# LBM-EPFL/MaD

Hardware: AMD Instinct MI355X
Metric: anchor-pair x rotation correlations/sec on 256^3 map; top-k pose agreement (higher is better)
Workload: dtype i8 (correlation, exact int32 accumulate) / f64 (binning, pose scoring)

## Files before the change

### include/mad_amd.h

```cpp
#ifndef MAD_AMD_H
#define MAD_AMD_H

#include <stdint.h>

#ifdef __cplusplus
extern "C" {
#endif

#define MAD_OK        0
#define MAD_EINVAL   -22
#define MAD_ENOMEM   -12
#define MAD_ENOSPC   -28
#define MAD_ENODEV   -19
#define MAD_EDOM     -33
#define MAD_EHIP     -5

#define MAD_MAX_Z      128
#define MAD_MAX_FIELDS 64
#define MAD_POSE_CLUSTER_MAX_N 4096
#define MAD_RESULT_COLS 23

typedef struct mad_ctx mad_ctx;
typedef struct mad_set mad_set;


int mad_init(int device, mad_ctx **out);
void mad_destroy(mad_ctx *ctx);
const char *mad_last_error(const mad_ctx *ctx);
int mad_synchronize(mad_ctx *ctx);
void *mad_stream(mad_ctx *ctx);
int mad_set_overlap(mad_ctx *ctx, int on);
int mad_timing_enable(mad_ctx *ctx, int on);
int mad_timing_reset(mad_ctx *ctx);
int mad_timing_get(mad_ctx *ctx, const char *what, double *total_ms, int64_t *launches);
double mad_last_ms(mad_ctx *ctx, const char *what);

int mad_probe_peaks(mad_ctx *ctx, double *copy_gbs, double *i8_tops);

int mad_set_eqsp(mad_ctx *ctx, int which, int Z, const double *bounds,
                 const double *to_dom, const double *adj_sec);


int mad_upload_field(mad_ctx *ctx, int slot, const float *gx, const float *gy, const float *gz,
                     int nx, int ny, int nz);
int mad_upload_field_device(mad_ctx *ctx, int slot, const float *g3_device, int nx, int ny, int nz);
int mad_free_field(mad_ctx *ctx, int slot);


int mad_set_orient_window(mad_ctx *ctx, double gw_sig);
int mad_orient(mad_ctx *ctx, int slot, int octave, const int32_t *coords, int n, int r,
               int lim_main, int lim_sec,
               int32_t *row_anchor, int32_t *row_main, int32_t *row_sec, double *row_R,
               int32_t *row_count, int64_t *n_rows, int64_t cap, int32_t *n_reject);


int mad_describe(mad_ctx *ctx, int slot, int octave, const int32_t *coords, const double *R,
                 int64_t n_rows, int r, int16_t *dsc);
int mad_describe_sized(mad_ctx *ctx, int slot, int octave, const int32_t *coords, const double *R,
                       int64_t n_rows, int r, int dsc_size, int16_t *dsc);


int mad_correlate(mad_ctx *ctx, const int16_t *hi, int64_t n_hi, const int16_t *lo, int64_t n_lo,
                  int D, double cc, int32_t *pair_hi, int32_t *pair_lo, double *pair_score,
                  int64_t *n_pairs, int64_t cap);


int mad_pose_score(mad_ctx *ctx, const int32_t *pair_hi, const int32_t *pair_lo, const double *pair_score,
                   int64_t n_pairs,
                   const double *hi_p, const double *hi_R, const int32_t *hi_meta, int64_t n_hi,
                   const double *lo_p, const double *lo_R, const int32_t *lo_meta, int64_t n_lo,
                   const double *hi_cloud, int64_t l_hi, const double *lo_cloud, int64_t l_lo,
                   double dist, double *results, int32_t *counts);

int mad_topk(mad_ctx *ctx, const int32_t *counts, int64_t n, int64_t k, int64_t *order);


int mad_set_create(mad_ctx *ctx, mad_set **out);
void mad_set_destroy(mad_ctx *ctx, mad_set *set);
int mad_set_build(mad_ctx *ctx, mad_set *set, const int *slot_of_octave,
                  const int32_t *anc_coords, const int32_t *anc_octave, const double *anc_subv,
                  const int32_t *anc_index, int n_anchors, int r, int lim_main, int lim_sec);
int mad_set_build_many(mad_ctx *ctx, int n_sets, mad_set *const *sets, const int *slot_of_octave,
                       const int32_t *const *anc_coords, const int32_t *const *anc_octave,
                       const double *const *anc_subv, const int32_t *const *anc_index, const int *n_anchors,
                       int r, int lim_main, int lim_sec);
int mad_set_mark_wide(mad_ctx *ctx, mad_set *set, int wide);
int mad_set_is_wide(mad_ctx *ctx, const mad_set *set);
int mad_set_load(mad_ctx *ctx, mad_set *set, int64_t n_rows, const int32_t *row_anchor,
                 const int32_t *row_main, const double *row_R, const int16_t *dsc, int D,
                 const double *anc_subv, const int32_t *anc_index, const int32_t *anc_octave, int n_anchors);
int mad_set_size(mad_ctx *ctx, const mad_set *set, int64_t *n_rows, int32_t *n_anchors);
int mad_set_download(mad_ctx *ctx, const mad_set *set, int32_t *row_anchor, int32_t *row_main,
                     int32_t *row_sec, double *row_R, int16_t *dsc);

int mad_match_topk(mad_ctx *ctx, const mad_set *hi, const mad_set *lo, double cc, double dist,
                   int64_t k, double *results, int64_t *pair_index, int64_t *n_out, int64_t *stats);
int mad_match_topk_many(mad_ctx *ctx, int n, const mad_set *const *hi, const mad_set *lo, double cc, double dist,
                        int64_t k, double *results, int64_t *pair_index, int64_t *n_out, int64_t *stats);

int mad_match_topk_many_begin(mad_ctx *ctx, int n, const mad_set *const *hi, const mad_set *lo, double cc, double dist,
                              int64_t k, double *results, int64_t *pair_index, int64_t *n_out, int64_t *stats);
int mad_match_topk_many_finish(mad_ctx *ctx);
int mad_match_topk_many_begin2(mad_ctx *ctx, int n, const mad_set *const *hi, const mad_set *lo, double cc, double dist,
                               int64_t k, double *results, int64_t *pair_index, int64_t *n_out, int64_t *stats,
                               uint8_t *used_hi, uint8_t *used_lo);
int mad_match_topk_many2(mad_ctx *ctx, int n, const mad_set *const *hi, const mad_set *lo, double cc, double dist,
                         int64_t k, double *results, int64_t *pair_index, int64_t *n_out, int64_t *stats,
                         uint8_t *used_hi, uint8_t *used_lo);
int mad_set_batching(mad_ctx *ctx, int on);
int mad_set_option(mad_ctx *ctx, const char *name, double value);

int mad_last_pose_kernel(mad_ctx *ctx);
int64_t mad_last_pose_selected(mad_ctx *ctx);
int64_t mad_device_allocations(mad_ctx *ctx);
int mad_match_fetch(mad_ctx *ctx, int32_t *pair_hi, int32_t *pair_lo, double *pair_score,
                    int32_t *counts, int64_t cap);
int mad_match_results(mad_ctx *ctx, const mad_set *hi, const mad_set *lo, double *results, int64_t cap);
int mad_match_used(mad_ctx *ctx, uint8_t *hi_anchor_used, int32_t n_hi_anchors,
                   uint8_t *lo_anchor_used, int32_t n_lo_anchors);


int mad_upload_density(mad_ctx *ctx, const float *grid, int nx, int ny, int nz,
                       double ox, double oy, double oz, double voxsp);
int mad_refine(mad_ctx *ctx, double *coords, int n_cand, int64_t n_atoms, int n_steps,
               double max_step, double min_step, int32_t *converged, int32_t *last_step);


int mad_structure_to_density(mad_ctx *ctx, const double *atoms, const double *mass, int64_t n,
                             double resolution, double voxsp, double isovalue, int pad,
                             int32_t dims[3], double origin[3], float *grid);


int mad_ccc(mad_ctx *ctx, float *grid1, const int32_t dims1[3], const double origin1[3],
            float *grid2, const int32_t dims2[3], const double origin2[3],
            double voxsp, double isovalue, double *ccc);


int mad_match_shard_pairs(mad_ctx *ctx, const mad_set *hi, const mad_set *lo, int64_t lo_begin, int64_t lo_end, double cc,
                          uint8_t *used_hi, uint8_t *used_lo, int64_t *n_pairs);

int mad_match_shard_topk(mad_ctx *ctx, const mad_set *hi, const mad_set *lo, const uint8_t *used_hi_all,
                         const uint8_t *used_lo_all, double dist, int64_t k, double *results, int64_t *pair_rank,
                         int32_t *counts, int64_t *n_out, int64_t *l_hi);

int64_t mad_match_shard_record_doubles(int64_t k);
int mad_match_shard_begin(mad_ctx *ctx, const mad_set *hi, const mad_set *lo, int64_t lo_begin, int64_t lo_end, int64_t n_lo,
                          double cc, uint8_t *d_flags);
int mad_match_shard_score(mad_ctx *ctx, const mad_set *hi, const mad_set *lo, const uint8_t *d_flags_all, double dist, int64_t k,
                          double *d_out);
int mad_match_shard_collect(mad_ctx *ctx, const mad_set *hi, const double *d_all, int64_t n, int *ticket);
int mad_match_shard_wait(mad_ctx *ctx, int ticket, double *out, int64_t n);


int64_t mad_set_wire_bytes(int D, int64_t cap_rows);
int mad_set_export(mad_ctx *ctx, const mad_set *share, void *wire, int wire_on_device, int64_t cap_rows);
int mad_set_import(mad_ctx *ctx, mad_set *set, const void *wires, int wires_on_device, int n_shares, int64_t cap_rows,
                   const int32_t *anc_coords, const int32_t *anc_octave, const double *anc_subv, const int32_t *anc_index,
                   int n_anchors);
int mad_set_lane(mad_ctx *ctx, const mad_set *set);
void *mad_set_stream(mad_ctx *ctx, const mad_set *set);
int mad_set_bind_lane(mad_ctx *ctx, mad_set *set, int lane);

int mad_density_ccc(mad_ctx *ctx, const double *atoms, const double *mass, int n_cand, int64_t n,
                    double resolution, double density_isovalue, double ccc_isovalue, double *ccc);

int mad_dock_refine_score(mad_ctx *ctx, int n_struct, const double *base_atoms, const double *mass, const int64_t *first_atom,
                          int n_cand, const int32_t *cand_struct, const double *hi_p, const double *lo_p, const double *rot,
                          int n_steps, double max_step, double min_step, double resolution, double density_isovalue,
                          double ccc_isovalue, double *coords, int32_t *converged, int32_t *last_step, double *ccc);


int mad_grid_overlap(mad_ctx *ctx, float *grid1, const int32_t d1[3], const double o1[3], float *grid2,
                     const int32_t d2[3], const double o2[3], double voxsp, double isovalue, int64_t *common,
                     int64_t *n_pos1);

int mad_overlap_matrix(mad_ctx *ctx, const double *atoms, const double *mass, const int64_t *first_atom,
                       int n_struct, double resolution, double voxsp, double density_isovalue,
                       double overlap_isovalue, double *overlap);


typedef struct mad_space mad_space;

int mad_space_create(mad_ctx *ctx, mad_space **out);
void mad_space_destroy(mad_ctx *ctx, mad_space *s);

int mad_space_build(mad_ctx *ctx, mad_space *s, const void *grid, int is_f64, int nx, int ny, int nz, int pad,
                    int oct_mode, const double *g0, const double *g2, int radius, double sig2,
                    const double *pre, int pre_radius, const double *const *lu, const double *const *ev_w,
                    const int32_t *const *ev_i, int slot_up, int slot_base);

int mad_space_info(mad_ctx *ctx, const mad_space *s, int *n_octaves, int32_t *dims6, int32_t *kind2, int32_t *is_f64_2);

int mad_space_download(mad_ctx *ctx, const mad_space *s, int entry, int what, void *out);

int mad_space_peaks(mad_ctx *ctx, const mad_space *s, int entry, double threshold, int border, int64_t *lin_index,
                    double *value, int64_t cap, int64_t *n_out);

int mad_space_patches(mad_ctx *ctx, const mad_space *s, int entry, const int32_t *coords, int n, int r, void *out);

int mad_space_localize(mad_ctx *ctx, const mad_space *s, int entry, const int32_t *cand, int n, int32_t *status,
                       int32_t *coord, void *H, void *G, int64_t *n_undecided);

int mad_localize_volume(mad_ctx *ctx, const void *vol, int is_f64, int nx, int ny, int nz, const int32_t *cand, int n,
                        int32_t *status, int32_t *coord, void *H, void *G, int64_t *n_undecided);

int mad_pose_cluster_many(mad_ctx *ctx, int n_match, const double *const *rows, const int32_t *n_rows,
                          const double *const *cloud, const int32_t *n_cloud, double rmsd_thresh, int32_t *const *owner_out,
                          double *const *d2min_out, int32_t *n_done_out, int32_t *status_out);

#ifdef __cplusplus
}
#endif
#endif
```

### mad_amd/_lib.py

```python
import ctypes as C
import os

import numpy as np

_HERE = os.path.dirname(os.path.abspath(__file__))
LIB_PATH = os.environ.get("MAD_LIB_PATH") or os.path.join(_HERE, "libmad_amd.so")
RESULT_COLS = 23
POSE_CLUSTER_MAX_N = 4096
WIDE_FROM_R = 11
WIDE_C = 108
WIDE_MAX = WIDE_C + 127

ERRORS = {-22: "EINVAL", -12: "ENOMEM", -28: "ENOSPC", -19: "ENODEV", -33: "EDOM", -5: "EHIP"}

SYMBOLS = [
    "mad_init", "mad_destroy", "mad_last_error", "mad_synchronize", "mad_stream", "mad_set_overlap",
    "mad_timing_enable", "mad_timing_reset", "mad_timing_get", "mad_last_ms", "mad_probe_peaks",
    "mad_set_eqsp", "mad_upload_field", "mad_upload_field_device", "mad_free_field",
    "mad_set_orient_window", "mad_orient", "mad_describe", "mad_describe_sized", "mad_correlate", "mad_pose_score", "mad_topk",
    "mad_set_create", "mad_set_destroy", "mad_set_build", "mad_set_build_many", "mad_set_load", "mad_set_mark_wide", "mad_set_is_wide", "mad_set_size", "mad_set_download",
    "mad_match_topk", "mad_match_topk_many", "mad_match_topk_many_begin", "mad_match_topk_many_finish", "mad_match_topk_many_begin2", "mad_match_topk_many2", "mad_set_batching", "mad_set_option", "mad_last_pose_kernel", "mad_last_pose_selected", "mad_device_allocations", "mad_match_fetch", "mad_match_results", "mad_match_used",
    "mad_match_shard_pairs", "mad_match_shard_topk", "mad_match_shard_begin", "mad_match_shard_score", "mad_match_shard_record_doubles", "mad_match_shard_collect", "mad_match_shard_wait",
    "mad_set_wire_bytes", "mad_set_export", "mad_set_import", "mad_set_lane", "mad_set_stream", "mad_set_bind_lane",
    "mad_upload_density", "mad_refine", "mad_structure_to_density", "mad_ccc", "mad_density_ccc", "mad_dock_refine_score", "mad_grid_overlap", "mad_overlap_matrix",
    "mad_space_create", "mad_space_destroy", "mad_space_build", "mad_space_info", "mad_space_download",
    "mad_space_peaks", "mad_space_patches", "mad_space_localize", "mad_localize_volume",
    "mad_pose_cluster_many",
]


class MadBackendError(RuntimeError):
    pass


_dll = None


def _share_torch_hip_runtime():
    import importlib.util
    if os.environ.get("MAD_OWN_HIP_RUNTIME", "0") == "1":
        return
    try:
        spec = importlib.util.find_spec("torch")
    except (ImportError, ValueError):
        spec = None
    if spec is None or not spec.submodule_search_locations:
        return
    for d in spec.submodule_search_locations:
        path = os.path.join(d, "lib", "libamdhip64.so")
        if os.path.exists(path):
            try:
                C.CDLL(path, mode=C.RTLD_GLOBAL)
            except OSError:
                pass
            return


def load_library():
    global _dll
    if _dll is None:
        if not os.path.exists(LIB_PATH):
            raise MadBackendError(
                "MaD> %s not found: build it with `python -c 'import __graft_entry__ as g; g.build()'` "
                "or `make -C mad_amd/csrc` (there is no CPU fallback)" % LIB_PATH)
        _share_torch_hip_runtime()
        try:
            _dll = C.CDLL(LIB_PATH)
        except OSError as e:
            raise MadBackendError("MaD> cannot load %s: %s" % (LIB_PATH, e))
        _dll.mad_last_error.restype = C.c_char_p
        _dll.mad_last_error.argtypes = [C.c_void_p]
        _dll.mad_stream.restype = C.c_void_p
        _dll.mad_stream.argtypes = [C.c_void_p]
        _dll.mad_last_ms.restype = C.c_double
        _dll.mad_last_ms.argtypes = [C.c_void_p, C.c_char_p]
        _dll.mad_set_stream.restype = C.c_void_p
        _dll.mad_set_stream.argtypes = [C.c_void_p, C.c_void_p]
        _dll.mad_last_pose_selected.restype = C.c_int64
        _dll.mad_last_pose_selected.argtypes = [C.c_void_p]
        _dll.mad_device_allocations.restype = C.c_int64
        _dll.mad_device_allocations.argtypes = [C.c_void_p]
        _dll.mad_set_wire_bytes.restype = C.c_int64
        _dll.mad_set_wire_bytes.argtypes = [C.c_int, C.c_int64]
        _dll.mad_match_shard_record_doubles.restype = C.c_int64
        _dll.mad_match_shard_record_doubles.argtypes = [C.c_int64]
        _dll.mad_destroy.restype = None
        _dll.mad_set_destroy.restype = None
        _dll.mad_space_destroy.restype = None
    return _dll


def _p(a):
    return a.ctypes.data_as(C.c_void_p) if a is not None else None


def _c(a, dt):
    return np.ascontiguousarray(a, dtype=dt)


def _pad_rows(dsc, to=128):
    d = dsc.shape[1] if dsc.ndim == 2 else 0
    if d == 0 or d % to == 0:
        return dsc
    out = np.zeros((dsc.shape[0], (d + to - 1) // to * to), dsc.dtype)
    out[:, :d] = dsc
    return out


class BuildBatch(object):

    def __init__(self, lib, jobs, r, lim_main, lim_sec, gw_sig=0.0):
        self.lib, self.r, self.lim_main, self.lim_sec, self.gw_sig = lib, int(r), int(lim_main), int(lim_sec), float(gw_sig)
        n = len(jobs)
        self.sets = [job[5] if len(job) > 5 and job[5] is not None else DeviceSet(lib) for job in jobs]
        self._keep = []
        coords, octave, subv, index, counts, slots = [], [], [], [], [], []
        for job in jobs:
            c, o = _c(job[1], np.int32).reshape(-1, 3), _c(job[2], np.int32)
            v, i = _c(job[3], np.float64).reshape(-1, 3), _c(job[4], np.int32)
            if not (len(c) == len(o) == len(v) == len(i)):
                raise ValueError("set_build_many: anchor arrays of different lengths")
            self._keep += [c, o, v, i]
            coords.append(c.ctypes.data); octave.append(o.ctypes.data); subv.append(v.ctypes.data); index.append(i.ctypes.data)
            counts.append(len(o))
            slots += [int(job[0][0]), int(job[0][1])]
        self.counts = counts
        self._h = (C.c_void_p * max(n, 1))(*[s.h.value for s in self.sets])
        self._slots = (C.c_int * max(2 * n, 1))(*slots)
        self._coords = (C.c_void_p * max(n, 1))(*coords)
        self._octave = (C.c_void_p * max(n, 1))(*octave)
        self._subv = (C.c_void_p * max(n, 1))(*subv)
        self._index = (C.c_void_p * max(n, 1))(*index)
        self._n = (C.c_int * max(n, 1))(*counts)

    def run(self):
        self.lib.set_orient_window(self.gw_sig)
        for s, n in zip(self.sets, self.counts):
            s.n_anchors = n
        self.lib._chk(self.lib.dll.mad_set_build_many(self.lib.ctx, C.c_int(len(self.sets)), self._h, self._slots, self._coords, self._octave,
                                                      self._subv, self._index, self._n, C.c_int(self.r), C.c_int(self.lim_main),
                                                      C.c_int(self.lim_sec)))
        return self.sets


class DeviceSet(object):

    def __init__(self, lib, lane=None):
        self.lib = lib
        self.h = C.c_void_p()
        lib._chk(lib.dll.mad_set_create(lib.ctx, C.byref(self.h)))
        self.n_anchors = 0
        if lane is not None:
            self.bind_lane(lane)

    def lane(self):
        return int(self.lib.dll.mad_set_lane(self.lib.ctx, self.h))

    def is_wide(self):
        return int(self.lib.dll.mad_set_is_wide(self.lib.ctx, self.h)) == 1

    def bind_lane(self, lane):
        self.lib._chk(self.lib.dll.mad_set_bind_lane(self.lib.ctx, self.h, C.c_int(int(lane))))

    def stream(self):
        return self.lib.dll.mad_set_stream(self.lib.ctx, self.h)

    def size(self):
        n = C.c_int64(0)
        a = C.c_int32(0)
        self.lib._chk(self.lib.dll.mad_set_size(self.lib.ctx, self.h, C.byref(n), C.byref(a)))
        return n.value, a.value

    def download(self, want_dsc=True, D=1024):
        n, _ = self.size()
# ... 246 lines not shown
        R = np.zeros((cap, 9))
        cnt = np.zeros((cap, Z), np.int32) if want_counts else None
        nrows = C.c_int64(0)
        nrej = C.c_int32(0)
        self._chk(self.dll.mad_orient(self.ctx, C.c_int(slot), C.c_int(octave), _p(coords), C.c_int(n), C.c_int(r),
                                      C.c_int(lim_main), C.c_int(lim_sec), _p(ra), _p(rm), _p(rs), _p(R), _p(cnt),
                                      C.byref(nrows), C.c_int64(cap), C.byref(nrej)))
        k = nrows.value
        return dict(anchor=ra[:k].copy(), main=rm[:k].copy(), sec=rs[:k].copy(), R=R[:k].reshape(k, 3, 3).copy(),
                    counts=None if cnt is None else cnt[:k].copy(), n_reject=nrej.value)

    def describe(self, slot, octave, coords, R, r=8, Zd=16, dsc_size=64):
        coords = _c(coords, np.int32).reshape(-1, 3)
        R = _c(R, np.float64).reshape(-1, 9)
        n = len(coords)
        out = np.zeros((n, dsc_size * Zd), np.int16)
        self._chk(self.dll.mad_describe_sized(self.ctx, C.c_int(slot), C.c_int(octave), _p(coords), _p(R), C.c_int64(n), C.c_int(r),
                                              C.c_int(dsc_size), _p(out)))
        return out

    def correlate(self, hi, lo, cc):
        hi, lo = _pad_rows(_c(hi, np.int16)), _pad_rows(_c(lo, np.int16))
        n_hi, D = hi.shape
        n_lo = lo.shape[0]
        npairs = C.c_int64(0)
        cap = 1 << 16
        while True:
            ph, pl, ps = np.zeros(cap, np.int32), np.zeros(cap, np.int32), np.zeros(cap)
            rc = self.dll.mad_correlate(self.ctx, _p(hi), C.c_int64(n_hi), _p(lo), C.c_int64(n_lo), C.c_int(D), C.c_double(cc),
                                        _p(ph), _p(pl), _p(ps), C.byref(npairs), C.c_int64(cap))
            if rc == -28:
                cap = npairs.value
                continue
            self._chk(rc)
            break
        k = npairs.value
        return ph[:k].copy(), pl[:k].copy(), ps[:k].copy()

    def pose_score(self, pair_hi, pair_lo, pair_score, hi_p, hi_R, hi_meta, lo_p, lo_R, lo_meta, hi_cloud, lo_cloud,
                   dist=4.0, want_results=True):
        pair_hi, pair_lo = _c(pair_hi, np.int32), _c(pair_lo, np.int32)
        pair_score = _c(pair_score, np.float64)
        hi_p, lo_p = _c(hi_p, np.float64), _c(lo_p, np.float64)
        hi_R, lo_R = _c(hi_R, np.float64).reshape(-1, 9), _c(lo_R, np.float64).reshape(-1, 9)
        hi_meta, lo_meta = _c(hi_meta, np.int32), _c(lo_meta, np.int32)
        hi_cloud, lo_cloud = _c(hi_cloud, np.float64), _c(lo_cloud, np.float64)
        n = len(pair_hi)
        res = np.zeros((n, RESULT_COLS)) if want_results else None
        cnt = np.zeros(n, np.int32)
        self._chk(self.dll.mad_pose_score(self.ctx, _p(pair_hi), _p(pair_lo), _p(pair_score), C.c_int64(n),
                                          _p(hi_p), _p(hi_R), _p(hi_meta), C.c_int64(len(hi_p)),
                                          _p(lo_p), _p(lo_R), _p(lo_meta), C.c_int64(len(lo_p)),
                                          _p(hi_cloud), C.c_int64(len(hi_cloud)), _p(lo_cloud), C.c_int64(len(lo_cloud)),
                                          C.c_double(dist), _p(res), _p(cnt)))
        return res, cnt

    def topk(self, counts, k):
        counts = _c(counts, np.int32)
        k = min(int(k), len(counts))
        order = np.zeros(max(k, 1), np.int64)
        self._chk(self.dll.mad_topk(self.ctx, _p(counts), C.c_int64(len(counts)), C.c_int64(k), _p(order)))
        return order[:k]

    def set_build(self, slots, anc_coords, anc_octave, anc_subv, anc_index, r=8, lim_main=6, lim_sec=6, into=None, gw_sig=0.0):
        self.set_orient_window(gw_sig)
        s = into if into is not None else DeviceSet(self)
        slots = (C.c_int * 2)(int(slots[0]), int(slots[1]))
        anc_coords = _c(anc_coords, np.int32).reshape(-1, 3)
        anc_octave = _c(anc_octave, np.int32)
        anc_subv = _c(anc_subv, np.float64).reshape(-1, 3)
        anc_index = _c(anc_index, np.int32)
        s.n_anchors = len(anc_octave)
        self._chk(self.dll.mad_set_build(self.ctx, s.h, slots, _p(anc_coords), _p(anc_octave), _p(anc_subv), _p(anc_index),
                                         C.c_int(len(anc_octave)), C.c_int(r), C.c_int(lim_main), C.c_int(lim_sec)))
        return s

    def prepare_build_many(self, jobs, r=8, lim_main=6, lim_sec=6, gw_sig=0.0):
        return BuildBatch(self, jobs, r, lim_main, lim_sec, gw_sig)

    def set_build_many(self, jobs, r=8, lim_main=6, lim_sec=6, gw_sig=0.0):
        return self.prepare_build_many(jobs, r, lim_main, lim_sec, gw_sig).run()

    def set_load(self, row_anchor, row_main, row_R, dsc, anc_subv, anc_index, anc_octave, wide=False):
        s = DeviceSet(self)
        if wide:
            self._chk(self.dll.mad_set_mark_wide(self.ctx, s.h, C.c_int(1)))
        row_anchor, row_main = _c(row_anchor, np.int32), _c(row_main, np.int32)
        row_R = _c(row_R, np.float64).reshape(-1, 9)
        dsc = _c(dsc, np.int16)
        if dsc.ndim != 2:
            dsc = dsc.reshape(len(row_anchor), -1)
        dsc = _pad_rows(dsc)
        anc_subv = _c(anc_subv, np.float64).reshape(-1, 3)
        anc_index, anc_octave = _c(anc_index, np.int32), _c(anc_octave, np.int32)
        s.n_anchors = len(anc_index)
        self._chk(self.dll.mad_set_load(self.ctx, s.h, C.c_int64(len(row_anchor)), _p(row_anchor), _p(row_main), _p(row_R),
                                        _p(dsc), C.c_int(dsc.shape[1] if len(dsc) else 1024), _p(anc_subv), _p(anc_index),
                                        _p(anc_octave), C.c_int(len(anc_index))))
        return s

    def match_topk(self, hi, lo, cc, dist, k):
        k = int(k)
        res = np.zeros((max(k, 1), RESULT_COLS))
        idx = np.zeros(max(k, 1), np.int64)
        n_out = C.c_int64(0)
        stats = np.zeros(4, np.int64)
        self._chk(self.dll.mad_match_topk(self.ctx, hi.h, lo.h, C.c_double(cc), C.c_double(dist), C.c_int64(k), _p(res), _p(idx),
                                          C.byref(n_out), _p(stats)))
        g = n_out.value
        return res[:g], idx[:g], dict(n_pairs=int(stats[0]), l_hi=int(stats[1]), l_lo=int(stats[2]), n_corr=int(stats[3]))

    def match_topk_many(self, his, lo, cc, dist, k, want_used=False):
        h = self._many_args(his, lo, k, want_used)
        n = h["n"]
        if want_used:
            self._chk(self.dll.mad_match_topk_many2(self.ctx, C.c_int(n), h["arr"], lo.h, C.c_double(cc), C.c_double(dist), C.c_int64(h["k"]),
                                                    _p(h["res"]), _p(h["idx"]), _p(h["n_out"]), _p(h["stats"]), _p(h["used_hi"]),
                                                    _p(h["used_lo"])))
        else:
            self._chk(self.dll.mad_match_topk_many(self.ctx, C.c_int(n), h["arr"], lo.h, C.c_double(cc), C.c_double(dist), C.c_int64(h["k"]),
                                                   _p(h["res"]), _p(h["idx"]), _p(h["n_out"]), _p(h["stats"])))
        return self._many_unpack(h)

    @staticmethod
    def _many_args(his, lo, k, want_used):
        k = int(k)
        n = len(his)
        h = dict(n=n, k=k, res=np.zeros((max(n, 1), max(k, 1), RESULT_COLS)), idx=np.zeros((max(n, 1), max(k, 1)), np.int64),
                 n_out=np.zeros(max(n, 1), np.int64), stats=np.zeros((max(n, 1), 4), np.int64), sets=(list(his), lo),
                 arr=(C.c_void_p * max(n, 1))(*[x.h.value for x in his]), want_used=bool(want_used))
        if want_used:
            h["hi_off"] = np.concatenate([[0], np.cumsum([x.n_anchors for x in his], dtype=np.int64)]).astype(np.int64)
            h["used_hi"] = np.zeros(max(int(h["hi_off"][-1]), 1), np.uint8)
            h["used_lo"] = np.zeros((max(n, 1), max(lo.n_anchors, 1)), np.uint8)
        return h

    @staticmethod
    def _many_unpack(h):
        out = []
        for i in range(h["n"]):
            g = int(h["n_out"][i])
            st = h["stats"][i]
            row = (h["res"][i, :g], h["idx"][i, :g], dict(n_pairs=int(st[0]), l_hi=int(st[1]), l_lo=int(st[2]), n_corr=int(st[3])))
            if h["want_used"]:
                a, b = int(h["hi_off"][i]), int(h["hi_off"][i + 1])
                n_lo = h["sets"][1].n_anchors
                row += (h["used_hi"][a:b].astype(bool), h["used_lo"][i, :n_lo].astype(bool))
            out.append(row)
        return out

    def last_pose_kernel(self):
        return int(self.dll.mad_last_pose_kernel(self.ctx))

    def last_pose_selected(self):
        return int(self.dll.mad_last_pose_selected(self.ctx))

    def device_allocations(self):
        return int(self.dll.mad_device_allocations(self.ctx))

    def match_topk_many_begin(self, his, lo, cc, dist, k, want_used=False):
        h = self._many_args(his, lo, k, want_used)
        n = h["n"]
        if want_used:
            self._chk(self.dll.mad_match_topk_many_begin2(self.ctx, C.c_int(n), h["arr"], lo.h, C.c_double(cc), C.c_double(dist),
                                                          C.c_int64(h["k"]), _p(h["res"]), _p(h["idx"]), _p(h["n_out"]), _p(h["stats"]),
                                                          _p(h["used_hi"]), _p(h["used_lo"])))
        else:
            self._chk(self.dll.mad_match_topk_many_begin(self.ctx, C.c_int(n), h["arr"], lo.h, C.c_double(cc), C.c_double(dist),
                                                         C.c_int64(h["k"]), _p(h["res"]), _p(h["idx"]), _p(h["n_out"]), _p(h["stats"])))
        self._open_brackets = getattr(self, "_open_brackets", []) + [h]
        return h

    def match_topk_many_finish(self, h):
        pending = getattr(self, "_open_brackets", [])
        if not pending or pending[0] is not h:
            raise MadBackendError("MaD> match_topk_many_finish: brackets finish in the order they were begun")
        self._open_brackets = pending[1:]
        self._chk(self.dll.mad_match_topk_many_finish(self.ctx))
        return self._many_unpack(h)

    def match_shard_pairs(self, hi, lo, lo_begin, lo_end, cc):
        used_hi, used_lo = np.zeros(max(hi.n_anchors, 1), np.uint8), np.zeros(max(lo.n_anchors, 1), np.uint8)
        n = C.c_int64(0)
        self._chk(self.dll.mad_match_shard_pairs(self.ctx, hi.h, lo.h, C.c_int64(lo_begin), C.c_int64(lo_end), C.c_double(cc),
                                                 _p(used_hi), _p(used_lo), C.byref(n)))
        return used_hi[:hi.n_anchors], used_lo[:lo.n_anchors], n.value

    def match_shard_topk(self, hi, lo, used_hi_all, used_lo_all, dist, k):
        uh, ul = _c(used_hi_all, np.uint8), _c(used_lo_all, np.uint8)
        assert len(uh) == hi.n_anchors and len(ul) == lo.n_anchors
        res = np.zeros((k, RESULT_COLS))
        rank, cnt = np.zeros(k, np.int64), np.zeros(k, np.int32)
        n, l_hi = C.c_int64(0), C.c_int64(0)
        self._chk(self.dll.mad_match_shard_topk(self.ctx, hi.h, lo.h, _p(uh), _p(ul), C.c_double(dist), C.c_int64(k), _p(res), _p(rank),
                                                _p(cnt), C.byref(n), C.byref(l_hi)))
        m = n.value
        return res[:m].copy(), cnt[:m].copy(), rank[:m].copy(), l_hi.value

    def match_shard_record_doubles(self, k):
        return int(self.dll.mad_match_shard_record_doubles(C.c_int64(int(k))))

    def match_shard_begin(self, hi, lo, lo_begin, lo_end, n_lo, cc, flags_ptr):
        self._chk(self.dll.mad_match_shard_begin(self.ctx, hi.h, lo.h, C.c_int64(int(lo_begin)), C.c_int64(int(lo_end)), C.c_int64(int(n_lo)),
                                                 C.c_double(cc), C.c_void_p(int(flags_ptr))))

    def match_shard_score(self, hi, lo, flags_all_ptr, dist, k, out_ptr):
        self._chk(self.dll.mad_match_shard_score(self.ctx, hi.h, lo.h, C.c_void_p(int(flags_all_ptr)), C.c_double(dist), C.c_int64(int(k)),
                                                 C.c_void_p(int(out_ptr))))

    def match_shard_collect(self, hi, all_ptr, n):
        t = C.c_int(0)
        self._chk(self.dll.mad_match_shard_collect(self.ctx, hi.h, C.c_void_p(int(all_ptr)), C.c_int64(int(n)), C.byref(t)))
        return t.value

    def match_shard_wait(self, ticket, n):
        out = np.zeros(int(n))
        self._chk(self.dll.mad_match_shard_wait(self.ctx, C.c_int(int(ticket)), _p(out), C.c_int64(int(n))))
        return out

    def set_wire_bytes(self, cap_rows, D=1024):
        n = int(self.dll.mad_set_wire_bytes(C.c_int(int(D)), C.c_int64(int(cap_rows))))
        if n < 0:
            raise ValueError("set_wire_bytes(%r, %r)" % (cap_rows, D))
        return n

    def set_export(self, share, cap_rows, wire=None, device_ptr=None):
        if device_ptr is not None:
            self._chk(self.dll.mad_set_export(self.ctx, share.h, C.c_void_p(int(device_ptr)), C.c_int(1), C.c_int64(int(cap_rows))))
            return None
        nbytes = self.set_wire_bytes(cap_rows)
        if wire is None:
            wire = np.zeros(nbytes, np.uint8)
        if wire.dtype != np.uint8 or wire.size != nbytes or not wire.flags.c_contiguous:
            raise ValueError("set_export: wire must be a contiguous uint8 array of %d bytes" % nbytes)
        self._chk(self.dll.mad_set_export(self.ctx, share.h, _p(wire), C.c_int(0), C.c_int64(int(cap_rows))))
        return wire

    def set_import(self, n_shares, cap_rows, anc_coords, anc_octave, anc_subv, anc_index, wires=None, device_ptr=None, into=None):
        s = into if into is not None else DeviceSet(self)
        anc_octave = _c(anc_octave, np.int32)
        anc_subv = _c(anc_subv, np.float64).reshape(-1, 3)
        anc_index = _c(anc_index, np.int32)
        anc_coords = None if anc_coords is None else _c(anc_coords, np.int32).reshape(-1, 3)
        n = len(anc_octave)
        if len(anc_subv) != n or len(anc_index) != n or (anc_coords is not None and len(anc_coords) != n):
            raise ValueError("set_import: anchor arrays of different lengths")
        if device_ptr is not None:
            src, on_dev = C.c_void_p(int(device_ptr)), 1
        else:
            wires = np.ascontiguousarray(wires, dtype=np.uint8)
            if wires.size != n_shares * self.set_wire_bytes(cap_rows):
                raise ValueError("set_import: %d bytes for %d shares of %d" % (wires.size, n_shares, self.set_wire_bytes(cap_rows)))
            src, on_dev = _p(wires), 0
        s.n_anchors = n
        self._chk(self.dll.mad_set_import(self.ctx, s.h, src, C.c_int(on_dev), C.c_int(int(n_shares)), C.c_int64(int(cap_rows)),
                                          _p(anc_coords), _p(anc_octave), _p(anc_subv), _p(anc_index), C.c_int(n)))
        return s

    def match_fetch(self, n_pairs):
        ph, pl = np.zeros(n_pairs, np.int32), np.zeros(n_pairs, np.int32)
        ps, cn = np.zeros(n_pairs), np.zeros(n_pairs, np.int32)
        self._chk(self.dll.mad_match_fetch(self.ctx, _p(ph), _p(pl), _p(ps), _p(cn), C.c_int64(n_pairs)))
        return ph, pl, ps, cn

    def match_results(self, hi, lo, n_pairs):
        res = np.zeros((max(n_pairs, 1), RESULT_COLS))
        self._chk(self.dll.mad_match_results(self.ctx, hi.h, lo.h, _p(res), C.c_int64(n_pairs)))
        return res[:n_pairs]

    def match_used(self, n_hi_anchors, n_lo_anchors):
        uh, ul = np.zeros(max(n_hi_anchors, 1), np.uint8), np.zeros(max(n_lo_anchors, 1), np.uint8)
        self._chk(self.dll.mad_match_used(self.ctx, _p(uh), C.c_int32(n_hi_anchors), _p(ul), C.c_int32(n_lo_anchors)))
        return uh[:n_hi_anchors].astype(bool), ul[:n_lo_anchors].astype(bool)

    def pose_cluster_many(self, rows_list, clouds, n_samples_list, rmsd_thresh=10.0):
        nm = len(rows_list)
        if not (len(clouds) == len(n_samples_list) == nm):
            raise ValueError("pose_cluster_many: %d row lists, %d clouds, %d sample counts" % (nm, len(clouds), len(n_samples_list)))
        rows, cl, ns = [], [], []
        for r, c, k in zip(rows_list, clouds, n_samples_list):
            r = _c(r, np.float64).reshape(-1, RESULT_COLS)
            if int(k) < 0:
                raise ValueError("pose_cluster_many: n_samples = %d" % int(k))
            rows.append(r)
            cl.append(_c(c, np.float64).reshape(-1, 3))
            ns.append(min(len(r), int(k)))
        owner = [np.zeros(n, np.int32) for n in ns]
        d2min = [np.zeros(n, np.float64) for n in ns]
        n_rows, n_cloud = np.array(ns, np.int32), np.array([len(c) for c in cl], np.int32)
        n_done, status = np.zeros(max(nm, 1), np.int32), np.zeros(max(nm, 1), np.int32)
        PP = C.c_void_p * max(nm, 1)
        ptrs = [PP(*[a.ctypes.data if a.size else None for a in arrs]) for arrs in (rows, cl, owner, d2min)]
        self._chk(self.dll.mad_pose_cluster_many(self.ctx, C.c_int(nm), ptrs[0], _p(n_rows), ptrs[1], _p(n_cloud), C.c_double(float(rmsd_thresh)),
                                                 ptrs[2], ptrs[3], _p(n_done), _p(status)))
        return [(owner[m], d2min[m], int(n_done[m]), int(status[m])) for m in range(nm)]

    def upload_density(self, grid, origin, voxsp):
        grid = _c(grid, np.float32)
        nx, ny, nz = grid.shape
        self._chk(self.dll.mad_upload_density(self.ctx, _p(grid), C.c_int(nx), C.c_int(ny), C.c_int(nz),
                                              C.c_double(origin[0]), C.c_double(origin[1]), C.c_double(origin[2]), C.c_double(voxsp)))

    def refine(self, coords, n_steps=500, max_step=0.5, min_step=0.01):
        c = _c(coords, np.float64).copy()
        single = c.ndim == 2
        if single:
# ... 118 lines not shown
```

### mad_amd/csrc/mad_common.h

```cpp
#pragma once

#include <hip/hip_runtime.h>

#include <cmath>
#include <cstdarg>
#include <cstdint>
#include <cstdio>
#include <cstdlib>
#include <cstring>

#include "../../include/mad_amd.h"

#define MAD_WAVE 64
#define MAD_ZLUT 1024
#define MAD_MAX_BELT 32


struct __attribute__((aligned(16))) EqspFastLds {
    float g32[MAD_MAX_Z][4];
    float z_in_lo[MAD_MAX_BELT], z_in_hi[MAD_MAX_BELT], belt_lo0[MAD_MAX_BELT], belt_inv_w[MAD_MAX_BELT];
    int belt_first[MAD_MAX_BELT], belt_count[MAD_MAX_BELT];
    unsigned char zlut[MAD_ZLUT];
    float4 belt_f[MAD_MAX_BELT];
    int2 belt_i[MAD_MAX_BELT];
    double dir[MAD_MAX_Z][4];
    double zthr[MAD_MAX_BELT][4];
    int nbelt;
    int tier2_ok;
    double th_lo[MAD_MAX_Z], th_hi[MAD_MAX_Z], ph_lo[MAD_MAX_BELT], ph_hi[MAD_MAX_BELT];
};

#define MAD_TAB_BELTS 4
#define MAD_TAB_PBINS 2048
#define MAD_TAB_ZBINS 2048
#define MAD_TAB_GUARD 4e-3
struct __attribute__((aligned(16))) EqspTabLds {
    unsigned char zbelt[MAD_TAB_ZBINS];
    unsigned char ptab[MAD_TAB_BELTS][MAD_TAB_PBINS];
};

#define MAD_T2_MARGIN64 1e-9
#define MAD_T2_MARGIN32 2e-6

struct EqspDev {
    int Z;
    int nbelt;
    double th_lo[MAD_MAX_Z];
    double th_hi[MAD_MAX_Z];
    double ph_lo[MAD_MAX_Z];
    double ph_hi[MAD_MAX_Z];
    int belt_first[MAD_MAX_Z];
    int belt_count[MAD_MAX_Z];
    double to_dom[MAD_MAX_Z][9];
    double adj_sec[MAD_MAX_Z][9];
    unsigned char zlut[MAD_ZLUT];
    float z_in_lo[MAD_MAX_BELT];
    float z_in_hi[MAD_MAX_BELT];
    float belt_lo0[MAD_MAX_BELT];
    float belt_inv_w[MAD_MAX_BELT];
    int belt_first32[MAD_MAX_BELT];
    int belt_count32[MAD_MAX_BELT];
    float g32[MAD_MAX_Z][4];
    EqspFastLds image;
    EqspTabLds tab;
    int tab_ok;
};

#ifndef MAD_EQSP_GUARD
#define MAD_EQSP_GUARD 4e-5
#endif

struct FieldDev {
    const float4 *tex;
    int nx, ny, nz;
    const unsigned *tex4;
};

#ifdef __HIPCC__
__host__ __device__
#endif
static inline bool mad_ball_interior(int c0, int c1, int c2, int nx, int ny, int nz) {
    const int reach = 14;
    return c0 - reach >= 1 && c0 + reach <= nx - 2 && c1 - reach >= 1 && c1 + reach <= ny - 2 && c2 - reach >= 1 && c2 + reach <= nz - 2;
}


struct DevBuf {
    void *p = nullptr;
    size_t cap = 0;
};

enum { MAD_T_ORIENT = 0, MAD_T_DESCRIBE, MAD_T_CORRELATE, MAD_T_PAIRS, MAD_T_POSE, MAD_T_TOPK, MAD_T_REFINE,
       MAD_T_DENSITY, MAD_T_CCC, MAD_T_COUNT };

#define MAD_T_RING 32
#define MAD_LANES 8
#define MAD_BRACKETS 3
#define MAD_SHARD_RING 8
#define MAD_RES (2 * MAD_LANES)

struct TimerGroup {
    hipEvent_t start[MAD_T_RING];
    hipEvent_t stop[MAD_T_RING];
    int pending = 0;
    double total_ms = 0.0;
    int64_t launches = 0;
};

struct DensityDev {
    float *grid = nullptr;
    float4 *grad = nullptr;
    int nx = 0, ny = 0, nz = 0;
    double o[3] = {0, 0, 0};
    double vs = 0;
};

struct MatchState {
    int64_t n_pairs = 0;
    int32_t l_hi = 0, l_lo = 0;
    int32_t n_hi_anchors = 0, n_lo_anchors = 0;
    int64_t cap_c = 0;
    int64_t cap_pairs = 0;
    int lane = 0;
    bool pruned = false, fits = true;
    const void *hi = nullptr, *lo = nullptr;
    uint64_t hi_gen = 0, lo_gen = 0;
    double dist = 0;
    int64_t cap_pairs_used = 0;
    int64_t n_sel = 0;
    const void *shard_hi = nullptr, *shard_lo = nullptr;
    int64_t shard_begin = 0, shard_end = 0, shard_pairs = 0, shard_cap_pairs = 0;
};

struct ShardAsync {
    const void *hi = nullptr, *lo = nullptr;
    uint64_t hi_gen = 0, lo_gen = 0;
    int64_t begin = 0, nb = 0, n_lo = 0, cap_pairs = 0;
};

struct mad_ctx {
    int device = -1;
    hipStream_t stream = nullptr;
    hipStream_t lane_stream[MAD_LANES] = {};
    int next_set_lane = 0;
    bool overlap = true;
    int ori_queue_cap = 1 << 20, dsc_queue_cap = 1 << 20;
    int pose_mx = 0;
    int pose_split = -1;
    int64_t n_device_allocs = 0;
    int64_t pose_split_min = 4096;
    bool batch_gemm = false;
    bool spatial_order = true;
    char err[512] = {0};
    FieldDev fields[MAD_MAX_FIELDS];
    void *field_mem[MAD_MAX_FIELDS];
    EqspDev *eq[2] = {nullptr, nullptr};
    EqspDev eq_host[2];
    bool eq_set[2] = {false, false};
    double gw_sig = 0.0, gw_built = 0.0;
    unsigned long long *gw_tab = nullptr;
    int gw_r = -1;
    int8_t *mask_off = nullptr;
    int mask_r = -1;
    int mask_n = 0;
    unsigned *ball_colinfo = nullptr;
    bool dsc_ball = false;
    DevBuf scratch[64 * MAD_LANES];
    int lane = 0;
    hipEvent_t lane_done[MAD_BRACKETS][MAD_RES];
    hipEvent_t lane_pre[MAD_LANES];
    hipEvent_t gemm_done[MAD_BRACKETS];
    void *host_res[MAD_BRACKETS][MAD_RES] = {};
    size_t host_res_cap[MAD_BRACKETS][MAD_RES] = {};
    void *host_used[MAD_BRACKETS][MAD_RES] = {};
    size_t host_used_cap[MAD_BRACKETS][MAD_RES] = {};
    int res_slot = 0, res_idx = 0;
    int64_t *pinned = nullptr;
    int next_pinned = 64;
    DensityDev dens;
    MatchState match;
    ShardAsync shard_async[MAD_LANES];
    void *shard_host[MAD_LANES][MAD_SHARD_RING] = {};
    size_t shard_host_cap[MAD_LANES][MAD_SHARD_RING] = {};
    hipEvent_t shard_ev[MAD_LANES][MAD_SHARD_RING] = {};
    bool shard_busy[MAD_LANES][MAD_SHARD_RING] = {};
    int shard_next[MAD_LANES] = {};
    int last_pose_kernel = -1;
    int64_t lane_sel_hint[MAD_LANES] = {};
    void *many[MAD_BRACKETS] = {};
    int many_oldest = 0, many_open = 0;
    bool timing = false;
    TimerGroup timers[MAD_T_COUNT];
    int n_cu = 256;
};

#define MAD_WIDE_FROM_R 11
#define MAD_WIDE_C 108
#define MAD_WIDE_MAX (MAD_WIDE_C + 127)
#define MAD_WIDE_ZERO4 ((int32_t)0x94949494)
#define MAD_WIDE_BIAS(sum, D) (MAD_WIDE_C * (int)(sum) - ((int)(D) / 2) * (MAD_WIDE_C * MAD_WIDE_C))
static_assert((uint8_t)(int8_t)-MAD_WIDE_C == 0x94, "MAD_WIDE_ZERO4");

struct mad_set {
    int32_t n_anchors = 0;
    uint64_t gen = 0;
    int64_t cap_rows = 0;
    int D = 0;
    DevBuf anc_blob;
    DevBuf anc_coords, anc_octave, anc_subv, anc_index, anc_canon;
    DevBuf anc_order;
    void *host_stage = nullptr;
    size_t host_stage_cap = 0;
    int staged_n = -1;
    bool staged_coords = false;
    hipEvent_t uploaded = nullptr;
    int lane = 0;
    hipEvent_t built = nullptr;
    DevBuf row_anchor, row_main, row_sec, row_R, row_Rinv, row_meta, dsc, dsc8, norm;
    DevBuf rsum;
    bool wide = false;
    bool wide_mark = false;
    DevBuf row_perm;
    DevBuf row_rec;
    DevBuf anc_rows;
    int n_rowwise = 0;
    int ball_dims[3] = {0, 0, 0};
    int last_fan = 0;
    DevBuf dev_n;
    int64_t n_rows_host = -1;
    bool range_bad = false;
    int64_t rows_hint = 0;
    FieldDev last_f[2];
    int last_r = 0;
    bool last_perm = false, last_rec = false;
    int pinned_slot = 0;
    hipEvent_t ready = nullptr;
    DevBuf cell_start, cell_pts, cell_ids;
    double cell_min[3] = {0, 0, 0};
    double bb_min[3] = {0, 0, 0}, bb_max[3] = {0, 0, 0};
    double cell_size = 0;
    int cell_dim[3] = {0, 0, 0};
    bool cells_ready = false;
};

#define MAD_BATCH_MAX 16
template <class Args> struct Batch {
    int n_jobs;
    int first[MAD_BATCH_MAX + 1];
    Args job[MAD_BATCH_MAX];
};
template <class Args> __device__ __forceinline__ int batch_job(const Batch<Args> &B, int block) {
    int j = 0;
    while (j + 1 < B.n_jobs && block >= B.first[j + 1]) j++;
    return j;
}

enum {
    S_COORDS = 0, S_OCT, S_SLOT_CNT, S_SLOT_MAIN, S_SLOT_SEC, S_SLOT_HIST, S_ROW_OFF, S_SCAN_TMP,
    S_ROW_ANCHOR, S_ROW_MAIN, S_ROW_SEC, S_ROW_R, S_ROW_COUNT, S_DSC, S_ROW_COORDS,
    S_HI16, S_LO16, S_HI8, S_LO8, S_HNORM, S_LNORM, S_CMAT, S_ROWCNT, S_ROWOFF,
    S_PAIR_HI, S_PAIR_LO, S_PAIR_SCORE, S_COUNTS, S_USED_HI, S_USED_LO, S_HI_CLOUD, S_MISC,
    S_HIST, S_SEL, S_RESULTS, S_TMP_A, S_TMP_B, S_TMP_C, S_TMP_D, S_TMP_E, S_TMP_F, S_TMP_G,
    S_TIE_FLAG, S_TIE_OFF, S_SEL_OUT, S_TMP_H, S_TMP_I, S_TMP_J,
    S_CELL_START, S_CELL_PTS, S_CELL_IDS, S_PG_START, S_PG_PTS, S_PG_PTSF, S_ZERO, S_CMASK, S_PG_BITS, S_PG_PAIRS, S_PERM_OFF, S_CFLAG,
    S_FILT_IN, S_FILT_D2, S_FILT_OUT,
    S_N_SLOTS
};
static_assert(S_N_SLOTS <= 64, "grow mad_ctx::scratch");

int mad_fail(mad_ctx *ctx, int code, const char *fmt, ...);
int mad_reserve(mad_ctx *ctx, DevBuf &b, size_t bytes);
void mad_release(DevBuf &b);
int mad_field_alloc(mad_ctx *ctx, int slot, int nx, int ny, int nz, size_t *n_texels);
static inline DevBuf &mad_sb(mad_ctx *ctx, int slot) { return ctx->scratch[ctx->lane * 64 + slot]; }
static inline void mad_use_lane(mad_ctx *ctx, int lane) { ctx->lane = lane; ctx->stream = ctx->lane_stream[ctx->overlap ? lane : 0]; }
template <class T> static inline T *scratch(mad_ctx *ctx, int slot) { return (T *)mad_sb(ctx, slot).p; }

void mad_timer_begin(mad_ctx *ctx, int group);
void mad_timer_end(mad_ctx *ctx, int group);

int mad_scan_i32(mad_ctx *ctx, const int32_t *in, int32_t *out, int64_t n);

void mad_scan_small(mad_ctx *ctx, const int32_t *in, int32_t *out, const int32_t *d_n, int32_t *total_out, int n_host = 0);

struct alignas(16) DscRowRec {
    int32_t row;
    int32_t c[3];
    int32_t octave;
    int32_t pad0[3];
    double inv[9];
    int32_t pad1[6];
    float hf[9];
    float rf[9];
    float ru[3];
    int32_t pad2[3];
};
#define MAD_ROWREC_WORDS ((int)(sizeof(DscRowRec) / 4))
#define MAD_ANCROW_WORDS 8
static_assert(sizeof(DscRowRec) == 224 && offsetof(DscRowRec, hf) == 128, "k_describe reads the first 32 dwords of a DscRowRec");

struct OrientOut {
    int32_t *row_anchor, *row_main, *row_sec;
    double *row_R;
    int32_t *row_count;
    double *row_Rinv = nullptr;
    int32_t *row_meta = nullptr;
    const int32_t *anc_index = nullptr, *anc_octave = nullptr;
    const int32_t *anc_order = nullptr;
    int32_t *row_perm = nullptr;
    DscRowRec *row_rec = nullptr;
    int32_t *anc_rows = nullptr;
    bool counters_zeroed = false;
    int32_t *d_n_rows;
    int32_t *d_n_reject;
};
int mad_orient_device(mad_ctx *ctx, FieldDev f0, FieldDev f1, const int32_t *d_coords, const int32_t *d_octave,
                      int uniform_octave, int n, int r, int lim_main, int lim_sec, OrientOut out);
struct OrientJob {
    FieldDev f[2];
    const int32_t *d_coords, *d_octave;
    int uniform_octave;
    int n;
    OrientOut out;
};
struct DescribeJob {
    FieldDev f[2];
    const int32_t *d_anc_coords, *d_anc_octave;
    int uniform_octave;
    const int32_t *d_row_anchor;
    const double *d_row_R, *d_row_Rinv;
    const int32_t *d_row_perm = nullptr;
    const DscRowRec *d_row_rec = nullptr;
    const int32_t *d_anc_rows = nullptr;
    int n_anchors = 0, n_rowwise = 0, fan = 0;
    const int32_t *d_n_rows;
    int64_t grid_rows;
    int32_t *d_overflow;
    int16_t *d_dsc;
    int8_t *d_dsc8;
// ... 267 lines not shown
```

### mad_amd/csrc/mad_ctx.hip

```cpp
#include "mad_common.h"

static char g_init_err[512] = "";
#define MAD_TWO_PI_H 6.283185307179586476925286766559

int mad_fail(mad_ctx *ctx, int code, const char *fmt, ...) {
    char *dst = ctx ? ctx->err : g_init_err;
    va_list ap;
    va_start(ap, fmt);
    vsnprintf(dst, 512, fmt, ap);
    va_end(ap);
    return code;
}

extern "C" const char *mad_last_error(const mad_ctx *ctx) { return ctx ? ctx->err : g_init_err; }

int mad_reserve(mad_ctx *ctx, DevBuf &b, size_t bytes) {
    if (bytes == 0) bytes = 16;
    if (b.cap >= bytes) return MAD_OK;
    if (b.p) {
        MAD_HIP(hipStreamSynchronize(ctx->stream));
        (void)hipFree(b.p);
        b.p = nullptr;
        b.cap = 0;
    }
    size_t want = bytes + bytes / 4 + 256;
    want = (want + 255) & ~size_t(255);
    hipError_t e = hipMalloc(&b.p, want);
    if (e != hipSuccess) {
        b.p = nullptr;
        return mad_fail(ctx, MAD_ENOMEM, "hipMalloc(%zu) failed: %s", want, hipGetErrorString(e));
    }
    b.cap = want;
    ctx->n_device_allocs++;
    return MAD_OK;
}

extern "C" int64_t mad_device_allocations(mad_ctx *ctx) { return ctx ? ctx->n_device_allocs : -1; }

void mad_release(DevBuf &b) {
    if (b.p) (void)hipFree(b.p);
    b.p = nullptr;
    b.cap = 0;
}

extern "C" int mad_init(int device, mad_ctx **out) {
    if (!out) return mad_fail(nullptr, MAD_EINVAL, "mad_init: out is NULL");
    *out = nullptr;
    int ndev = 0;
    hipError_t e = hipGetDeviceCount(&ndev);
    if (e != hipSuccess || ndev == 0)
        return mad_fail(nullptr, MAD_ENODEV, "mad_init: no HIP device (%s)", hipGetErrorString(e));
    if (device < 0 || device >= ndev) return mad_fail(nullptr, MAD_EINVAL, "mad_init: device %d of %d", device, ndev);
    e = hipSetDevice(device);
    if (e != hipSuccess) return mad_fail(nullptr, MAD_ENODEV, "hipSetDevice(%d): %s", device, hipGetErrorString(e));
    hipDeviceProp_t prop;
    e = hipGetDeviceProperties(&prop, device);
    if (e != hipSuccess) return mad_fail(nullptr, MAD_ENODEV, "hipGetDeviceProperties: %s", hipGetErrorString(e));
    if (strncmp(prop.gcnArchName, "gfx950", 6) != 0)
        return mad_fail(nullptr, MAD_ENODEV, "mad_init: device %d is %s; this library is built for gfx950 only", device,
                        prop.gcnArchName);
    mad_ctx *ctx = new mad_ctx();
    ctx->spatial_order = getenv("MAD_NO_SPATIAL_ORDER") == nullptr;
    ctx->batch_gemm = getenv("MAD_GEMM_BATCH") != nullptr;
    if (getenv("MAD_POSE_SPLIT_MIN")) ctx->pose_split_min = atoll(getenv("MAD_POSE_SPLIT_MIN"));
    if (getenv("MAD_POSE_SPLIT")) ctx->pose_split = atoi(getenv("MAD_POSE_SPLIT"));
    if (getenv("MAD_POSE_MX")) ctx->pose_mx = atoi(getenv("MAD_POSE_MX")) != 0;
    if (getenv("MAD_BALL")) ctx->dsc_ball = atoi(getenv("MAD_BALL")) != 0;
    ctx->device = device;
    ctx->n_cu = prop.multiProcessorCount;
    for (int i = 0; i < MAD_MAX_FIELDS; i++) {
        ctx->fields[i] = FieldDev{nullptr, 0, 0, 0};
        ctx->field_mem[i] = nullptr;
    }
    bool streams_ok = true;
    for (int l = 0; l < MAD_LANES; l++) streams_ok &= hipStreamCreateWithFlags(&ctx->lane_stream[l], hipStreamNonBlocking) == hipSuccess;
    ctx->stream = ctx->lane_stream[0];
    if (!streams_ok ||
        hipMalloc((void **)&ctx->eq[0], sizeof(EqspDev)) != hipSuccess ||
        hipMalloc((void **)&ctx->eq[1], sizeof(EqspDev)) != hipSuccess ||
        hipHostMalloc((void **)&ctx->pinned, 8192) != hipSuccess) {
        mad_fail(nullptr, MAD_EHIP, "mad_init: stream / table allocation failed");
        delete ctx;
        return MAD_EHIP;
    }
    for (int g = 0; g < MAD_T_COUNT; g++)
        for (int i = 0; i < MAD_T_RING; i++) {
            (void)hipEventCreate(&ctx->timers[g].start[i]);
            (void)hipEventCreate(&ctx->timers[g].stop[i]);
        }
    for (int r = 0; r < MAD_BRACKETS; r++)
        for (int l = 0; l < MAD_RES; l++) (void)hipEventCreateWithFlags(&ctx->lane_done[r][l], hipEventDisableTiming);
    for (int l = 0; l < MAD_LANES; l++) (void)hipEventCreateWithFlags(&ctx->lane_pre[l], hipEventDisableTiming);
    for (int r = 0; r < MAD_BRACKETS; r++) (void)hipEventCreateWithFlags(&ctx->gemm_done[r], hipEventDisableTiming);
    *out = ctx;
    return MAD_OK;
}

extern "C" void mad_destroy(mad_ctx *ctx) {
    if (ctx) { mad_synchronize(ctx); mad_many_abandon(ctx); }
    if (!ctx) return;
    (void)hipSetDevice(ctx->device);
    for (int l = 0; l < MAD_LANES; l++) (void)hipStreamSynchronize(ctx->lane_stream[l]);
    for (int i = 0; i < MAD_MAX_FIELDS; i++)
        if (ctx->field_mem[i]) (void)hipFree(ctx->field_mem[i]);
    for (auto &b : ctx->scratch) mad_release(b);
    if (ctx->eq[0]) (void)hipFree(ctx->eq[0]);
    if (ctx->eq[1]) (void)hipFree(ctx->eq[1]);
    if (ctx->mask_off) (void)hipFree(ctx->mask_off);
    if (ctx->gw_tab) (void)hipFree(ctx->gw_tab);
    if (ctx->pinned) (void)hipHostFree(ctx->pinned);
    if (ctx->dens.grid) (void)hipFree(ctx->dens.grid);
    if (ctx->dens.grad) (void)hipFree(ctx->dens.grad);
    for (int g = 0; g < MAD_T_COUNT; g++)
        for (int i = 0; i < MAD_T_RING; i++) {
            (void)hipEventDestroy(ctx->timers[g].start[i]);
            (void)hipEventDestroy(ctx->timers[g].stop[i]);
        }
    for (int r = 0; r < MAD_BRACKETS; r++) (void)hipEventDestroy(ctx->gemm_done[r]);
    for (int l = 0; l < MAD_LANES; l++) (void)hipEventDestroy(ctx->lane_pre[l]);
    for (int l = 0; l < MAD_LANES; l++)
        for (int r = 0; r < MAD_SHARD_RING; r++) {
            if (ctx->shard_ev[l][r]) (void)hipEventDestroy(ctx->shard_ev[l][r]);
            if (ctx->shard_host[l][r]) (void)hipHostFree(ctx->shard_host[l][r]);
        }
    for (int l = 0; l < MAD_RES; l++)
        for (int r = 0; r < MAD_BRACKETS; r++) {
            (void)hipEventDestroy(ctx->lane_done[r][l]);
            if (ctx->host_res[r][l]) (void)hipHostFree(ctx->host_res[r][l]);
            if (ctx->host_used[r][l]) (void)hipHostFree(ctx->host_used[r][l]);
        }
    for (int l = 0; l < MAD_LANES; l++)
        if (ctx->lane_stream[l]) (void)hipStreamDestroy(ctx->lane_stream[l]);
    delete ctx;
}

extern "C" int mad_synchronize(mad_ctx *ctx) {
    if (!ctx) return MAD_EINVAL;
    for (int l = 0; l < MAD_LANES; l++) MAD_HIP(hipStreamSynchronize(ctx->lane_stream[l]));
    return MAD_OK;
}

extern "C" int mad_set_overlap(mad_ctx *ctx, int on) {
    if (!ctx) return MAD_EINVAL;
    MAD_TRY(mad_synchronize(ctx));
    ctx->overlap = on != 0;
    mad_use_lane(ctx, 0);
    return MAD_OK;
}

extern "C" void *mad_stream(mad_ctx *ctx) { return ctx ? (void *)ctx->lane_stream[0] : nullptr; }


static void timer_drain(mad_ctx *ctx, TimerGroup &t) {
    for (int i = 0; i < t.pending; i++) {
        float ms = 0;
        if (hipEventSynchronize(t.stop[i]) == hipSuccess && hipEventElapsedTime(&ms, t.start[i], t.stop[i]) == hipSuccess)
            t.total_ms += ms;
        t.launches++;
    }
    t.pending = 0;
}

void mad_timer_begin(mad_ctx *ctx, int group) {
    if (!ctx->timing) return;
    TimerGroup &t = ctx->timers[group];
    if (t.pending == MAD_T_RING) timer_drain(ctx, t);
    (void)hipEventRecord(t.start[t.pending], ctx->stream);
}

void mad_timer_end(mad_ctx *ctx, int group) {
    if (!ctx->timing) return;
    TimerGroup &t = ctx->timers[group];
    (void)hipEventRecord(t.stop[t.pending], ctx->stream);
    t.pending++;
}

static const char *k_timer_names[MAD_T_COUNT] = {"orient", "describe", "correlate", "pairs", "pose",
                                                 "topk",   "refine",   "density",   "ccc"};

extern "C" int mad_timing_enable(mad_ctx *ctx, int on) {
    if (!ctx) return MAD_EINVAL;
    ctx->timing = on != 0;
    return MAD_OK;
}

extern "C" int mad_timing_reset(mad_ctx *ctx) {
    if (!ctx) return MAD_EINVAL;
    for (int g = 0; g < MAD_T_COUNT; g++) {
        timer_drain(ctx, ctx->timers[g]);
        ctx->timers[g].total_ms = 0;
        ctx->timers[g].launches = 0;
    }
    return MAD_OK;
}

extern "C" int mad_timing_get(mad_ctx *ctx, const char *what, double *total_ms, int64_t *launches) {
    if (!ctx || !what) return MAD_EINVAL;
    for (int g = 0; g < MAD_T_COUNT; g++)
        if (strcmp(what, k_timer_names[g]) == 0) {
            timer_drain(ctx, ctx->timers[g]);
            if (total_ms) *total_ms = ctx->timers[g].total_ms;
            if (launches) *launches = ctx->timers[g].launches;
            return MAD_OK;
        }
    return mad_fail(ctx, MAD_EINVAL, "mad_timing_get: unknown group '%s'", what);
}

extern "C" double mad_last_ms(mad_ctx *ctx, const char *what) {
    double t = -1;
    int64_t n = 0;
    if (mad_timing_get(ctx, what, &t, &n) != MAD_OK || n == 0) return -1.0;
    return t / (double)n;
}


extern "C" int mad_set_eqsp(mad_ctx *ctx, int which, int Z, const double *bounds, const double *to_dom,
                            const double *adj_sec) {
    if (!ctx) return MAD_EINVAL;
// ... 423 lines not shown
```

### mad_amd/csrc/mad_match.hip

```cpp
#include <vector>

#include "mad_common.h"

enum { ST_NPAIRS = 0, ST_LHI, ST_LLO, ST_NKEYS, ST_FLAG_C, ST_FLAG_PAIRS, ST_BAD, ST_NSEL, ST_NHI = 8, ST_NLO = 12, ST_FLAG_SEL = 16, ST_COUNT = 20 };


__global__ __launch_bounds__(256) void k_pack_rows(const int16_t *__restrict__ src, const int32_t *__restrict__ n_ptr, int D,
                                                   int8_t *__restrict__ dst, double *__restrict__ norm,
                                                   int32_t *__restrict__ bad) {
    const int64_t n = *n_ptr;
    const int64_t n_pad = (n + 127) / 128 * 128;
    const int lane = lane_id();
    const int64_t wave = (int64_t)blockIdx.x * 4 + (threadIdx.x >> 6), nw = (int64_t)gridDim.x * 4;
    for (int64_t row = wave; row < n_pad; row += nw) {
        if (row >= n) {
            for (int k = lane; k < D; k += MAD_WAVE) dst[row * D + k] = 0;
            if (lane == 0) norm[row] = 0.0;
            continue;
        }
        long long ss = 0;
        int oob = 0;
        for (int k = lane; k < D; k += MAD_WAVE) {
            const int v = src[row * D + k];
            if (v > 127 || v < -128) oob = 1;
// ... 337 lines not shown
                const int b = __ffs(m) - 1;
                m &= m - 1;
                list[o++] = (unsigned)((f + q) * 32 + b);
            }
        }
        __builtin_amdgcn_fence(__ATOMIC_ACQ_REL, "wavefront");
    }
    return total;
}

__global__ __launch_bounds__(256) void k_pair_count(const int32_t *__restrict__ C, uint32_t *__restrict__ mask, const uint8_t *__restrict__ cflag,
                                                    const int32_t *__restrict__ n_hi_ptr, const int32_t *__restrict__ n_lo_ptr,
                                                    const double *__restrict__ hn, const double *__restrict__ ln, double cc,
                                                    int32_t *__restrict__ row_cnt, const int32_t *__restrict__ status) {
    __shared__ unsigned s_list[4][PAIR_LIST];
    if (status[ST_FLAG_C]) return;
    const int64_t n_hi = *n_hi_ptr, n_lo = *n_lo_ptr;
    const int64_t ldc = (n_lo + GEMM_BN - 1) / GEMM_BN * GEMM_BN, ldm = ldc / 32, ldf = mad_cflag_pitch(ldc);
    const int lane = (int)lane_id();
    unsigned *const list = s_list[threadIdx.x >> 6];
    for (int64_t i = (int64_t)blockIdx.x * 4 + (threadIdx.x >> 6); i < n_hi; i += (int64_t)gridDim.x * 4) {
        const double nh = hn[i];
        uint32_t *const mrow = mask + i * ldm;
        int c = 0;
        for (int64_t f0 = 0; f0 < ldf; f0 += PAIR_WORDS * MAD_WAVE) {
            unsigned mw[PAIR_WORDS];
            const int total = pair_list_row(mrow, cflag + i * ldf, f0, ldf, list, mw);
            if (total > PAIR_LIST) {
#pragma unroll
                for (int q = 0; q < PAIR_WORDS; q++) {
                    unsigned m = mw[q], exact = 0;
                    if (!m) continue;
                    const int64_t w = f0 + PAIR_WORDS * lane + q;
                    while (m) {
                        const int b = __ffs(m) - 1;
                        m &= m - 1;
                        const int64_t j = w * 32 + b;
                        if (j < n_lo && corr_score(C[i * ldc + j], nh, ln[j]) > cc) exact |= 1u << b;
                    }
                    mrow[w] = exact;
                    c += __popc(exact);
                }
                continue;
            }
            for (int k = lane; k < total; k += MAD_WAVE) {
                const int64_t j = list[k];
                const bool ok = j < n_lo && corr_score(C[i * ldc + j], nh, ln[j]) > cc;
                if (!ok) atomicAnd(&mrow[j >> 5], ~(1u << (j & 31)));
                c += ok ? 1 : 0;
            }
        }
        c = wave_sum_i32(c);
        if (lane == 0) row_cnt[i] = c;
    }
}

__global__ __launch_bounds__(256) void k_pair_emit2(const int32_t *__restrict__ C, const uint32_t *__restrict__ mask, const uint8_t *__restrict__ cflag,
                                                    const int32_t *__restrict__ n_hi_ptr, const int32_t *__restrict__ n_lo_ptr,
                                                    const double *__restrict__ hn, const double *__restrict__ ln,
                                                    const int32_t *__restrict__ row_cnt, int64_t cap_pairs,
                                                    int32_t *__restrict__ pair_hi, int32_t *__restrict__ pair_lo,
                                                    double *__restrict__ pair_score, const int32_t *__restrict__ hi_row_anchor,
                                                    const int32_t *__restrict__ lo_row_anchor, const int32_t *__restrict__ hi_canon,
                                                    const int32_t *__restrict__ lo_canon, uint8_t *__restrict__ used_hi,
                                                    uint8_t *__restrict__ used_lo, int32_t *__restrict__ status) {
    __shared__ unsigned s_list[4][PAIR_LIST];
    __shared__ long long s_sum[4];
    __shared__ int s_cnt[4];
    if (status[ST_FLAG_C]) return;
    const int64_t n_hi = *n_hi_ptr, n_lo = *n_lo_ptr;
    const int64_t ldc = (n_lo + GEMM_BN - 1) / GEMM_BN * GEMM_BN, ldm = ldc / 32, ldf = mad_cflag_pitch(ldc);
    const int lane = (int)lane_id(), wv = threadIdx.x >> 6;
    unsigned *const list = s_list[wv];
    auto block_sum = [&](int64_t a, int64_t b) -> long long {
        long long v = 0;
        for (int64_t q = a + threadIdx.x; q < b; q += 256) v += row_cnt[q];
#pragma unroll
        for (int o = 32; o > 0; o >>= 1) v += __shfl_xor(v, o, MAD_WAVE);
        __syncthreads();
        if (lane == 0) s_sum[wv] = v;
        __syncthreads();
        return s_sum[0] + s_sum[1] + s_sum[2] + s_sum[3];
    };
    if (blockIdx.x == 0) {
        const long long total = block_sum(0, n_hi);
        if (threadIdx.x == 0) {
            status[ST_NPAIRS] = (int32_t)min(total, (long long)INT32_MAX);
            if (total > cap_pairs) status[ST_FLAG_PAIRS] = 1;
        }
    }
    int64_t done = 0;
    long long before = 0;
    for (int64_t i0 = (int64_t)blockIdx.x * 4; i0 < n_hi; i0 += (int64_t)gridDim.x * 4) {
        before += block_sum(done, i0);
        const int64_t i = i0 + wv;
        const int count = i < n_hi ? row_cnt[i] : 0;
        if (lane == 0) s_cnt[wv] = count;
        __syncthreads();
        long long mine = before;
        for (int q = 0; q < wv; q++) mine += s_cnt[q];
        before += s_cnt[0] + s_cnt[1] + s_cnt[2] + s_cnt[3];
        done = min(i0 + 4, n_hi);
        if (count == 0 || mine + count > cap_pairs) continue;
        const double nh = hn[i];
        int64_t base = mine;
        auto put = [&](int64_t o, int64_t j) {
            pair_hi[o] = (int32_t)i;
            pair_lo[o] = (int32_t)j;
            pair_score[o] = corr_score(C[i * ldc + j], nh, ln[j]);
            if (used_lo) { const int a = lo_row_anchor ? lo_row_anchor[j] : (int)j; used_lo[lo_canon ? lo_canon[a] : a] = 1; }
        };
        for (int64_t f0 = 0; f0 < ldf; f0 += PAIR_WORDS * MAD_WAVE) {
            unsigned mw[PAIR_WORDS];
            const int total = pair_list_row(mask + i * ldm, cflag + i * ldf, f0, ldf, list, mw);
            if (total > PAIR_LIST) {
                int pc = 0;
#pragma unroll
                for (int q = 0; q < PAIR_WORDS; q++) pc += __popc(mw[q]);
                int64_t o = base + wave_incl_scan_i32(pc) - pc;
#pragma unroll
                for (int q = 0; q < PAIR_WORDS; q++) {
                    unsigned m = mw[q];
                    while (m) {
                        const int b = __ffs(m) - 1;
                        m &= m - 1;
                        put(o++, (f0 + PAIR_WORDS * lane + q) * 32 + b);
                    }
                }
            } else {
                for (int k = lane; k < total; k += MAD_WAVE) put(base + k, (int64_t)list[k]);
            }
            base += total;
        }
        if (lane == 0 && used_hi) { const int a = hi_row_anchor ? hi_row_anchor[i] : (int)i; used_hi[hi_canon ? hi_canon[a] : a] = 1; }
    }
}


struct CloudJob {
    const double *subv;
    const uint8_t *used;
    int n;
    double *cloud;
    int32_t *count;
    const int32_t *hi_words, *lo_words;
    int32_t *status;
};

__device__ __forceinline__ void compact_cloud_block(const CloudJob &J, int *wt , int *s_base) {
    if (threadIdx.x == 0) *s_base = 0;
    if (J.hi_words && threadIdx.x < 4) J.status[ST_NHI + threadIdx.x] = J.hi_words[threadIdx.x];
    if (J.lo_words && threadIdx.x >= 4 && threadIdx.x < 8) J.status[ST_NLO + threadIdx.x - 4] = J.lo_words[threadIdx.x - 4];
    __syncthreads();
    for (int b = 0; b < J.n; b += 1024) {
        const int i = b + threadIdx.x;
        const bool p = i < J.n && (!J.used || J.used[i]);
        int tot;
        const int pos = block_excl_scan(p ? 1 : 0, wt, &tot);
        if (p) {
            const int o = *s_base + pos;
            J.cloud[3 * o] = J.subv[3 * i]; J.cloud[3 * o + 1] = J.subv[3 * i + 1]; J.cloud[3 * o + 2] = J.subv[3 * i + 2];
        }
        __syncthreads();
        if (threadIdx.x == 0) *s_base += tot;
        __syncthreads();
    }
    if (threadIdx.x == 0) *J.count = *s_base;
}

__global__ __launch_bounds__(1024) void k_compact_cloud(CloudJob J) {
    __shared__ int wt[17];
    __shared__ int s_base;
    compact_cloud_block(J, wt, &s_base);
}

__global__ void k_count_flags(const uint8_t *__restrict__ used, int n, int32_t *__restrict__ count) {
    const int i = blockIdx.x * blockDim.x + threadIdx.x;
    const int v = (i < n && used[i]) ? 1 : 0;
    const int s = wave_sum_i32(v);
    if (lane_id() == 0 && s) atomicAdd(count, s);
}

struct PoseGrid {
    double mn[3];
    double inv_cell[3];
    float inv_cell_f[3];
    int dim[3];
    int ncell;
};

__device__ __forceinline__ int pg_cell(double v, double mn, double inv, int dim) {
    const int c = (int)floor((v - mn) * inv);
    return min(max(c, 0), dim - 1);
}

__device__ __forceinline__ void pose_grid_block(const double *__restrict__ pts, const uint8_t *__restrict__ used, int n, const PoseGrid &G,
                                                int32_t *__restrict__ cell_start, unsigned short *__restrict__ cell_start16,
                                                double *__restrict__ sorted, float4 *__restrict__ sorted_f, int32_t *__restrict__ n_used,
                                                int *cnt, int *wt, int *carry_p) {
    int &carry = *carry_p;
    for (int c = threadIdx.x; c < G.ncell; c += 1024) cnt[c] = 0;
    if (threadIdx.x == 0) carry = 0;
    __syncthreads();
    for (int i = threadIdx.x; i < n; i += 1024)
        if (!used || used[i]) {
            const int c = (pg_cell(pts[3 * i], G.mn[0], G.inv_cell[0], G.dim[0]) * G.dim[1] +
                           pg_cell(pts[3 * i + 1], G.mn[1], G.inv_cell[1], G.dim[1])) * G.dim[2] +
                          pg_cell(pts[3 * i + 2], G.mn[2], G.inv_cell[2], G.dim[2]);
            atomicAdd(&cnt[c], 1);
        }
    __syncthreads();
    {
        const int per = (G.ncell + 1023) / 1024;
        const int c0 = min((int)threadIdx.x * per, G.ncell), c1 = min(c0 + per, G.ncell);
        int sum = 0;
        for (int c = c0; c < c1; c++) sum += cnt[c];
        int tot;
        int run = block_excl_scan(sum, wt, &tot);
        for (int c = c0; c < c1; c++) {
            const int v = cnt[c];
            cnt[c] = run; cell_start[c] = run; cell_start16[c] = (unsigned short)run;
            run += v;
        }
        if (threadIdx.x == 0) carry = tot;
        __syncthreads();
    }
    if (threadIdx.x == 0) {
        cell_start[G.ncell] = carry; *n_used = carry;
        cell_start16[G.ncell] = (unsigned short)carry; cell_start16[G.ncell + 1] = 0;
    }
    __syncthreads();
    for (int i = threadIdx.x; i < n; i += 1024)
        if (!used || used[i]) {
            const int c = (pg_cell(pts[3 * i], G.mn[0], G.inv_cell[0], G.dim[0]) * G.dim[1] +
                           pg_cell(pts[3 * i + 1], G.mn[1], G.inv_cell[1], G.dim[1])) * G.dim[2] +
                          pg_cell(pts[3 * i + 2], G.mn[2], G.inv_cell[2], G.dim[2]);
            const int o = atomicAdd(&cnt[c], 1);
            sorted[3 * o] = pts[3 * i]; sorted[3 * o + 1] = pts[3 * i + 1]; sorted[3 * o + 2] = pts[3 * i + 2];
            if (sorted_f)
                sorted_f[o] = make_float4((float)(pts[3 * i] - G.mn[0]), (float)(pts[3 * i + 1] - G.mn[1]), (float)(pts[3 * i + 2] - G.mn[2]), 0.f);
        }
}

__global__ __launch_bounds__(1024) void k_pose_grid_build(const double *__restrict__ pts, const uint8_t *__restrict__ used, int n,
                                                          PoseGrid G, int32_t *__restrict__ cell_start,
                                                          unsigned short *__restrict__ cell_start16, double *__restrict__ sorted,
                                                          float4 *__restrict__ sorted_f, int32_t *__restrict__ n_used, CloudJob J) {
    extern __shared__ __align__(16) unsigned char smem[];
    __shared__ int wt[17];
    __shared__ int carry;
    if (J.subv) {
        compact_cloud_block(J, wt, &carry);
        __syncthreads();
    }
    pose_grid_block(pts, used, n, G, cell_start, cell_start16, sorted, sorted_f, n_used, (int *)smem, wt, &carry);
}

__host__ __device__ __forceinline__ size_t pad16(size_t b) { return (b + 15) & ~(size_t)15; }

struct PoseBits {
    double mn[3];
    double h;
    int dim[3];
    int wz;
};

struct PoseBitsJobs {
    PoseBits B[4];
    double rad[4];
    int plane[4];
    int planes[4];
    unsigned *bits[4];
};

__device__ __forceinline__ void pose_bits_point(const PoseBits &B, double rad, int plane, int planes, unsigned *__restrict__ bits, double qx,
                                                double qy, double qz, int t0, int nthr) {
    const double inv_h = 1.0 / B.h, rad2 = rad * rad;
    const double px = qx - B.mn[0], py = qy - B.mn[1], pz = qz - B.mn[2];
    const int x0 = max((int)floor((px - rad) * inv_h - 0.5), 0), x1 = min((int)ceil((px + rad) * inv_h - 0.5), B.dim[0] - 1);
    const int y0 = max((int)floor((py - rad) * inv_h - 0.5), 0), y1 = min((int)ceil((py + rad) * inv_h - 0.5), B.dim[1] - 1);
    const int ny = y1 - y0 + 1, nrow = (x1 - x0 + 1) * ny;
    for (int t = t0; t < nrow; t += nthr) {
        const int kx = x0 + t / ny, ky = y0 + t % ny;
        const double dx = (kx + 0.5) * B.h - px, dy = (ky + 0.5) * B.h - py;
        const double rem = rad2 - dx * dx - dy * dy;
        if (rem < 0.0) continue;
        const double sq = sqrt(rem);
        const int z0 = max(plane == 0 ? (int)floor((pz - sq) * inv_h - 0.5) : (int)ceil((pz - sq) * inv_h - 0.5 + 1e-9), 0);
        const int z1 = min(plane == 0 ? (int)ceil((pz + sq) * inv_h - 0.5) : (int)floor((pz + sq) * inv_h - 0.5 - 1e-9), B.dim[2] - 1);
        if (z1 < z0) continue;
        unsigned *row = bits + planes * ((size_t)kx * B.dim[1] + ky) * B.wz + plane;
        for (int w = z0 >> 5; w <= (z1 >> 5); w++) {
            const int lo = max(z0 - 32 * w, 0), hi = min(z1 - 32 * w, 31);
            const unsigned m = (hi == 31 ? 0xffffffffu : ((1u << (hi + 1)) - 1u)) & ~((1u << lo) - 1u);
            atomicOr(&row[planes * w], m);
        }
    }
}

__global__ __launch_bounds__(256) void k_pose_bits(const double *__restrict__ sorted, const int32_t *__restrict__ cell_start, int ncell,
                                                   PoseBitsJobs J) {
    const PoseBits B = J.B[blockIdx.y];
    const int l_lo = cell_start[ncell];
    for (int p = blockIdx.x; p < l_lo; p += gridDim.x)
        pose_bits_point(B, J.rad[blockIdx.y], J.plane[blockIdx.y], J.planes[blockIdx.y], J.bits[blockIdx.y], sorted[3 * p], sorted[3 * p + 1],
                        sorted[3 * p + 2], (int)threadIdx.x, 256);
}

struct PoseVox {
    float m[9], t[3];
};

__device__ __forceinline__ void pose_vox_setup(const double *R, double ph0, double ph1, double ph2, double pl0, double pl1, double pl2,
                                               const PoseBits &B, PoseVox *V) {
    const double ih = 1.0 / B.h;
    for (int i = 0; i < 9; i++) V->m[i] = (float)(R[i] * ih);
    V->t[0] = (float)(((pl0 - (ph0 * R[0] + ph1 * R[1] + ph2 * R[2])) - B.mn[0]) * ih);
    V->t[1] = (float)(((pl1 - (ph0 * R[3] + ph1 * R[4] + ph2 * R[5])) - B.mn[1]) * ih);
    V->t[2] = (float)(((pl2 - (ph0 * R[6] + ph1 * R[7] + ph2 * R[8])) - B.mn[2]) * ih);
}

__device__ __forceinline__ void pose_vox_fetch(const PoseVox &V, float cx, float cy, float cz, const PoseBits &B,
                                               const unsigned *bits, uint2 *word, int *bit) {
    const float vx = fmaf(cz, V.m[2], fmaf(cy, V.m[1], fmaf(cx, V.m[0], V.t[0])));
    const float vy = fmaf(cz, V.m[5], fmaf(cy, V.m[4], fmaf(cx, V.m[3], V.t[1])));
    const float vz = fmaf(cz, V.m[8], fmaf(cy, V.m[7], fmaf(cx, V.m[6], V.t[2])));
    const int ix = cvt_floor(vx), iy = cvt_floor(vy), iz = cvt_floor(vz);
    *bit = iz & 31;
    *word = make_uint2(0u, 0u);
    const bool in = ((unsigned)ix < (unsigned)B.dim[0]) & ((unsigned)iy < (unsigned)B.dim[1]) & ((unsigned)iz < (unsigned)B.dim[2]);
    if (in) *word = ((const uint2 *)bits)[mad_u24(mad_u24((unsigned)ix, (unsigned)B.dim[1], (unsigned)iy), (unsigned)B.wz, (unsigned)(iz >> 5))];
}

#define POSE_STACK 128
#define POSE_BATCH 4
template <class Cloud32, class Exact>
__device__ __forceinline__ int pose_count_filtered(int l_hi, const PoseVox &V, const PoseBits &B, const unsigned *bits,
                                                   unsigned short *stack, Cloud32 cloud32, Exact exact) {
    const int lane = lane_id();
    int nq = 0, cnt = 0;
    for (int a0 = 0; a0 < l_hi; a0 += MAD_WAVE * POSE_BATCH) {
        uint2 word[POSE_BATCH];
        int bit[POSE_BATCH];
#pragma unroll
        for (int u = 0; u < POSE_BATCH; u++) {
            const int a = a0 + u * MAD_WAVE + lane;
            word[u] = make_uint2(0u, 0u); bit[u] = 0;
            if (a < l_hi) {
                float cx, cy, cz;
                cloud32(a, cx, cy, cz);
                pose_vox_fetch(V, cx, cy, cz, B, bits, &word[u], &bit[u]);
            }
        }
#pragma unroll
        for (int u = 0; u < POSE_BATCH; u++) {
            if (a0 + u * MAD_WAVE >= l_hi) break;
            const bool certain = (word[u].y >> bit[u]) & 1u;
            cnt += certain ? 1 : 0;
            const bool sv = ((word[u].x >> bit[u]) & 1u) && !certain;
            const unsigned long long bal = __ballot(sv);
            if (sv) stack[nq + __popcll(bal & lanemask_lt())] = (unsigned short)(a0 + u * MAD_WAVE + lane);
            nq += __popcll(bal);
            if (nq >= MAD_WAVE) {
                __builtin_amdgcn_wave_barrier();
                const int a2 = stack[nq - MAD_WAVE + lane];
                __builtin_amdgcn_wave_barrier();
                cnt += exact(a2) ? 1 : 0;
                nq -= MAD_WAVE;
            }
        }
    }
    if (nq > 0) {
        __builtin_amdgcn_wave_barrier();
        const int a2 = lane < nq ? stack[lane] : 0;
        __builtin_amdgcn_wave_barrier();
        if (lane < nq) cnt += exact(a2) ? 1 : 0;
    }
    return cnt;
}

struct PosePair {
    double R[9];
    double ph[3], pl[3];
    PoseVox vf, vc;
};

__device__ __forceinline__ void pose_prep_range(const int32_t *__restrict__ pair_hi, const int32_t *__restrict__ pair_lo, int64_t n_pairs,
                                                int64_t first, int64_t stride, const double *__restrict__ hi_p, const double *__restrict__ hi_R,
                                                const double *__restrict__ lo_p, const double *__restrict__ lo_Rinv,
                                                const int32_t *__restrict__ hi_row_anchor, const int32_t *__restrict__ lo_row_anchor,
                                                const PoseBits &Bf, const PoseBits &Bc, PosePair *__restrict__ rec) {
    for (int64_t p = first; p < n_pairs; p += stride) {
        const int ih = pair_hi[p], il = pair_lo[p];
        PosePair P;
        mat3_mul(lo_Rinv + 9 * il, hi_R + 9 * ih, P.R);
        const int ah = hi_row_anchor ? hi_row_anchor[ih] : ih, al = lo_row_anchor ? lo_row_anchor[il] : il;
        for (int d = 0; d < 3; d++) { P.ph[d] = hi_p[3 * ah + d]; P.pl[d] = lo_p[3 * al + d]; }
        pose_vox_setup(P.R, P.ph[0], P.ph[1], P.ph[2], P.pl[0], P.pl[1], P.pl[2], Bf, &P.vf);
        pose_vox_setup(P.R, P.ph[0], P.ph[1], P.ph[2], P.pl[0], P.pl[1], P.pl[2], Bc, &P.vc);
        rec[p] = P;
    }
}

__global__ __launch_bounds__(256) void k_pose_prep(const int32_t *__restrict__ pair_hi, const int32_t *__restrict__ pair_lo,
                                                   const int32_t *__restrict__ status, int64_t cap_pairs,
                                                   const double *__restrict__ hi_p, const double *__restrict__ hi_R,
                                                   const double *__restrict__ lo_p, const double *__restrict__ lo_Rinv,
                                                   const int32_t *__restrict__ hi_row_anchor, const int32_t *__restrict__ lo_row_anchor,
                                                   PoseBits Bf, PoseBits Bc, PosePair *__restrict__ rec) {
    if (status[ST_FLAG_C] || status[ST_FLAG_PAIRS]) return;
    const int64_t n_pairs = min((int64_t)status[ST_NPAIRS], cap_pairs);
    pose_prep_range(pair_hi, pair_lo, n_pairs, (int64_t)blockIdx.x * 256 + threadIdx.x, (int64_t)gridDim.x * 256, hi_p, hi_R, lo_p, lo_Rinv,
                    hi_row_anchor, lo_row_anchor, Bf, Bc, rec);
}

struct PoseSetup {
    const double *pts; const uint8_t *used; int n;
    PoseGrid G;
    int32_t *cell_start; unsigned short *cell_start16; double *sorted; float4 *sorted_f; int32_t *n_used;
    CloudJob J;
    PoseBitsJobs bits; int n_bit_jobs; int n_bits_wgs;
    const int32_t *pair_hi, *pair_lo; const int32_t *status; int64_t cap_pairs;
    const double *hi_p, *hi_R, *lo_p, *lo_Rinv; const int32_t *hi_row_anchor, *lo_row_anchor;
    PoseBits Bf, Bc; PosePair *rec;
    int roles;
};

__global__ __launch_bounds__(1024, 8) void k_pose_setup(PoseSetup S) {
    extern __shared__ __align__(16) unsigned char smem[];
    __shared__ int wt[17];
    __shared__ int carry;
    const int b = (int)blockIdx.x;
    if (b == 0) {
        if (S.roles & 1) pose_grid_block(S.pts, S.used, S.n, S.G, S.cell_start, S.cell_start16, S.sorted, S.sorted_f, S.n_used, (int *)smem, wt, &carry);
        return;
    }
    if (b == 1) {
        if (S.J.subv && (S.roles & 2)) compact_cloud_block(S.J, wt, &carry);
        return;
    }
    if (b < 2 + S.n_bits_wgs) {
        if (!(S.roles & 4)) return;
        const int groups = S.n_bits_wgs * 4 / S.n_bit_jobs;
        const int g = (b - 2) * 4 + ((int)threadIdx.x >> 8);
        const int job = g / groups, first = g % groups;
        if (job >= S.n_bit_jobs) return;
        const PoseBits B = S.bits.B[job];
        for (int p = first; p < S.n; p += groups) {
            if (S.used && !S.used[p]) continue;
            pose_bits_point(B, S.bits.rad[job], S.bits.plane[job], S.bits.planes[job], S.bits.bits[job], S.pts[3 * p], S.pts[3 * p + 1],
                            S.pts[3 * p + 2], (int)threadIdx.x & 255, 256);
        }
        return;
    }
    if (S.status[ST_FLAG_C] || S.status[ST_FLAG_PAIRS] || !(S.roles & 8)) return;
    const int64_t n_pairs = min((int64_t)S.status[ST_NPAIRS], S.cap_pairs);
    const int64_t wg = b - 2 - S.n_bits_wgs, n_wg = (int64_t)gridDim.x - 2 - S.n_bits_wgs;
    pose_prep_range(S.pair_hi, S.pair_lo, n_pairs, wg * 1024 + threadIdx.x, n_wg * 1024, S.hi_p, S.hi_R, S.lo_p, S.lo_Rinv, S.hi_row_anchor,
                    S.lo_row_anchor, S.Bf, S.Bc, S.rec);
}

#define POSE_LDS_THREADS 1024
__device__ __forceinline__ int topk_threshold(const int32_t *__restrict__ hist, int nbins, int64_t k, int *wt, int *sh, int *need);
#define POSE_PARTS 4
#define POSE_RING 256
#define POSE_WAVE_LDS (POSE_RING * 2 + 256)
#define POSE_OWN_CAP 2048

struct PoseOwnSel {
    const unsigned short *upper;
    const int32_t *hist;
    int nbins;
    int64_t k;
    int32_t *sel_out;
    int64_t sel_cap;
    int32_t *status_w;
};

__global__ __launch_bounds__(POSE_LDS_THREADS) void k_pose_lds(const int32_t *__restrict__ status, int64_t cap_pairs,
                                                               const PosePair *__restrict__ rec,
                                                               const double *__restrict__ hi_cloud, const double *__restrict__ lo_sorted,
                                                               const int32_t *__restrict__ cell_start,
                                                               const unsigned short *__restrict__ cell_start16, PoseGrid G, int l_hi_cap,
                                                               int l_lo_cap, float reach, double dd_lim, PoseBits B,
                                                               const unsigned *__restrict__ bits, int32_t *__restrict__ counts,
                                                               const int32_t *__restrict__ sel, PoseOwnSel own) {
    extern __shared__ __align__(16) unsigned char smem[];
    __shared__ int t_wt[POSE_LDS_THREADS / MAD_WAVE + 1];
    __shared__ int t_sh[3];
    __shared__ int s_nloc, s_gbase;
    if (status[ST_FLAG_C] || status[ST_FLAG_PAIRS]) return;
    double *cl = (double *)smem;
    double *lp = (double *)(smem + pad16((size_t)l_hi_cap * 24));
    float4 *clf = (float4 *)((unsigned char *)lp + pad16((size_t)l_lo_cap * 24));
    unsigned short *cs = (unsigned short *)(clf + l_hi_cap);
    unsigned char *wave_lds = (unsigned char *)cs + pad16((size_t)(G.ncell + 1) * 2) + (threadIdx.x >> 6) * POSE_WAVE_LDS;
    unsigned short *ring = (unsigned short *)wave_lds;
    double *recs = (double *)(wave_lds + POSE_RING * 2);
    const bool own_sel = own.upper != nullptr;
    const bool listed = own_sel || sel != nullptr;
    const int parts = listed ? POSE_PARTS : 1;
    const int l_hi = status[ST_LHI];
    const int l_lo = cell_start[G.ncell];
    stage_lds(lp, lo_sorted, (size_t)l_lo * 24);
    stage_lds(cs, cell_start16, (size_t)((G.ncell + 2) & ~1) * 2);
    stage_lds(cl, hi_cloud, (size_t)l_hi * 24);
    const int lane = lane_id();
    int *own_list = (int *)((unsigned char *)cs + pad16((size_t)(G.ncell + 1) * 2) + (POSE_LDS_THREADS / MAD_WAVE) * POSE_WAVE_LDS);
    if (own_sel) {
        const int64_t n_all = min((int64_t)status[ST_NPAIRS], cap_pairs);
        int need;
        const int T = max(topk_threshold(own.hist, own.nbins, min(own.k, n_all), t_wt, t_sh, &need), 0);
        if (threadIdx.x == 0) s_nloc = 0;
        __syncthreads();
        const int64_t per_wg = (n_all + gridDim.x - 1) / gridDim.x;
        for (int64_t j0 = 0; j0 < per_wg; j0 += POSE_LDS_THREADS) {
            const int64_t i = (int64_t)blockIdx.x + (int64_t)gridDim.x * (j0 + threadIdx.x);
            const bool take = i < n_all && (int)own.upper[i] >= T;
            const unsigned long long bal = __ballot(take);
            if (bal == 0ull) continue;
            int base = 0;
            if (lane == 0) base = atomicAdd(&s_nloc, __popcll(bal));
            base = __shfl(base, 0, MAD_WAVE);
            const int o = base + __popcll(bal & lanemask_lt());
            if (take) {
                if (o < POSE_OWN_CAP) own_list[o] = (int)i;
                counts[i] = 0;
            }
        }
        __syncthreads();
        if (threadIdx.x == 0) {
            const int n_loc = s_nloc;
            if (n_loc > POSE_OWN_CAP) { own.status_w[ST_FLAG_SEL] = 1; s_gbase = -1; }
            else s_gbase = n_loc ? atomicAdd(own.status_w + ST_NSEL, n_loc) : 0;
        }
    }
    __syncthreads();
    if (own_sel) {
        if (s_gbase < 0) return;
        for (int i = threadIdx.x; i < s_nloc; i += POSE_LDS_THREADS)
            if (s_gbase + i < own.sel_cap) own.sel_out[s_gbase + i] = own_list[i];
            else own.status_w[ST_FLAG_SEL] = 1;
    }
    const int *lst = own_sel ? own_list : sel;
    const int64_t n_pairs = own_sel ? (int64_t)s_nloc * parts
                                    : (sel ? (int64_t)status[ST_NSEL] * parts : min((int64_t)status[ST_NPAIRS], cap_pairs));
    for (int i = threadIdx.x; i < l_hi; i += POSE_LDS_THREADS)
        clf[i] = make_float4((float)cl[3 * i], (float)cl[3 * i + 1], (float)cl[3 * i + 2], 0.f);
    __syncthreads();
    const int64_t wave = own_sel ? (int64_t)(threadIdx.x >> 6)
                                 : (int64_t)__builtin_amdgcn_readfirstlane((int)(blockIdx.x * (POSE_LDS_THREADS / MAD_WAVE) + (threadIdx.x >> 6)));
    const int64_t nwaves = own_sel ? (int64_t)(POSE_LDS_THREADS / MAD_WAVE) : (int64_t)gridDim.x * (POSE_LDS_THREADS / MAD_WAVE);
    PosePair cur;
    if (wave < n_pairs) cur = rec[listed ? lst[wave / parts] : wave];
    const float mnx = (float)G.mn[0], mny = (float)G.mn[1], mnz = (float)G.mn[2];
    const int part_len = (l_hi + parts - 1) / parts;
    auto emit = [&](int64_t p, int c) {
        if (listed) atomicAdd(&counts[p], c);
        else counts[p] = c;
    };

    auto exact = [&](int e) -> bool {
        const double *P = recs + 16 * (e >> 15);
        const int a = e & 0x7fff;
        const double d0 = cl[3 * a] - P[9], d1 = cl[3 * a + 1] - P[10], d2 = cl[3 * a + 2] - P[11];
        const double x = (d0 * P[0] + d1 * P[1] + d2 * P[2]) + P[12];
        const double y = (d0 * P[3] + d1 * P[4] + d2 * P[5]) + P[13];
        const double z = (d0 * P[6] + d1 * P[7] + d2 * P[8]) + P[14];
        const float xf = (float)x - mnx, yf = (float)y - mny, zf = (float)z - mnz;
        const int x0 = cvt_floor((xf - reach) * G.inv_cell_f[0]), x1 = cvt_floor((xf + reach) * G.inv_cell_f[0]);
        const int y0 = cvt_floor((yf - reach) * G.inv_cell_f[1]), y1 = cvt_floor((yf + reach) * G.inv_cell_f[1]);
        const int z0 = cvt_floor((zf - reach) * G.inv_cell_f[2]), z1 = cvt_floor((zf + reach) * G.inv_cell_f[2]);
        bool hit = false;
        if (x1 >= 0 && x0 < G.dim[0] && y1 >= 0 && y0 < G.dim[1] && z1 >= 0 && z0 < G.dim[2]) {
            const int zz0 = max(z0, 0), zz1 = min(z1, G.dim[2] - 1) + 1;
            const int xa = max(x0, 0), xb = min(x1, G.dim[0] - 1), ya = max(y0, 0), yb = min(y1, G.dim[1] - 1);
            const int c00 = __mul24(__mul24(xa, G.dim[1]) + ya, G.dim[2]), c01 = __mul24(__mul24(xa, G.dim[1]) + yb, G.dim[2]);
            const int c10 = __mul24(__mul24(xb, G.dim[1]) + ya, G.dim[2]), c11 = __mul24(__mul24(xb, G.dim[1]) + yb, G.dim[2]);
            int s[4], e4[4];
            s[0] = cs[c00 + zz0]; e4[0] = cs[c00 + zz1];
            s[1] = cs[c01 + zz0]; e4[1] = (yb != ya) ? cs[c01 + zz1] : s[1];
            s[2] = cs[c10 + zz0]; e4[2] = (xb != xa) ? cs[c10 + zz1] : s[2];
            s[3] = cs[c11 + zz0]; e4[3] = (xb != xa && yb != ya) ? cs[c11 + zz1] : s[3];
            const int n0 = e4[0] - s[0], n1 = n0 + (e4[1] - s[1]), n2 = n1 + (e4[2] - s[2]), n3 = n2 + (e4[3] - s[3]);
            const int b1 = s[1] - n0, b2 = s[2] - n1, b3 = s[3] - n2;
            for (int t = 0; t < n3 && !hit; t++) {
                const int q = t + (t < n0 ? s[0] : (t < n1 ? b1 : (t < n2 ? b2 : b3)));
                const double e0 = lp[3 * q] - x, e1 = lp[3 * q + 1] - y, e2 = lp[3 * q + 2] - z;
                hit = (e0 * e0 + e1 * e1 + e2 * e2) < dd_lim;
            }
        }
        return hit;
    };

    int head = 0, count = 0;
    int slot = 0;
    int cnt_cur = 0, cnt_old = 0;
    int old_left = 0;
    int64_t p_old = -1;
    auto round = [&](int n_take) {
        __builtin_amdgcn_wave_barrier();
        const int e = lane < n_take ? ring[(head + lane) & (POSE_RING - 1)] : 0;
        __builtin_amdgcn_wave_barrier();
        bool hit = false;
        if (lane < n_take) hit = exact(e);
        const unsigned long long bal = __ballot(hit), mine = __ballot(lane < n_take && (e >> 15) == slot);
        cnt_cur += __popcll(bal & mine);
        cnt_old += __popcll(bal & ~mine);
        head = (head + n_take) & (POSE_RING - 1);
        count -= n_take;
        if (old_left > 0) {
            old_left = max(old_left - n_take, 0);
            if (old_left == 0 && lane == 0) emit(p_old, cnt_old);
        }
    };
    for (int64_t it = wave; it < n_pairs; it += nwaves) {
        const int64_t p = listed ? lst[it / parts] : it;
        const int a_begin = listed ? (int)(it % parts) * part_len : 0, a_end = listed ? min(a_begin + part_len, l_hi) : l_hi;
        PosePair nxt;
        if (it + nwaves < n_pairs) nxt = rec[listed ? lst[(it + nwaves) / parts] : it + nwaves];
        const PoseVox V = cur.vf;
        if (lane == 0) {
            double *P = recs + 16 * slot;
            for (int i = 0; i < 9; i++) P[i] = cur.R[i];
            for (int i = 0; i < 3; i++) { P[9 + i] = cur.ph[i]; P[12 + i] = cur.pl[i]; }
        }
        for (int a0 = a_begin; a0 < a_end; a0 += MAD_WAVE * POSE_BATCH) {
            uint2 word[POSE_BATCH];
            int bit[POSE_BATCH];
            if (a0 + MAD_WAVE * POSE_BATCH <= a_end) {
                unsigned idx[POSE_BATCH];
                bool in[POSE_BATCH];
#pragma unroll
                for (int u = 0; u < POSE_BATCH; u++) {
                    const float4 c = clf[a0 + u * MAD_WAVE + lane];
                    const float vx = fmaf(c.z, V.m[2], fmaf(c.y, V.m[1], fmaf(c.x, V.m[0], V.t[0])));
                    const float vy = fmaf(c.z, V.m[5], fmaf(c.y, V.m[4], fmaf(c.x, V.m[3], V.t[1])));
                    const float vz = fmaf(c.z, V.m[8], fmaf(c.y, V.m[7], fmaf(c.x, V.m[6], V.t[2])));
                    const int ix = cvt_floor(vx), iy = cvt_floor(vy), iz = cvt_floor(vz);
                    bit[u] = iz & 31;
                    in[u] = ((unsigned)ix < (unsigned)B.dim[0]) & ((unsigned)iy < (unsigned)B.dim[1]) & ((unsigned)iz < (unsigned)B.dim[2]);
                    idx[u] = mad_u24(mad_u24((unsigned)ix, (unsigned)B.dim[1], (unsigned)iy), (unsigned)B.wz, (unsigned)(iz >> 5));
                }
#pragma unroll
                for (int u = 0; u < POSE_BATCH; u++) {
                    word[u] = make_uint2(0u, 0u);
                    if (in[u]) word[u] = ((const uint2 *)bits)[idx[u]];
                }
            } else {
#pragma unroll
                for (int u = 0; u < POSE_BATCH; u++) {
                    const int a = a0 + u * MAD_WAVE + lane;
                    word[u] = make_uint2(0u, 0u); bit[u] = 0;
                    if (a < a_end) {
                        const float4 c = clf[a];
                        pose_vox_fetch(V, c.x, c.y, c.z, B, bits, &word[u], &bit[u]);
                    }
                }
            }
#pragma unroll
            for (int u = 0; u < POSE_BATCH; u++) {
                if (a0 + u * MAD_WAVE >= a_end) break;
                const bool certain = (word[u].y >> bit[u]) & 1u;
                cnt_cur += __popcll(__ballot(certain));
                const bool sv = ((word[u].x >> bit[u]) & 1u) && !certain;
                const unsigned long long bal = __ballot(sv);
                if (sv)
                    ring[(head + count + __popcll(bal & lanemask_lt())) & (POSE_RING - 1)] =
                        (unsigned short)((slot << 15) | (a0 + u * MAD_WAVE + lane));
                count += __popcll(bal);
                if (count >= MAD_WAVE) round(MAD_WAVE);
            }
        }
        if (old_left > 0) round(count);
        p_old = p; cnt_old = cnt_cur; cnt_cur = 0; old_left = count;
        if (old_left == 0 && lane == 0) emit(p, cnt_old);
        slot ^= 1;
        cur = nxt;
    }
    if (count > 0) round(count);
}


template <bool HI_LDS>
__global__ __launch_bounds__(POSE_LDS_THREADS) void k_pose_lds32(const int32_t *__restrict__ status, int64_t cap_pairs,
                                                                 const PosePair *__restrict__ rec,
                                                                 const double *__restrict__ hi_cloud, const double *__restrict__ lo_sorted,
                                                                 const float4 *__restrict__ lo_sorted_f,
                                                                 const int32_t *__restrict__ cell_start,
                                                                 const unsigned short *__restrict__ cell_start16, PoseGrid G, int l_lo_cap, int l_hi_cap,
                                                                 float reach, double dd_lim, float lim_in, float lim_out, PoseBits B,
                                                                 const unsigned *__restrict__ bits, int32_t *__restrict__ counts,
                                                                 const int32_t *__restrict__ sel) {
    extern __shared__ __align__(16) unsigned char smem[];
    if (status[ST_FLAG_C] || status[ST_FLAG_PAIRS]) return;
    float4 *lpf = (float4 *)smem;
    unsigned short *cs = (unsigned short *)(lpf + l_lo_cap + 1);
    unsigned short *stack = (unsigned short *)((unsigned char *)cs + pad16((size_t)(G.ncell + 1) * 2)) + (threadIdx.x >> 6) * POSE_STACK;
    const int64_t n_pairs = sel ? (int64_t)status[ST_NSEL] : min((int64_t)status[ST_NPAIRS], cap_pairs);
    const int l_hi = status[ST_LHI];
    const int l_lo = cell_start[G.ncell];
    double *cl = (double *)((unsigned char *)cs + pad16((size_t)(G.ncell + 1) * 2) + (POSE_LDS_THREADS / MAD_WAVE) * POSE_STACK * 2);
    float4 *clf = (float4 *)((unsigned char *)cl + pad16((size_t)l_hi_cap * 24));
    stage_lds(lpf, lo_sorted_f, (size_t)l_lo * 16);
    stage_lds(cs, cell_start16, (size_t)((G.ncell + 2) & ~1) * 2);
// ... 852 lines not shown
}

static int build_cells(mad_ctx *ctx, const double bb_min[3], const double bb_max[3], const double *d_pts, int n, double cell,
                       DevBuf &b_start, DevBuf &b_pts, DevBuf &b_ids, double mn_out[3], int dim_out[3]) {
    size_t ncell = 1;
    for (int d = 0; d < 3; d++) {
        dim_out[d] = (int)floor((bb_max[d] - bb_min[d]) / cell) + 1;
        if (dim_out[d] < 1) dim_out[d] = 1;
        mn_out[d] = bb_min[d];
        ncell *= (size_t)dim_out[d];
    }
    if (ncell > ((size_t)1 << 28)) return mad_fail(ctx, MAD_EINVAL, "cell list of %zu cells is too large", ncell);
    MAD_TRY(mad_reserve(ctx, b_start, (ncell + 1) * 4));
    MAD_TRY(mad_reserve(ctx, b_pts, (size_t)(n > 0 ? n : 1) * 24));
    MAD_TRY(mad_reserve(ctx, b_ids, (size_t)(n > 0 ? n : 1) * 4));
    MAD_TRY(mad_reserve(ctx, mad_sb(ctx, S_TMP_C), (ncell + 1) * 4));
    MAD_TRY(mad_reserve(ctx, mad_sb(ctx, S_TMP_D), (size_t)(n > 0 ? n : 1) * 4));
    int32_t *cnt = scratch<int32_t>(ctx, S_TMP_C);
    int32_t *pt_cell = scratch<int32_t>(ctx, S_TMP_D);
    MAD_HIP(hipMemsetAsync(cnt, 0, (ncell + 1) * 4, ctx->stream));
    if (n > 0) {
        const unsigned nb = (unsigned)mad_ceil_div(n, 256);
        hipLaunchKernelGGL(k_cell_count, dim3(nb), dim3(256), 0, ctx->stream, d_pts, n, bb_min[0], bb_min[1], bb_min[2], 1.0 / cell,
                           dim_out[0], dim_out[1], dim_out[2], cnt, pt_cell);
        MAD_TRY(mad_scan_i32(ctx, cnt, (int32_t *)b_start.p, (int64_t)ncell));
        MAD_HIP(hipMemsetAsync(cnt, 0, (ncell + 1) * 4, ctx->stream));
        hipLaunchKernelGGL(k_cell_fill, dim3(nb), dim3(256), 0, ctx->stream, d_pts, n, pt_cell, (const int32_t *)b_start.p,
                           cnt, (double *)b_pts.p, (int32_t *)b_ids.p);
    } else {
        MAD_HIP(hipMemsetAsync(b_start.p, 0, (ncell + 1) * 4, ctx->stream));
    }
    MAD_HIP(hipGetLastError());
    return MAD_OK;
}

int mad_build_cells(mad_ctx *ctx, mad_set *set, double cell) {
    MAD_TRY(build_cells(ctx, set->bb_min, set->bb_max, (const double *)set->anc_subv.p, set->n_anchors, cell, set->cell_start,
                        set->cell_pts, set->cell_ids, set->cell_min, set->cell_dim));
    set->cell_size = cell;
    set->cells_ready = true;
    return MAD_OK;
}

static double sqrt_limit(double dist) {
    double t = dist * dist;
    while (sqrt(nextafter(t, 0.0)) >= dist) t = nextafter(t, 0.0);
    while (sqrt(t) < dist) t = nextafter(t, INFINITY);
    return t;
}


struct Side {
    const int8_t *dsc8;
    const double *norm;
    const double *R;
    const double *Rinv;
    const int32_t *meta;
    const int32_t *row_anchor;
    const int32_t *anc_canon;
    const double *p;
    const int32_t *n_rows;
    int64_t cap_rows;
    const int32_t *bias = nullptr;
};

template __global__ void k_corr_gemm2<true>(GemmBatchT<true> G);

template <bool WIDE>
static int gemm2_launch(mad_ctx *ctx, const GemmBatchT<WIDE> &G) {
    constexpr int lds = WIDE ? G2_LDS_WIDE : G2_LDS;
    static bool attr = false;
    if (!attr) {
        MAD_HIP(hipFuncSetAttribute((const void *)k_corr_gemm2<WIDE>, hipFuncAttributeMaxDynamicSharedMemorySize, lds));
        attr = true;
    }
    static const int per_cu = getenv("MAD_GEMM_WG_PER_CU") ? std::max(1, std::min(2, atoi(getenv("MAD_GEMM_WG_PER_CU")))) : 2;
    hipLaunchKernelGGL(k_corr_gemm2<WIDE>, dim3(ctx->n_cu * per_cu), dim3(GEMM_THREADS), lds, ctx->stream, G);
    return MAD_OK;
}

static size_t cflag_bytes(int64_t cap_c) { return (size_t)cap_c / 16 + 64; }

static int correlate_reserve(mad_ctx *ctx, const Side &hi, const Side &lo, int D, double cc, int32_t *d_status, int64_t cap_c,
                             int64_t cap_pairs, GemmJob *job) {
    if (D % GEMM_BK) return mad_fail(ctx, MAD_EINVAL, "correlate: D = %d is not a multiple of %d", D, GEMM_BK);
    if (hi.cap_rows > 65000) return mad_fail(ctx, MAD_EINVAL, "correlate: %lld hi rows exceed the single-launch scan", (long long)hi.cap_rows);
    MAD_TRY(mad_reserve(ctx, mad_sb(ctx, S_CMAT), (size_t)cap_c * 4));
    MAD_TRY(mad_reserve(ctx, mad_sb(ctx, S_ROWCNT), (size_t)(hi.cap_rows + 2) * 4));
    MAD_TRY(mad_reserve(ctx, mad_sb(ctx, S_ROWOFF), (size_t)(hi.cap_rows + 2) * 4));
    MAD_TRY(mad_reserve(ctx, mad_sb(ctx, S_PAIR_HI), (size_t)cap_pairs * 4));
    MAD_TRY(mad_reserve(ctx, mad_sb(ctx, S_PAIR_LO), (size_t)cap_pairs * 4));
    MAD_TRY(mad_reserve(ctx, mad_sb(ctx, S_PAIR_SCORE), (size_t)cap_pairs * 8));
    MAD_TRY(mad_reserve(ctx, mad_sb(ctx, S_CMASK), (size_t)cap_c / 8 + 64));
    MAD_TRY(mad_reserve(ctx, mad_sb(ctx, S_CFLAG), cflag_bytes(cap_c)));
    if ((hi.bias != nullptr) != (lo.bias != nullptr))
        return mad_fail(ctx, MAD_EINVAL, "correlate: a wide set (descriptor radius >= %d) against a narrow one", MAD_WIDE_FROM_R);
    *job = GemmJob{{hi.dsc8, lo.dsc8, scratch<int32_t>(ctx, S_CMAT), hi.n_rows, lo.n_rows, cap_c, d_status, hi.norm, lo.norm,
                    scratch<uint32_t>(ctx, S_CMASK), scratch<uint8_t>(ctx, S_CFLAG)}, hi.bias, lo.bias};
    return MAD_OK;
}

static int correlate_gemm(mad_ctx *ctx, int n_jobs, const GemmJob *jobs, int D, double cc) {
    mad_timer_begin(ctx, MAD_T_CORRELATE);
    static const bool no_split = getenv("MAD_GEMM_NO_SPLIT") != nullptr;
    const bool wide = n_jobs > 0 && jobs[0].hb != nullptr;
    for (int j = 1; j < n_jobs; j++)
        if ((jobs[j].hb != nullptr) != wide) return mad_fail(ctx, MAD_EINVAL, "correlate: wide and narrow sets in one batch of matches");
    for (int j0 = 0; j0 < n_jobs; j0 += MAD_BATCH_MAX) {
        if (!wide) {
            GemmBatch G;
            G.n_jobs = std::min(n_jobs - j0, MAD_BATCH_MAX); G.K = D; G.cc = cc;
            G.split_tail = no_split ? 0 : 1;
            for (int j = 0; j < G.n_jobs; j++) G.job[j] = jobs[j0 + j];
            MAD_TRY(gemm2_launch(ctx, G));
            continue;
        }
        GemmBatchT<true> G;
        G.n_jobs = std::min(n_jobs - j0, MAD_BATCH_MAX); G.K = D; G.cc = cc;
        G.split_tail = no_split ? 0 : 1;
        for (int j = 0; j < G.n_jobs; j++) G.job[j] = jobs[j0 + j];
        MAD_TRY(gemm2_launch(ctx, G));
    }
    mad_timer_end(ctx, MAD_T_CORRELATE);
    MAD_HIP(hipGetLastError());
    return MAD_OK;
}

static int correlate_pairs(mad_ctx *ctx, const Side &hi, const Side &lo, double cc, int32_t *d_status, int64_t cap_pairs, uint8_t *d_used_hi,
                           uint8_t *d_used_lo) {
    int32_t *C = scratch<int32_t>(ctx, S_CMAT);
    uint32_t *mask = scratch<uint32_t>(ctx, S_CMASK);
    mad_timer_begin(ctx, MAD_T_PAIRS);
    const uint8_t *cflag = scratch<uint8_t>(ctx, S_CFLAG);
    hipLaunchKernelGGL(k_pair_count, dim3(ctx->n_cu * 4), dim3(256), 0, ctx->stream, C, mask, cflag, hi.n_rows, lo.n_rows, hi.norm, lo.norm, cc,
                       scratch<int32_t>(ctx, S_ROWCNT), d_status);
    hipLaunchKernelGGL(k_pair_emit2, dim3(ctx->n_cu * 4), dim3(256), 0, ctx->stream, C, mask, cflag, hi.n_rows, lo.n_rows, hi.norm, lo.norm,
                       scratch<int32_t>(ctx, S_ROWCNT), cap_pairs, scratch<int32_t>(ctx, S_PAIR_HI), scratch<int32_t>(ctx, S_PAIR_LO),
                       scratch<double>(ctx, S_PAIR_SCORE), hi.row_anchor, lo.row_anchor, hi.anc_canon, lo.anc_canon, d_used_hi, d_used_lo,
                       d_status);
    mad_timer_end(ctx, MAD_T_PAIRS);
    MAD_HIP(hipGetLastError());
    return MAD_OK;
}

static int correlate_device(mad_ctx *ctx, const Side &hi, const Side &lo, int D, double cc, int32_t *d_status, int64_t cap_c,
                            int64_t cap_pairs, uint8_t *d_used_hi, uint8_t *d_used_lo) {
    GemmJob job;
    MAD_TRY(correlate_reserve(ctx, hi, lo, D, cc, d_status, cap_c, cap_pairs, &job));
    mad_zero_words(ctx, job.cflag, cflag_bytes(cap_c));
    MAD_TRY(correlate_gemm(ctx, 1, &job, D, cc));
    return correlate_pairs(ctx, hi, lo, cc, d_status, cap_pairs, d_used_hi, d_used_lo);
}

static int pose_wgs_per_cu() {
    static const int v = getenv("MAD_POSE_WGS") ? atoi(getenv("MAD_POSE_WGS")) : 1;
    return v == 2 ? 2 : 1;
}

struct PosePlan {
    PoseGrid G;
    PoseBits B;
    PoseCoarse PC;
    double bits_rad, bits_rad_in, rad_c_out, dd_lim, reach;
    size_t n_words, fine_bytes, coarse_bytes, lds, lds32, lds32_hi;
    float lim_in, lim_out;
    bool fits64, fits32, hi_in_lds, lds_path, prune;
    int l_hi_max, n_cloud;
};

static void pose_plan(const mad_ctx *ctx, int l_hi_max, int n_cloud, const double bb_min[3], const double bb_max[3], bool have_fallback,
                      double dist, int64_t prune_k, bool have_hist2, PosePlan *Q) {
    PosePlan &P = *Q;
    P.l_hi_max = l_hi_max; P.n_cloud = n_cloud;
    P.dd_lim = sqrt_limit(dist);
    P.reach = dist + 0.01;
    const double reach = P.reach;
    PoseGrid &G = P.G;
    G.ncell = 1;
    for (int d = 0; d < 3; d++) {
        const double ext = bb_max[d] - bb_min[d];
        double cell = 2.0 * reach + 0.05;
        if (ext / cell > 24.0) cell = ext / 24.0;
        G.mn[d] = bb_min[d];
        G.inv_cell[d] = 1.0 / cell;
        G.inv_cell_f[d] = (float)(1.0 / cell);
        G.dim[d] = (int)floor(ext / cell) + 1;
        if (G.dim[d] < 1) G.dim[d] = 1;
        G.ncell *= G.dim[d];
    }
    const size_t stacks = (size_t)(POSE_LDS_THREADS / MAD_WAVE) * POSE_WAVE_LDS;
    const size_t stacks32 = (size_t)(POSE_LDS_THREADS / MAD_WAVE) * POSE_STACK * 2;
    P.lds32 = (size_t)(n_cloud + 1) * 16 + pad16((size_t)(G.ncell + 1) * 2) + stacks32 + 16;
    P.lds32_hi = P.lds32 + pad16((size_t)l_hi_max * 24) + (size_t)l_hi_max * 16;
    P.hi_in_lds = P.lds32_hi <= 150 * 1024;
    const size_t lds_base = pad16((size_t)l_hi_max * 24) + pad16((size_t)n_cloud * 24) + (size_t)l_hi_max * 16 + pad16((size_t)(G.ncell + 1) * 2) +
                            stacks + (size_t)POSE_OWN_CAP * 4 + 16;
    const bool base64 = lds_base <= 150 * 1024;
    const size_t bits_budget = (size_t)16 << 20;
    static const double h0 = getenv("MAD_POSE_VOXEL") ? atof(getenv("MAD_POSE_VOXEL")) : 0.8;
    PoseBits &B = P.B;
    const double slack = 0.02;
    for (B.h = (h0 >= 0.25 && h0 <= 8.0) ? h0 : 0.8;; B.h *= 1.08) {
        const double guard = dist + B.h * 0.8660254037844387 + slack + B.h;
        for (int d = 0; d < 3; d++) {
            B.mn[d] = bb_min[d] - guard;
            B.dim[d] = (int)ceil((bb_max[d] - bb_min[d] + 2.0 * guard) / B.h) + 1;
        }
        B.wz = (B.dim[2] + 31) / 32;
        P.n_words = 2 * (size_t)B.dim[0] * B.dim[1] * B.wz;
        if (P.n_words * 4 <= bits_budget) break;
    }
    P.lds = lds_base;
    P.bits_rad = dist + B.h * 0.8660254037844387 + slack;
    P.bits_rad_in = dist - B.h * 0.8660254037844387 - slack;
    {
        PoseBits &Bc = P.PC.B;
        const int nb_sets = (l_hi_max + MAD_WAVE - 1) / MAD_WAVE;
        const size_t q_sets = nb_sets <= 8 ? (size_t)2 * ((nb_sets + 1) & ~1) + 1 : (size_t)((nb_sets + 1) & ~1) + 5;
        const size_t budget = (size_t)150 * 1024 - pad16((size_t)(l_hi_max + 4) * 16) - (size_t)(PB_THREADS / MAD_WAVE) * (q_sets * MAD_WAVE * 2 + 192) - pad16((size_t)(l_hi_max + 1) * 4) - 64;
        size_t n_words_c = 0;
        for (Bc.h = std::max(1.2, B.h);; Bc.h *= 1.05) {
            const double guard = dist + Bc.h * 0.8660254037844387 + slack + Bc.h;
            for (int d = 0; d < 3; d++) {
                Bc.mn[d] = bb_min[d] - guard;
                Bc.dim[d] = (int)ceil((bb_max[d] - bb_min[d] + 2.0 * guard) / Bc.h) + 1;
            }
            Bc.wz = (Bc.dim[2] + 31) / 32;
            n_words_c = (size_t)Bc.dim[0] * Bc.dim[1] * Bc.wz;
            if (n_words_c * 4 <= budget || Bc.h > 16.0) break;
        }
        P.PC.n_words = (int)n_words_c;
        P.rad_c_out = dist + Bc.h * 0.8660254037844387 + slack;
    }
    double M = reach;
    for (int d = 0; d < 3; d++) M = std::max(M, bb_max[d] - bb_min[d] + 2.0 * reach);
    const double ulpM = ldexp(1.0, (int)ceil(log2(M)) - 23);
    const double band = 4.0 * (2.0 * sqrt(3.0) * (dist + 1.0) * ulpM + 1e-5 * dist * dist);
    P.lim_in = nextafterf((float)(dist * dist - band), 0.f);
    P.lim_out = nextafterf((float)(dist * dist + band), 1e30f);
    P.fits64 = base64 && l_hi_max < 32768;
    P.fits32 = P.lds32 <= 150 * 1024 && P.lim_in > 0.f && l_hi_max < 65536;
    P.lds_path = !have_fallback && (P.fits64 || P.fits32) && n_cloud < 65535 && G.ncell <= 30000;
    static const bool no_prune = getenv("MAD_NO_PRUNE") != nullptr;
    P.prune = P.lds_path && prune_k > 0 && have_hist2 && P.bits_rad_in > 0.5 && P.PC.B.h <= 16.0 && l_hi_max <= PB_MAX_SETS * MAD_WAVE && !no_prune;
    P.fine_bytes = P.lds_path ? pad16(P.n_words * 4) : 0;
    P.coarse_bytes = P.prune ? pad16((size_t)P.PC.n_words * 4) : 0;
    (void)ctx;
}

static int pose_device(mad_ctx *ctx, const Side &hi, const Side &lo, int32_t *d_status, int64_t cap_pairs,
                       const double *d_hi_cloud, int l_hi_max, const double *d_cloud, int n_cloud, const uint8_t *d_cloud_used,
                       const double bb_min[3], const double bb_max[3], const CellGrid *fallback, double dist, int64_t prune_k = 0,
                       int32_t *hist2 = nullptr, bool *pruned = nullptr, const CloudJob *job = nullptr, const PosePlan *pre = nullptr,
                       bool fused = false, bool *own_sel = nullptr) {
    if (pruned) *pruned = false;
    if (own_sel) *own_sel = false;
    const CloudJob no_job = {nullptr, nullptr, 0, nullptr, nullptr, nullptr, nullptr, nullptr};
    MAD_TRY(mad_reserve(ctx, mad_sb(ctx, S_COUNTS), (size_t)cap_pairs * 4));
    PosePlan local;
    if (!pre) pose_plan(ctx, l_hi_max, n_cloud, bb_min, bb_max, fallback != nullptr, dist, prune_k, hist2 != nullptr, &local);
    const PosePlan &P = pre ? *pre : local;
    const PoseGrid &G = P.G;
    const PoseBits &B = P.B;
    const PoseCoarse &PC = P.PC;
    const double dd_lim = P.dd_lim, reach = P.reach;
    const bool fits64 = P.fits64;
    if (P.lds_path) {
        MAD_TRY(mad_reserve(ctx, mad_sb(ctx, S_PG_START), (size_t)(G.ncell + 2) * 4 + pad16((size_t)(G.ncell + 2) * 2) + 16));
        unsigned short *d_start16 = (unsigned short *)(scratch<char>(ctx, S_PG_START) + pad16((size_t)(G.ncell + 2) * 4));
        MAD_TRY(mad_reserve(ctx, mad_sb(ctx, S_PG_PTS), (size_t)(n_cloud + 2) * 24));
        if (!fits64) MAD_TRY(mad_reserve(ctx, mad_sb(ctx, S_PG_PTSF), (size_t)(n_cloud + 2) * 16));
        static bool attr_set = false;
        if (!attr_set) {
            MAD_HIP(hipFuncSetAttribute((const void *)k_pose_lds32<true>, hipFuncAttributeMaxDynamicSharedMemorySize, 160 * 1024));
            MAD_HIP(hipFuncSetAttribute((const void *)k_pose_lds32<false>, hipFuncAttributeMaxDynamicSharedMemorySize, 160 * 1024));
            MAD_HIP(hipFuncSetAttribute((const void *)k_pose_lds, hipFuncAttributeMaxDynamicSharedMemorySize, 159 * 1024));
            MAD_HIP(hipFuncSetAttribute((const void *)k_pose_grid_build, hipFuncAttributeMaxDynamicSharedMemorySize, 150 * 1024));
            MAD_HIP(hipFuncSetAttribute((const void *)k_pose_setup, hipFuncAttributeMaxDynamicSharedMemorySize, 150 * 1024));
            attr_set = true;
        }
        const bool prune = P.prune;
        static const bool dbg_prune = getenv("MAD_DEBUG_PRUNE") != nullptr;
        if (dbg_prune)
            fprintf(stderr, "pose_device: prune=%d prune_k=%lld hist2=%p rad_in=%g coarse h=%g l_hi_max=%d fits64=%d fits32=%d fine h=%g n_cloud=%d\n", (int)prune,
                    (long long)prune_k, (void *)hist2, P.bits_rad_in, PC.B.h, l_hi_max, (int)fits64, (int)P.fits32, B.h, n_cloud);
        const size_t fine_bytes = P.fine_bytes, coarse_bytes = P.coarse_bytes;
        if (!pre) {
            MAD_TRY(mad_reserve(ctx, mad_sb(ctx, S_PG_BITS), fine_bytes + coarse_bytes + 16));
            mad_zero_words(ctx, scratch<unsigned>(ctx, S_PG_BITS), fine_bytes + coarse_bytes);
        }
        unsigned *d_bits = scratch<unsigned>(ctx, S_PG_BITS);
        unsigned *d_bits_c = (unsigned *)(scratch<char>(ctx, S_PG_BITS) + fine_bytes);
        PoseBitsJobs J;
        int n_jobs = 0;
        auto bjob = [&](const PoseBits &b, double rad, int plane, int planes, unsigned *bits) {
            J.B[n_jobs] = b; J.rad[n_jobs] = rad; J.plane[n_jobs] = plane; J.planes[n_jobs] = planes; J.bits[n_jobs] = bits; n_jobs++;
        };
        bjob(B, P.bits_rad, 0, 2, d_bits);
        if (P.bits_rad_in > 0.5) bjob(B, P.bits_rad_in, 1, 2, d_bits);
        if (prune) bjob(PC.B, P.rad_c_out, 0, 1, d_bits_c);
        for (int j = n_jobs; j < 4; j++) { J.B[j] = B; J.rad[j] = 0; J.plane[j] = 0; J.planes[j] = 2; J.bits[j] = nullptr; }
        MAD_TRY(mad_reserve(ctx, mad_sb(ctx, S_PG_PAIRS), (size_t)cap_pairs * sizeof(PosePair)));
        PosePair *d_rec = scratch<PosePair>(ctx, S_PG_PAIRS);
        if (fused) {
            PoseSetup S;
            S.pts = d_cloud; S.used = d_cloud_used; S.n = n_cloud; S.G = G;
            S.cell_start = scratch<int32_t>(ctx, S_PG_START); S.cell_start16 = d_start16; S.sorted = scratch<double>(ctx, S_PG_PTS);
            S.sorted_f = fits64 ? (float4 *)nullptr : scratch<float4>(ctx, S_PG_PTSF); S.n_used = d_status + ST_LLO;
            S.J = job ? *job : no_job;
            S.bits = J; S.n_bit_jobs = n_jobs; S.n_bits_wgs = n_jobs * 64;
            S.pair_hi = scratch<int32_t>(ctx, S_PAIR_HI); S.pair_lo = scratch<int32_t>(ctx, S_PAIR_LO); S.status = d_status; S.cap_pairs = cap_pairs;
            S.hi_p = hi.p; S.hi_R = hi.R; S.lo_p = lo.p; S.lo_Rinv = lo.Rinv; S.hi_row_anchor = hi.row_anchor; S.lo_row_anchor = lo.row_anchor;
            S.Bf = B; S.Bc = PC.B; S.rec = d_rec;
            const int prep_wgs = std::max(ctx->n_cu * 2 - 2 - S.n_bits_wgs, ctx->n_cu / 2);
            S.roles = 15;
            hipLaunchKernelGGL(k_pose_setup, dim3((unsigned)(2 + S.n_bits_wgs + prep_wgs)), dim3(1024), (size_t)G.ncell * 4, ctx->stream, S);
            static const bool probe_setup = getenv("MAD_PROBE_SETUP") != nullptr;
            if (probe_setup)
                for (int r = 1; r < 16; r <<= 1) {
                    S.roles = r;
                    hipLaunchKernelGGL(k_pose_setup, dim3((unsigned)(2 + S.n_bits_wgs + prep_wgs)), dim3(1024), (size_t)G.ncell * 4, ctx->stream, S);
                }
        } else {
            hipLaunchKernelGGL(k_pose_grid_build, dim3(1), dim3(1024), (size_t)G.ncell * 4, ctx->stream, d_cloud, d_cloud_used, n_cloud, G,
                               scratch<int32_t>(ctx, S_PG_START), d_start16, scratch<double>(ctx, S_PG_PTS),
                               fits64 ? (float4 *)nullptr : scratch<float4>(ctx, S_PG_PTSF), d_status + ST_LLO, job ? *job : no_job);
            hipLaunchKernelGGL(k_pose_bits, dim3((unsigned)std::min(std::max(n_cloud, 1), ctx->n_cu * 4), n_jobs), dim3(256), 0, ctx->stream,
                               (const double *)scratch<double>(ctx, S_PG_PTS), (const int32_t *)scratch<int32_t>(ctx, S_PG_START), G.ncell, J);
            hipLaunchKernelGGL(k_pose_prep, dim3(ctx->n_cu * 8), dim3(256), 0, ctx->stream, scratch<int32_t>(ctx, S_PAIR_HI),
                               scratch<int32_t>(ctx, S_PAIR_LO), d_status, cap_pairs, hi.p, hi.R, lo.p, lo.Rinv, hi.row_anchor, lo.row_anchor, B, PC.B, d_rec);
        }
        ctx->last_pose_kernel = fits64 ? 0 : 1;
        mad_timer_begin(ctx, MAD_T_POSE);
        const int32_t *d_sel = nullptr;
        PoseOwnSel own = {nullptr, nullptr, 0, 0, nullptr, 0, nullptr};
        if (prune) {
            MAD_TRY(mad_reserve(ctx, mad_sb(ctx, S_TMP_C), (size_t)cap_pairs * 2 + 64));
            MAD_TRY(mad_reserve(ctx, mad_sb(ctx, S_TMP_D), (size_t)cap_pairs * 4 + 64));
            const int nbins = l_hi_max + 1;
            static bool attr_b = false;
            if (!attr_b) {
                MAD_HIP(hipFuncSetAttribute((const void *)k_pose_bounds<2, false>, hipFuncAttributeMaxDynamicSharedMemorySize, 155 * 1024));
                MAD_HIP(hipFuncSetAttribute((const void *)k_pose_bounds<2, true>, hipFuncAttributeMaxDynamicSharedMemorySize, 155 * 1024));
                MAD_HIP(hipFuncSetAttribute((const void *)k_pose_bounds<4, false>, hipFuncAttributeMaxDynamicSharedMemorySize, 155 * 1024));
                MAD_HIP(hipFuncSetAttribute((const void *)k_pose_bounds<4, true>, hipFuncAttributeMaxDynamicSharedMemorySize, 155 * 1024));
                MAD_HIP(hipFuncSetAttribute((const void *)k_pose_bounds<6, false>, hipFuncAttributeMaxDynamicSharedMemorySize, 155 * 1024));
                MAD_HIP(hipFuncSetAttribute((const void *)k_pose_bounds<6, true>, hipFuncAttributeMaxDynamicSharedMemorySize, 155 * 1024));
                MAD_HIP(hipFuncSetAttribute((const void *)k_pose_bounds<8, false>, hipFuncAttributeMaxDynamicSharedMemorySize, 155 * 1024));
                MAD_HIP(hipFuncSetAttribute((const void *)k_pose_bounds<8, true>, hipFuncAttributeMaxDynamicSharedMemorySize, 155 * 1024));
                MAD_HIP(hipFuncSetAttribute((const void *)k_pose_bounds<10, false>, hipFuncAttributeMaxDynamicSharedMemorySize, 155 * 1024));
                MAD_HIP(hipFuncSetAttribute((const void *)k_pose_bounds<10, true>, hipFuncAttributeMaxDynamicSharedMemorySize, 155 * 1024));
                MAD_HIP(hipFuncSetAttribute((const void *)k_pose_bounds<12, false>, hipFuncAttributeMaxDynamicSharedMemorySize, 155 * 1024));
                MAD_HIP(hipFuncSetAttribute((const void *)k_pose_bounds<12, true>, hipFuncAttributeMaxDynamicSharedMemorySize, 155 * 1024));
                MAD_HIP(hipFuncSetAttribute((const void *)k_pose_bounds<16, false>, hipFuncAttributeMaxDynamicSharedMemorySize, 155 * 1024));
                MAD_HIP(hipFuncSetAttribute((const void *)k_pose_bounds<16, true>, hipFuncAttributeMaxDynamicSharedMemorySize, 155 * 1024));
                MAD_HIP(hipFuncSetAttribute((const void *)k_pose_bounds_mx<2>, hipFuncAttributeMaxDynamicSharedMemorySize, 155 * 1024));
                MAD_HIP(hipFuncSetAttribute((const void *)k_pose_bounds_mx<4>, hipFuncAttributeMaxDynamicSharedMemorySize, 155 * 1024));
                MAD_HIP(hipFuncSetAttribute((const void *)k_pose_bounds_mx<6>, hipFuncAttributeMaxDynamicSharedMemorySize, 155 * 1024));
                MAD_HIP(hipFuncSetAttribute((const void *)k_pose_bounds_mx<8>, hipFuncAttributeMaxDynamicSharedMemorySize, 155 * 1024));
                attr_b = true;
            }
            const bool split = ctx->pose_split >= 0 ? ctx->pose_split != 0 : l_hi_max > 8 * MAD_WAVE;
            static const int split_factor = getenv("MAD_POSE_SPLIT_FACTOR") ? atoi(getenv("MAD_POSE_SPLIT_FACTOR")) : 64;
            const int64_t target_a = std::max<int64_t>(ctx->pose_split_min, (int64_t)split_factor * prune_k);
            const int nb = (l_hi_max + MAD_WAVE - 1) / MAD_WAVE;
            const int nbv = nb <= 2 ? 2 : (nb <= 4 ? 4 : (nb <= 6 ? 6 : (nb <= 8 ? 8 : (nb <= 10 ? 10 : (nb <= 12 ? 12 : 16)))));
            const size_t lds_b = pad16((size_t)PC.n_words * 4) + pad16((size_t)(l_hi_max + 4) * 16) + (size_t)(PB_THREADS / MAD_WAVE) * (nbv + 1) * MAD_WAVE * 2 +
                                 pad16((size_t)nbins * 4) + 16;
#define MAD_PB_LAUNCH(NBV, SPL)                                                                                                              \
    hipLaunchKernelGGL((k_pose_bounds<NBV, SPL>), dim3(ctx->n_cu), dim3(PB_THREADS), lds_b, ctx->stream, d_status, cap_pairs, d_rec, d_hi_cloud, B, \
                       d_bits, PC, d_bits_c, scratch<int32_t>(ctx, S_COUNTS), scratch<unsigned short>(ctx, S_TMP_C), hist2, nbins,              \
                       (const double *)scratch<double>(ctx, S_PAIR_SCORE), pb_phase, target_a, pb_stop)
            static_assert(3 <= 17, "hist2 has l_hi_max + 17 words (zr_hist2): bins 0 .. l_hi_max, then T_stop and the ticket");
            if (split && nbins + 3 > l_hi_max + 17) return mad_fail(ctx, MAD_EINVAL, "pose bounds: %d bins for %d hi anchors", nbins, l_hi_max);
            const bool mx = ctx->pose_mx != 0 && !split && nbv <= 8;
            if (mx) {
                const size_t lds_mx = pad16((size_t)PC.n_words * 4) + pad16((size_t)(l_hi_max + 4) * 16) +
                                      (size_t)(PB_THREADS / MAD_WAVE) * ((size_t)(2 * nbv + 1) * MAD_WAVE * 2 + 192) + pad16((size_t)nbins * 4) + 16;
                if (lds_mx > (size_t)155 * 1024) return mad_fail(ctx, MAD_EINVAL, "pose bounds: %zu bytes of LDS", lds_mx);
#define MAD_PBX_LAUNCH(NBV)                                                                                                                        \
    hipLaunchKernelGGL((k_pose_bounds_mx<NBV>), dim3(ctx->n_cu), dim3(PB_THREADS), lds_mx, ctx->stream, d_status, cap_pairs, d_rec, d_hi_cloud, B, \
                       d_bits, PC, d_bits_c, scratch<int32_t>(ctx, S_COUNTS), scratch<unsigned short>(ctx, S_TMP_C), hist2, nbins)
                if (nbv == 2) MAD_PBX_LAUNCH(2);
                else if (nbv == 4) MAD_PBX_LAUNCH(4);
                else if (nbv == 6) MAD_PBX_LAUNCH(6);
                else MAD_PBX_LAUNCH(8);
#undef MAD_PBX_LAUNCH
            }
            for (int pass = 0; pass < (mx ? 0 : (split ? 2 : 1)); pass++) {
                const int pb_phase = split ? pass + 1 : 0;
                const int64_t pb_stop = split ? prune_k : 0;
                if (split) {
                    if (nbv == 2) MAD_PB_LAUNCH(2, true);
                    else if (nbv == 4) MAD_PB_LAUNCH(4, true);
                    else if (nbv == 6) MAD_PB_LAUNCH(6, true);
                    else if (nbv == 8) MAD_PB_LAUNCH(8, true);
                    else if (nbv == 10) MAD_PB_LAUNCH(10, true);
                    else if (nbv == 12) MAD_PB_LAUNCH(12, true);
                    else MAD_PB_LAUNCH(16, true);
                } else {
                    if (nbv == 2) MAD_PB_LAUNCH(2, false);
                    else if (nbv == 4) MAD_PB_LAUNCH(4, false);
                    else if (nbv == 6) MAD_PB_LAUNCH(6, false);
                    else if (nbv == 8) MAD_PB_LAUNCH(8, false);
                    else if (nbv == 10) MAD_PB_LAUNCH(10, false);
                    else if (nbv == 12) MAD_PB_LAUNCH(12, false);
                    else MAD_PB_LAUNCH(16, false);
                }
            }
#undef MAD_PB_LAUNCH
            if (fused && fits64 && ctx->lane_sel_hint[ctx->lane] > 0) {
                own.upper = scratch<unsigned short>(ctx, S_TMP_C); own.hist = hist2; own.nbins = nbins; own.k = prune_k;
                own.sel_out = scratch<int32_t>(ctx, S_TMP_D); own.sel_cap = cap_pairs; own.status_w = d_status;
                if (own_sel) *own_sel = true;
            } else {
                hipLaunchKernelGGL(k_prune_select, dim3(ctx->n_cu / 2), dim3(256), 0, ctx->stream, d_status, cap_pairs, hist2, nbins, prune_k,
                                   scratch<unsigned short>(ctx, S_TMP_C), scratch<int32_t>(ctx, S_TMP_D), d_status + ST_NSEL, hist2 + nbins,
                                   fits64 ? scratch<int32_t>(ctx, S_COUNTS) : (int32_t *)nullptr);
                d_sel = scratch<int32_t>(ctx, S_TMP_D);
            }
            if (pruned) *pruned = true;
        }
        unsigned wgs_sel = (unsigned)ctx->n_cu;
        if ((d_sel || own.upper) && ctx->lane_sel_hint[ctx->lane] > 0)
            wgs_sel = (unsigned)std::min<int64_t>(ctx->n_cu, std::max<int64_t>(16, (ctx->lane_sel_hint[ctx->lane] * (fits64 ? POSE_PARTS : 1) * 5 / 4) / (POSE_LDS_THREADS / MAD_WAVE) + 4));
        const bool listed = d_sel || own.upper;
        if (fits64)
            hipLaunchKernelGGL(k_pose_lds, dim3(listed ? wgs_sel : ctx->n_cu * (P.lds > 80 * 1024 ? 1 : pose_wgs_per_cu())), dim3(POSE_LDS_THREADS), P.lds, ctx->stream, d_status, cap_pairs, d_rec,
                               d_hi_cloud, scratch<double>(ctx, S_PG_PTS), scratch<int32_t>(ctx, S_PG_START), d_start16, G,
                               l_hi_max, n_cloud, (float)reach, dd_lim, B, d_bits, scratch<int32_t>(ctx, S_COUNTS), d_sel, own);
        else if (P.hi_in_lds)
            hipLaunchKernelGGL(k_pose_lds32<true>, dim3(d_sel ? wgs_sel : ctx->n_cu), dim3(POSE_LDS_THREADS), P.lds32_hi, ctx->stream, d_status, cap_pairs, d_rec,
                               d_hi_cloud, scratch<double>(ctx, S_PG_PTS), scratch<float4>(ctx, S_PG_PTSF),
                               scratch<int32_t>(ctx, S_PG_START), d_start16, G, n_cloud, l_hi_max, (float)reach, dd_lim, P.lim_in, P.lim_out, B, d_bits,
                               scratch<int32_t>(ctx, S_COUNTS), d_sel);
        else
            hipLaunchKernelGGL(k_pose_lds32<false>, dim3(d_sel ? wgs_sel : ctx->n_cu), dim3(POSE_LDS_THREADS), P.lds32, ctx->stream, d_status, cap_pairs, d_rec,
                               d_hi_cloud, scratch<double>(ctx, S_PG_PTS), scratch<float4>(ctx, S_PG_PTSF),
                               scratch<int32_t>(ctx, S_PG_START), d_start16, G, n_cloud, l_hi_max, (float)reach, dd_lim, P.lim_in, P.lim_out, B, d_bits,
                               scratch<int32_t>(ctx, S_COUNTS), d_sel);
        mad_timer_end(ctx, MAD_T_POSE);
        MAD_HIP(hipGetLastError());
        return MAD_OK;
    }
    if (!fallback) return mad_fail(ctx, MAD_EINVAL, "pose: clouds of %d + %d points need the global cell list", l_hi_max, n_cloud);
    if (job) hipLaunchKernelGGL(k_compact_cloud, dim3(1), dim3(1024), 0, ctx->stream, *job);
    const size_t lds2 = (size_t)l_hi_max * 24;
    if (lds2 > 150 * 1024) return mad_fail(ctx, MAD_EINVAL, "pose: hi cloud of %d anchors does not fit LDS", l_hi_max);
    MAD_HIP(hipFuncSetAttribute((const void *)k_pose, hipFuncAttributeMaxDynamicSharedMemorySize, 160 * 1024));
    MAD_HIP(hipMemsetAsync(d_status + ST_LLO, 0, 4, ctx->stream));
    if (d_cloud_used)
        hipLaunchKernelGGL(k_count_flags, dim3((unsigned)mad_ceil_div(n_cloud, 256)), dim3(256), 0, ctx->stream, d_cloud_used, n_cloud,
                           d_status + ST_LLO);
    else
        MAD_HIP(hipMemcpyAsync(d_status + ST_LLO, &n_cloud, 4, hipMemcpyHostToDevice, ctx->stream));
    ctx->last_pose_kernel = 2;
    mad_timer_begin(ctx, MAD_T_POSE);
    hipLaunchKernelGGL(k_pose, dim3(ctx->n_cu * 8), dim3(POSE_THREADS), lds2, ctx->stream, scratch<int32_t>(ctx, S_PAIR_HI),
                       scratch<int32_t>(ctx, S_PAIR_LO), d_status, cap_pairs, hi.p, hi.R, lo.p, lo.Rinv, hi.row_anchor, lo.row_anchor,
                       d_hi_cloud, *fallback, dd_lim, scratch<int32_t>(ctx, S_COUNTS));
    mad_timer_end(ctx, MAD_T_POSE);
    MAD_HIP(hipGetLastError());
    return MAD_OK;
}

static bool clouds_fit_lds(int64_t l_hi, int64_t l_lo) {
    const size_t cells = 15632 * 2 + 16 + 64;
    const size_t fixed = cells + (POSE_LDS_THREADS / MAD_WAVE) * POSE_WAVE_LDS + (size_t)POSE_OWN_CAP * 4, fixed32 = cells + (POSE_LDS_THREADS / MAD_WAVE) * POSE_STACK * 2;
    return ((size_t)(l_hi + l_lo) * 24 + (size_t)l_hi * 16 + fixed <= 150 * 1024 || (size_t)(l_lo + 1) * 16 + fixed32 <= 150 * 1024) && l_lo < 65535 &&
           l_hi < 65536;
}

static int32_t *status_words(mad_ctx *ctx) {
    return scratch<int32_t>(ctx, S_MISC) + 64;
}


static int stage_rows(mad_ctx *ctx, const int16_t *h_rows, int64_t n, int D, int slot16, int slot8, int slotn, int32_t *d_n,
                      int32_t *d_bad) {
    const int64_t n_pad = mad_ceil_div(n > 0 ? n : 1, GEMM_BM) * GEMM_BM;
    MAD_TRY(mad_reserve(ctx, mad_sb(ctx, slot16), (size_t)n * D * 2));
    MAD_TRY(mad_reserve(ctx, mad_sb(ctx, slot8), (size_t)n_pad * D));
    MAD_TRY(mad_reserve(ctx, mad_sb(ctx, slotn), (size_t)n_pad * 8));
    const int32_t n32 = (int32_t)n;
    MAD_HIP(hipMemcpyAsync(d_n, &n32, 4, hipMemcpyHostToDevice, ctx->stream));
    MAD_HIP(hipMemcpyAsync(mad_sb(ctx, slot16).p, h_rows, (size_t)n * D * 2, hipMemcpyHostToDevice, ctx->stream));
    hipLaunchKernelGGL(k_pack_rows, dim3((unsigned)std::min<int64_t>(mad_ceil_div(n_pad, 4), 4096)), dim3(256), 0, ctx->stream,
                       scratch<int16_t>(ctx, slot16), d_n, D, scratch<int8_t>(ctx, slot8), scratch<double>(ctx, slotn), d_bad);
    MAD_HIP(hipGetLastError());
    return MAD_OK;
}

extern "C" int mad_correlate(mad_ctx *ctx, const int16_t *hi, int64_t n_hi, const int16_t *lo, int64_t n_lo, int D,
                             double cc, int32_t *pair_hi, int32_t *pair_lo, double *pair_score, int64_t *n_pairs,
                             int64_t cap) {
    if (ctx) mad_use_lane(ctx, 0);
    if (!ctx || !n_pairs) return MAD_EINVAL;
    *n_pairs = 0;
    if (n_hi <= 0 || n_lo <= 0) return MAD_OK;
    if (!hi || !lo) return mad_fail(ctx, MAD_EINVAL, "mad_correlate: NULL descriptors");
    if (n_hi * n_lo >= ((int64_t)1 << 31)) return mad_fail(ctx, MAD_EINVAL, "mad_correlate: %lld x %lld too large", (long long)n_hi, (long long)n_lo);
    MAD_TRY(mad_reserve(ctx, mad_sb(ctx, S_MISC), 4096));
    int32_t *st = status_words(ctx);
    MAD_HIP(hipMemsetAsync(st, 0, ST_COUNT * 4, ctx->stream));
    MAD_TRY(stage_rows(ctx, hi, n_hi, D, S_HI16, S_HI8, S_HNORM, st + ST_NHI, st + ST_BAD));
    MAD_TRY(stage_rows(ctx, lo, n_lo, D, S_LO16, S_LO8, S_LNORM, st + ST_NLO, st + ST_BAD));
    const int64_t hp = mad_ceil_div(n_hi, GEMM_BM) * GEMM_BM, lp = mad_ceil_div(n_lo, GEMM_BN) * GEMM_BN;
    const Side H = {scratch<int8_t>(ctx, S_HI8), scratch<double>(ctx, S_HNORM), nullptr, nullptr, nullptr, nullptr, nullptr, nullptr, st + ST_NHI, n_hi};
    const Side L = {scratch<int8_t>(ctx, S_LO8), scratch<double>(ctx, S_LNORM), nullptr, nullptr, nullptr, nullptr, nullptr, nullptr, st + ST_NLO, n_lo};
    const int32_t *hs = (const int32_t *)&ctx->pinned[0];
    int64_t cap_pairs = std::max<int64_t>(cap, 1);
    for (int attempt = 0; attempt < 2; attempt++) {
        MAD_TRY(correlate_device(ctx, H, L, D, cc, st, hp * lp, cap_pairs, nullptr, nullptr));
        MAD_HIP(hipMemcpyAsync(&ctx->pinned[0], st, ST_COUNT * 4, hipMemcpyDeviceToHost, ctx->stream));
        MAD_HIP(hipStreamSynchronize(ctx->stream));
        if (hs[ST_BAD]) return mad_fail(ctx, MAD_EDOM, "descriptor count outside the int8 range");
        *n_pairs = hs[ST_NPAIRS];
        if (!hs[ST_FLAG_PAIRS]) break;
        if (*n_pairs > cap) return mad_fail(ctx, MAD_ENOSPC, "mad_correlate: %lld pairs, capacity %lld", (long long)*n_pairs, (long long)cap);
        cap_pairs = *n_pairs;
        MAD_HIP(hipMemsetAsync(st + ST_FLAG_PAIRS, 0, 4, ctx->stream));
    }
    const int64_t np = *n_pairs;
    if (np > cap) return mad_fail(ctx, MAD_ENOSPC, "mad_correlate: %lld pairs, capacity %lld", (long long)np, (long long)cap);
    if (np > 0) {
        if (pair_hi) MAD_HIP(hipMemcpyAsync(pair_hi, mad_sb(ctx, S_PAIR_HI).p, np * 4, hipMemcpyDeviceToHost, ctx->stream));
        if (pair_lo) MAD_HIP(hipMemcpyAsync(pair_lo, mad_sb(ctx, S_PAIR_LO).p, np * 4, hipMemcpyDeviceToHost, ctx->stream));
        if (pair_score) MAD_HIP(hipMemcpyAsync(pair_score, mad_sb(ctx, S_PAIR_SCORE).p, np * 8, hipMemcpyDeviceToHost, ctx->stream));
        MAD_HIP(hipStreamSynchronize(ctx->stream));
    }
    return MAD_OK;
}

extern "C" int mad_pose_score(mad_ctx *ctx, const int32_t *pair_hi, const int32_t *pair_lo, const double *pair_score,
                              int64_t n_pairs, const double *hi_p, const double *hi_R, const int32_t *hi_meta, int64_t n_hi,
                              const double *lo_p, const double *lo_R, const int32_t *lo_meta, int64_t n_lo,
                              const double *hi_cloud, int64_t l_hi, const double *lo_cloud, int64_t l_lo, double dist,
                              double *results, int32_t *counts) {
    if (ctx) mad_use_lane(ctx, 0);
    if (!ctx) return MAD_EINVAL;
    if (n_pairs <= 0) return MAD_OK;
    if (!pair_hi || !pair_lo || !pair_score || !hi_p || !hi_R || !hi_meta || !lo_p || !lo_R || !lo_meta || !hi_cloud || !lo_cloud)
        return mad_fail(ctx, MAD_EINVAL, "mad_pose_score: NULL argument");
    if (l_hi <= 0 || l_lo <= 0 || !(dist > 0)) return mad_fail(ctx, MAD_EINVAL, "mad_pose_score: empty cloud or dist <= 0");
    struct Up { int slot; const void *src; size_t bytes; };
    const Up ups[] = {
        {S_PAIR_HI, pair_hi, (size_t)n_pairs * 4}, {S_PAIR_LO, pair_lo, (size_t)n_pairs * 4},
        {S_PAIR_SCORE, pair_score, (size_t)n_pairs * 8},
        {S_TMP_E, hi_p, (size_t)n_hi * 24}, {S_TMP_F, hi_R, (size_t)n_hi * 72}, {S_TMP_G, hi_meta, (size_t)n_hi * 12},
        {S_TMP_H, lo_p, (size_t)n_lo * 24}, {S_TMP_I, lo_R, (size_t)n_lo * 72}, {S_TMP_J, lo_meta, (size_t)n_lo * 12},
        {S_HI_CLOUD, hi_cloud, (size_t)l_hi * 24}, {S_USED_LO, lo_cloud, (size_t)l_lo * 24},
    };
    for (const Up &u : ups) {
        MAD_TRY(mad_reserve(ctx, mad_sb(ctx, u.slot), u.bytes));
        MAD_HIP(hipMemcpyAsync(mad_sb(ctx, u.slot).p, u.src, u.bytes, hipMemcpyHostToDevice, ctx->stream));
    }
    MAD_TRY(mad_reserve(ctx, mad_sb(ctx, S_TMP_A), (size_t)n_lo * 72));
    MAD_TRY(mad_reserve(ctx, mad_sb(ctx, S_MISC), 4096));
    int32_t *st = status_words(ctx);
    int32_t hs[ST_COUNT] = {0};
    hs[ST_NPAIRS] = (int32_t)n_pairs; hs[ST_LHI] = (int32_t)l_hi; hs[ST_NHI] = (int32_t)n_hi; hs[ST_NLO] = (int32_t)n_lo;
    MAD_HIP(hipMemcpyAsync(st, hs, sizeof(hs), hipMemcpyHostToDevice, ctx->stream));
    hipLaunchKernelGGL(k_row_aux, dim3(64), dim3(256), 0, ctx->stream, scratch<double>(ctx, S_TMP_I), st + ST_NLO,
                       scratch<double>(ctx, S_TMP_A), (const int32_t *)nullptr, (const int32_t *)nullptr, (const int32_t *)nullptr,
                       (const int32_t *)nullptr, (int32_t *)nullptr);
    double bmn[3] = {0, 0, 0}, bmx[3] = {0, 0, 0};
    for (int64_t i = 0; i < l_lo; i++)
        for (int d = 0; d < 3; d++) {
            const double v = lo_cloud[3 * i + d];
            if (i == 0 || v < bmn[d]) bmn[d] = v;
            if (i == 0 || v > bmx[d]) bmx[d] = v;
        }
    const Side H = {nullptr, nullptr, scratch<double>(ctx, S_TMP_F), nullptr, scratch<int32_t>(ctx, S_TMP_G), nullptr,
                    nullptr, scratch<double>(ctx, S_TMP_E), st + ST_NHI, n_hi};
    const Side L = {nullptr, nullptr, scratch<double>(ctx, S_TMP_I), scratch<double>(ctx, S_TMP_A), scratch<int32_t>(ctx, S_TMP_J),
                    nullptr, nullptr, scratch<double>(ctx, S_TMP_H), st + ST_NLO, n_lo};
    CellGrid G;
    const bool fits = clouds_fit_lds(l_hi, l_lo);
    if (!fits) {
        double mn[3];
        int dim[3];
        MAD_TRY(build_cells(ctx, bmn, bmx, scratch<double>(ctx, S_USED_LO), (int)l_lo, dist, mad_sb(ctx, S_CELL_START),
                            mad_sb(ctx, S_CELL_PTS), mad_sb(ctx, S_CELL_IDS), mn, dim));
        G.start = scratch<int32_t>(ctx, S_CELL_START); G.pts = scratch<double>(ctx, S_CELL_PTS); G.ids = scratch<int32_t>(ctx, S_CELL_IDS);
        G.used = nullptr;
        for (int d = 0; d < 3; d++) { G.mn[d] = mn[d]; G.dim[d] = dim[d]; }
        G.cell = dist;
    }
    MAD_TRY(pose_device(ctx, H, L, st, n_pairs, scratch<double>(ctx, S_HI_CLOUD), (int)l_hi, scratch<double>(ctx, S_USED_LO), (int)l_lo,
                        nullptr, bmn, bmx, fits ? nullptr : &G, dist));
    if (results) {
        MAD_TRY(mad_reserve(ctx, mad_sb(ctx, S_RESULTS), (size_t)n_pairs * MAD_RESULT_COLS * 8));
        hipLaunchKernelGGL(k_results, dim3((unsigned)std::min<int64_t>(mad_ceil_div(n_pairs, 256), 4096)), dim3(256), 0, ctx->stream,
                           (const int64_t *)nullptr, st + ST_NPAIRS, n_pairs, scratch<int32_t>(ctx, S_PAIR_HI),
                           scratch<int32_t>(ctx, S_PAIR_LO), scratch<double>(ctx, S_PAIR_SCORE), scratch<int32_t>(ctx, S_COUNTS), st,
                           H.p, H.R, H.meta, L.p, L.Rinv, L.meta, (const int32_t *)nullptr, (const int32_t *)nullptr,
                           scratch<double>(ctx, S_RESULTS), 0);
// ... 712 lines not shown
    int rc = match_finish(ctx, ri, M.hi[i], M.lo, &M.plans[ri], res_i, idx_i, &M.n_out[i], st_i);
    for (int attempt = 0; rc == 1 && attempt < 5; attempt++) {
        mad_use_lane(ctx, lane);
        MAD_TRY(match_enqueue(ctx, M.hi[i], M.lo, M.cc, M.dist, M.plans[ri]));
        MAD_HIP(hipStreamSynchronize(ctx->stream));
        rc = match_finish(ctx, ri, M.hi[i], M.lo, &M.plans[ri], res_i, idx_i, &M.n_out[i], st_i);
    }
    if (rc == 1) return mad_fail(ctx, MAD_EHIP, "mad_match_topk_many: capacity negotiation did not converge");
    if (rc == 0 && M.plans[ri].want_used) {
        const uint8_t *f = (const uint8_t *)ctx->host_used[M.slot][ri];
        const int n_hi = M.hi[i]->n_anchors, n_lo = M.lo->n_anchors;
        if (M.used_hi && n_hi > 0) memcpy(M.used_hi + M.hi_off[i], f, (size_t)n_hi);
        if (M.used_lo && n_lo > 0) memcpy(M.used_lo + (size_t)i * n_lo, f + ((n_hi + 31) & ~31), (size_t)n_lo);
    }
    return rc;
}

static int used_reserve(mad_ctx *ctx, const mad_set *hi, const mad_set *lo, MatchPlan *P) {
    const size_t want = (size_t)used_words(hi->n_anchors, lo->n_anchors) * 4;
    void *&buf = ctx->host_used[ctx->res_slot][ctx->res_idx];
    size_t &cap = ctx->host_used_cap[ctx->res_slot][ctx->res_idx];
    if (cap < want) {
        if (buf) {
            MAD_HIP(hipStreamSynchronize(ctx->stream));
            (void)hipHostFree(buf);
            buf = nullptr;
            cap = 0;
        }
        if (hipHostMalloc(&buf, want * 2) != hipSuccess) return mad_fail(ctx, MAD_ENOMEM, "pinned flag staging of %zu bytes", want * 2);
        cap = want * 2;
    }
    P->want_used = true;
    return MAD_OK;
}

extern "C" int mad_match_topk_many_begin2(mad_ctx *ctx, int n, const mad_set *const *hi, const mad_set *lo, double cc, double dist, int64_t k,
                                          double *results, int64_t *pair_index, int64_t *n_out, int64_t *stats, uint8_t *used_hi,
                                          uint8_t *used_lo) {
    if (!ctx || !hi || !lo || !n_out || n < 0) return MAD_EINVAL;
    if (ctx->many_open >= MAD_BRACKETS) return mad_fail(ctx, MAD_EINVAL, "mad_match_topk_many_begin: %d brackets are open already", MAD_BRACKETS);
    if (k < 1) k = 1;
    ManyState *Mp = new ManyState();
    ManyState &M = *Mp;
    M.slot = (ctx->many_oldest + ctx->many_open) % MAD_BRACKETS;
    ctx->many_open++;
    ctx->res_slot = M.slot;
    M.n = n; M.hi.assign(hi, hi + n); M.lo = lo; M.cc = cc; M.dist = dist; M.k = k;
    M.results = results; M.pair_index = pair_index; M.n_out = n_out; M.stats = stats;
    M.used_hi = used_hi; M.used_lo = used_lo;
    const bool want_used = used_hi || used_lo;
    if (want_used) {
        M.hi_off.assign(n + 1, 0);
        for (int i = 0; i < n; i++) M.hi_off[i + 1] = M.hi_off[i] + (hi[i] ? std::max(hi[i]->n_anchors, 0) : 0);
        if (used_hi && M.hi_off[n] > 0) memset(used_hi, 0, (size_t)M.hi_off[n]);
        if (used_lo && n > 0 && lo->n_anchors > 0) memset(used_lo, 0, (size_t)n * lo->n_anchors);
    }
    for (int l = 0; l < MAD_RES; l++) M.pending[l] = -1;
    ctx->many[M.slot] = Mp;
    int rc_all = MAD_OK;
    const bool no_batch = !ctx->batch_gemm;
    std::vector<int> batch;
    std::vector<GemmJob> jobs;
    bool taken[MAD_LANES] = {};
    for (int i = 0; i < n && rc_all == MAD_OK; i++) {
        n_out[i] = 0;
        if (stats) { stats[4 * i] = stats[4 * i + 1] = stats[4 * i + 2] = stats[4 * i + 3] = 0; }
        if (!hi[i]) { rc_all = mad_fail(ctx, MAD_EINVAL, "mad_match_topk_many: set %d is NULL", i); break; }
        if (match_trivial(hi[i], lo) || no_batch) continue;
        const int lane = hi[i]->lane;
        if (taken[lane] || hi[i]->D != hi[0]->D) continue;
        taken[lane] = true;
        mad_use_lane(ctx, lane);
        ctx->res_idx = lane;
        rc_all = match_prepare(ctx, hi[i], lo, dist, k, &M.plans[lane]);
        if (rc_all == MAD_OK && want_used) rc_all = used_reserve(ctx, hi[i], lo, &M.plans[lane]);
        if (rc_all != MAD_OK) break;
        GemmJob job;
        rc_all = match_enqueue_head(ctx, hi[i], lo, cc, M.plans[lane], &job);
        if (rc_all != MAD_OK) break;
        MAD_HIP(hipEventRecord(ctx->lane_pre[lane], ctx->stream));
        batch.push_back(i);
        jobs.push_back(job);
    }
    if (rc_all == MAD_OK && !batch.empty()) {
        const int g = hi[batch[0]]->lane;
        mad_use_lane(ctx, g);
        for (int i : batch)
            if (hi[i]->lane != g) MAD_HIP(hipStreamWaitEvent(ctx->stream, ctx->lane_pre[hi[i]->lane], 0));
        rc_all = correlate_gemm(ctx, (int)jobs.size(), jobs.data(), hi[batch[0]]->D, cc);
        if (rc_all == MAD_OK) MAD_HIP(hipEventRecord(ctx->gemm_done[M.slot], ctx->stream));
        for (size_t b = 0; b < batch.size() && rc_all == MAD_OK; b++) {
            const int i = batch[b], lane = hi[i]->lane;
            mad_use_lane(ctx, lane);
            ctx->res_idx = lane;
            if (lane != g) MAD_HIP(hipStreamWaitEvent(ctx->stream, ctx->gemm_done[M.slot], 0));
            rc_all = match_enqueue_tail(ctx, hi[i], lo, cc, dist, M.plans[lane]);
            M.pending[lane] = i;
        }
    }
    for (int i = 0; i < n && rc_all == MAD_OK; i++) {
        if (!hi[i] || match_trivial(hi[i], lo)) continue;
        if (std::find(batch.begin(), batch.end(), i) != batch.end()) continue;
        const int lane = hi[i]->lane;
        int ri = lane;
        if (M.pending[ri] >= 0) ri = MAD_LANES + lane;
        if (M.pending[ri] >= 0) {
            ri = lane;
            rc_all = many_retire(ctx, M, ri);
            if (rc_all != MAD_OK) break;
            if (M.pending[MAD_LANES + lane] >= 0) {
                rc_all = many_retire(ctx, M, MAD_LANES + lane);
                if (rc_all != MAD_OK) break;
            }
        }
        mad_use_lane(ctx, lane);
        ctx->res_slot = M.slot;
        ctx->res_idx = ri;
        rc_all = match_prepare(ctx, hi[i], lo, dist, k, &M.plans[ri]);
        if (rc_all == MAD_OK && want_used) rc_all = used_reserve(ctx, hi[i], lo, &M.plans[ri]);
        if (rc_all != MAD_OK) break;
        rc_all = match_enqueue(ctx, hi[i], lo, cc, dist, M.plans[ri]);
        M.pending[ri] = i;
    }
    mad_use_lane(ctx, ctx->match.lane);
    if (rc_all != MAD_OK) {
        for (int l = 0; l < MAD_RES; l++)
            if (M.pending[l] >= 0) { (void)hipEventSynchronize(ctx->lane_done[M.slot][l]); M.pending[l] = -1; }
        const int slot = M.slot;
        delete Mp;
        ctx->many[slot] = nullptr;
        ctx->many_open--;
    }
    ctx->res_slot = 0;
    ctx->res_idx = 0;
    return rc_all;
}

extern "C" int mad_match_topk_many_begin(mad_ctx *ctx, int n, const mad_set *const *hi, const mad_set *lo, double cc, double dist, int64_t k,
                                         double *results, int64_t *pair_index, int64_t *n_out, int64_t *stats) {
    return mad_match_topk_many_begin2(ctx, n, hi, lo, cc, dist, k, results, pair_index, n_out, stats, nullptr, nullptr);
}

extern "C" int mad_set_option(mad_ctx *ctx, const char *name, double value) {
    if (!ctx || !name) return MAD_EINVAL;
    if (!strcmp(name, "pose_split_min")) {
        if (!(value >= 0) || !(value < 1e12)) return mad_fail(ctx, MAD_EINVAL, "mad_set_option: pose_split_min = %g", value);
        ctx->pose_split_min = (int64_t)value;
        return MAD_OK;
    }
    if (!strcmp(name, "pose_mx")) {
        ctx->pose_mx = value != 0 ? 1 : 0;
        return MAD_OK;
    }
    if (!strcmp(name, "pose_split")) {
        ctx->pose_split = value < 0 ? -1 : (value != 0 ? 1 : 0);
        return MAD_OK;
    }
    if (!strcmp(name, "ori_queue") || !strcmp(name, "dsc_queue")) {
        if (!(value >= 0) || !(value < 1e9)) return mad_fail(ctx, MAD_EINVAL, "mad_set_option: %s = %g", name, value);
        (name[0] == 'o' ? ctx->ori_queue_cap : ctx->dsc_queue_cap) = (int)value;
        return MAD_OK;
    }
    if (!strcmp(name, "dsc_ball")) {
        ctx->dsc_ball = value != 0;
        return MAD_OK;
    }
    return mad_fail(ctx, MAD_EINVAL, "mad_set_option: unknown option '%s'", name);
}

extern "C" int mad_set_batching(mad_ctx *ctx, int on) {
    if (!ctx) return MAD_EINVAL;
    ctx->batch_gemm = on != 0;
    return MAD_OK;
}

extern "C" int mad_last_pose_kernel(mad_ctx *ctx) { return ctx ? ctx->last_pose_kernel : -1; }

extern "C" int64_t mad_last_pose_selected(mad_ctx *ctx) { return ctx ? ctx->match.n_sel : -1; }

extern "C" int mad_match_topk_many_finish(mad_ctx *ctx) {
    if (!ctx) return MAD_EINVAL;
    if (ctx->many_open <= 0) return mad_fail(ctx, MAD_EINVAL, "mad_match_topk_many_finish: nothing was begun");
    const int slot = ctx->many_oldest;
    ManyState *Mp = (ManyState *)ctx->many[slot];
    int rc_all = MAD_OK;
    for (int l = 0; l < MAD_RES; l++) {
        const int rc = many_retire(ctx, *Mp, l);
        if (rc_all == MAD_OK) rc_all = rc;
    }
    delete Mp;
    ctx->many[slot] = nullptr;
    ctx->many_oldest = (slot + 1) % MAD_BRACKETS;
    ctx->many_open--;
    ctx->res_slot = 0;
    ctx->res_idx = 0;
    mad_use_lane(ctx, ctx->match.lane);
    return rc_all;
}

void mad_many_abandon(mad_ctx *ctx) {
    for (int r = 0; ctx && r < MAD_BRACKETS; r++)
        if (ctx->many[r]) { delete (ManyState *)ctx->many[r]; ctx->many[r] = nullptr; }
    if (ctx) ctx->many_open = 0;
}

extern "C" int mad_match_topk_many(mad_ctx *ctx, int n, const mad_set *const *hi, const mad_set *lo, double cc, double dist, int64_t k,
                                   double *results, int64_t *pair_index, int64_t *n_out, int64_t *stats) {
    MAD_TRY(mad_match_topk_many_begin(ctx, n, hi, lo, cc, dist, k, results, pair_index, n_out, stats));
    return mad_match_topk_many_finish(ctx);
}

extern "C" int mad_match_topk_many2(mad_ctx *ctx, int n, const mad_set *const *hi, const mad_set *lo, double cc, double dist, int64_t k,
                                    double *results, int64_t *pair_index, int64_t *n_out, int64_t *stats, uint8_t *used_hi, uint8_t *used_lo) {
    MAD_TRY(mad_match_topk_many_begin2(ctx, n, hi, lo, cc, dist, k, results, pair_index, n_out, stats, used_hi, used_lo));
    return mad_match_topk_many_finish(ctx);
}


static Side side_block(const mad_set *s, int64_t begin, const int32_t *d_n_rows, int64_t n) {
    Side x = side_of(s);
    x.dsc8 += begin * s->D; x.norm += begin; x.R += 9 * begin; x.Rinv += 9 * begin; x.meta += 3 * begin; x.row_anchor += begin;
    x.n_rows = d_n_rows; x.cap_rows = n;
    return x;
}

extern "C" int mad_match_shard_pairs(mad_ctx *ctx, const mad_set *hi, const mad_set *lo, int64_t lo_begin, int64_t lo_end, double cc,
                                     uint8_t *used_hi, uint8_t *used_lo, int64_t *n_pairs) {
    if (!ctx || !hi || !lo || !used_hi || !used_lo || !n_pairs) return MAD_EINVAL;
    if (hi->wide || lo->wide) return mad_fail(ctx, MAD_EINVAL, "%s: wide sets (descriptor radius >= %d) are matched whole, on one device", "mad_match_shard_pairs", MAD_WIDE_FROM_R);
    mad_use_lane(ctx, 0);
    *n_pairs = 0;
    ctx->match.shard_hi = nullptr;
    int64_t n_hi = 0, n_lo = 0;
    MAD_TRY(set_rows(ctx, hi, &n_hi));
    MAD_TRY(set_rows(ctx, lo, &n_lo));
    if (hi->D != lo->D) return mad_fail(ctx, MAD_EINVAL, "mad_match_shard_pairs: descriptor lengths %d vs %d", hi->D, lo->D);
    if (lo_begin < 0 || lo_end < lo_begin || lo_end > n_lo) return mad_fail(ctx, MAD_EINVAL, "mad_match_shard_pairs: lo rows [%lld, %lld) of %lld", (long long)lo_begin, (long long)lo_end, (long long)n_lo);
    memset(used_hi, 0, (size_t)hi->n_anchors);
    memset(used_lo, 0, (size_t)lo->n_anchors);
    const int64_t nb = lo_end - lo_begin;
    MAD_TRY(mad_reserve(ctx, mad_sb(ctx, S_ZERO), zero_bytes(hi, lo)));
    int32_t *st = zero_status(ctx);
    uint8_t *d_used_hi = zr_used_hi(st, hi->n_anchors), *d_used_lo = zr_used_lo(st, hi->n_anchors);
    MAD_HIP(hipStreamWaitEvent(ctx->stream, hi->built, 0));
    MAD_HIP(hipStreamWaitEvent(ctx->stream, lo->built, 0));
    int64_t cap_pairs = std::max<int64_t>(ctx->match.cap_pairs, 1 << 16);
    const int64_t cap_c = (mad_ceil_div(std::max<int64_t>(n_hi, 1), 128) * 128) * (mad_ceil_div(std::max<int64_t>(nb, 1), 128) * 128);
    if (cap_c >= ((int64_t)1 << 31)) return mad_fail(ctx, MAD_EINVAL, "mad_match_shard_pairs: score matrix of %lld entries", (long long)cap_c);
    const int32_t *hs = (const int32_t *)&ctx->pinned[0];
    for (int attempt = 0; attempt < 4 && n_hi > 0 && nb > 0; attempt++) {
        mad_zero_words(ctx, st, zero_bytes(hi, lo));
        const int32_t nb32 = (int32_t)nb;
        MAD_HIP(hipMemcpyAsync(st + ST_NLO, &nb32, 4, hipMemcpyHostToDevice, ctx->stream));
        const Side H = side_of(hi), L = side_block(lo, lo_begin, st + ST_NLO, nb);
        MAD_TRY(correlate_device(ctx, H, L, hi->D, cc, st, cap_c, cap_pairs, d_used_hi, d_used_lo));
        MAD_HIP(hipMemcpyAsync(&ctx->pinned[0], st, ST_COUNT * 4, hipMemcpyDeviceToHost, ctx->stream));
        MAD_HIP(hipStreamSynchronize(ctx->stream));
        if (hs[ST_FLAG_C]) return mad_fail(ctx, MAD_EHIP, "mad_match_shard_pairs: score matrix capacity");
        if (!hs[ST_FLAG_PAIRS]) break;
        cap_pairs = (int64_t)hs[ST_NPAIRS] + 1024;
        if (attempt == 3) return mad_fail(ctx, MAD_EHIP, "mad_match_shard_pairs: pair capacity did not converge");
    }
    const int64_t np = (n_hi > 0 && nb > 0) ? hs[ST_NPAIRS] : 0;
    if (np > 0) {
        MAD_HIP(hipMemcpyAsync(used_hi, d_used_hi, (size_t)hi->n_anchors, hipMemcpyDeviceToHost, ctx->stream));
        MAD_HIP(hipMemcpyAsync(used_lo, d_used_lo, (size_t)lo->n_anchors, hipMemcpyDeviceToHost, ctx->stream));
        MAD_HIP(hipStreamSynchronize(ctx->stream));
    }
    ctx->match.cap_pairs = std::max(ctx->match.cap_pairs, cap_pairs);
    ctx->match.shard_hi = hi; ctx->match.shard_lo = lo;
    ctx->match.shard_begin = lo_begin; ctx->match.shard_end = lo_end; ctx->match.shard_pairs = np; ctx->match.shard_cap_pairs = cap_pairs;
    *n_pairs = np;
    return MAD_OK;
}

extern "C" int mad_match_shard_topk(mad_ctx *ctx, const mad_set *hi, const mad_set *lo, const uint8_t *used_hi_all,
                                    const uint8_t *used_lo_all, double dist, int64_t k, double *results, int64_t *pair_rank,
                                    int32_t *counts, int64_t *n_out, int64_t *l_hi) {
    if (!ctx || !hi || !lo || !used_hi_all || !used_lo_all || !results || !pair_rank || !counts || !n_out) return MAD_EINVAL;
    mad_use_lane(ctx, 0);
    *n_out = 0;
    if (l_hi) *l_hi = 0;
    if (ctx->match.shard_hi != hi || ctx->match.shard_lo != lo) return mad_fail(ctx, MAD_EINVAL, "mad_match_shard_topk: call mad_match_shard_pairs for these sets first");
    if (!(dist > 0) || k < 1) return mad_fail(ctx, MAD_EINVAL, "mad_match_shard_topk: dist %g k %lld", dist, (long long)k);
    int64_t n_lo = 0;
    MAD_TRY(set_rows(ctx, lo, &n_lo));
    const int64_t np = ctx->match.shard_pairs, begin = ctx->match.shard_begin, nb = ctx->match.shard_end - begin;
    int32_t *st = zero_status(ctx);
    int32_t *hist = zr_hist(st);
    uint8_t *d_used_hi = zr_used_hi(st, hi->n_anchors), *d_used_lo = zr_used_lo(st, hi->n_anchors);
    MAD_HIP(hipMemcpyAsync(d_used_hi, used_hi_all, (size_t)hi->n_anchors, hipMemcpyHostToDevice, ctx->stream));
    MAD_HIP(hipMemcpyAsync(d_used_lo, used_lo_all, (size_t)lo->n_anchors, hipMemcpyHostToDevice, ctx->stream));
    MAD_HIP(hipMemsetAsync(hist, 0, (size_t)(hi->n_anchors + 17) * 8, ctx->stream));
    MAD_HIP(hipMemsetAsync(st + ST_NKEYS, 0, 4, ctx->stream));
    MAD_HIP(hipMemsetAsync(st + ST_NSEL, 0, 4, ctx->stream));
    MAD_TRY(mad_reserve(ctx, mad_sb(ctx, S_HI_CLOUD), (size_t)hi->n_anchors * 24 + 24));
    MAD_TRY(mad_reserve(ctx, mad_sb(ctx, S_SEL_OUT), (size_t)(k + 8) * 8));
    MAD_TRY(mad_reserve(ctx, mad_sb(ctx, S_RESULTS), (size_t)(k + 1) * MAD_RESULT_COLS * 8));
    hipLaunchKernelGGL(k_compact_cloud, dim3(1), dim3(1024), 0, ctx->stream,
                       CloudJob{(const double *)hi->anc_subv.p, d_used_hi, hi->n_anchors, scratch<double>(ctx, S_HI_CLOUD), st + ST_LHI, nullptr, nullptr, st});
    MAD_HIP(hipGetLastError());
    if (np > 0) {
        const Side H = side_of(hi), L = side_block(lo, begin, st + ST_NLO, nb);
        const int64_t cap_pairs = ctx->match.shard_cap_pairs;
        const bool fits = clouds_fit_lds(hi->n_anchors, lo->n_anchors);
        CellGrid G;
        if (!fits) {
            if (!lo->cells_ready || lo->cell_size != dist) {
                MAD_TRY(mad_build_cells(ctx, const_cast<mad_set *>(lo), dist));
                MAD_HIP(hipStreamSynchronize(ctx->stream));
            }
            G.start = (const int32_t *)lo->cell_start.p; G.pts = (const double *)lo->cell_pts.p; G.ids = (const int32_t *)lo->cell_ids.p;
            for (int d = 0; d < 3; d++) { G.mn[d] = lo->cell_min[d]; G.dim[d] = lo->cell_dim[d]; }
            G.cell = lo->cell_size;
            G.used = d_used_lo;
        }
        MAD_TRY(pose_device(ctx, H, L, st, cap_pairs, scratch<double>(ctx, S_HI_CLOUD), hi->n_anchors, (const double *)lo->anc_subv.p,
                            lo->n_anchors, d_used_lo, lo->bb_min, lo->bb_max, fits ? nullptr : &G, dist, k, zr_hist2(st, hi->n_anchors)));
        MAD_TRY(topk_device(ctx, scratch<int32_t>(ctx, S_COUNTS), st, cap_pairs, k, hi->n_anchors, scratch<int64_t>(ctx, S_SEL_OUT), hist));
        hipLaunchKernelGGL(k_results, dim3((unsigned)mad_ceil_div(k, 256)), dim3(256), 0, ctx->stream, scratch<int64_t>(ctx, S_SEL_OUT),
                           st + ST_NKEYS, k, scratch<int32_t>(ctx, S_PAIR_HI), scratch<int32_t>(ctx, S_PAIR_LO),
                           scratch<double>(ctx, S_PAIR_SCORE), scratch<int32_t>(ctx, S_COUNTS), st, H.p, H.R, H.meta, L.p, L.Rinv, L.meta,
                           H.row_anchor, L.row_anchor, scratch<double>(ctx, S_RESULTS), 0);
        MAD_HIP(hipGetLastError());
    }
    MAD_HIP(hipMemcpyAsync(&ctx->pinned[0], st, ST_COUNT * 4, hipMemcpyDeviceToHost, ctx->stream));
    MAD_HIP(hipStreamSynchronize(ctx->stream));
    const int32_t *hs = (const int32_t *)&ctx->pinned[0];
    if (l_hi) *l_hi = hs[ST_LHI];
// ... 457 lines not shown
```

Baseline: 106.9 billion.

## Add narrow-workgroup pose setup and LDS kernels for sharing the GPU under overlap

Templates the pose setup and LDS pose kernels on thread count. It adds a 512-thread setup variant and a 256-thread LDS pose variant with a smaller own-list and less LDS, so several workgroups can co-reside on a CU when other work overlaps. The narrow setup is chosen by default when overlap is enabled. The narrow pose kernel runs only when pose_shared is explicitly 1. The grid builder gains an unrolled load-then-atomic loop. A query API reports which narrow forms ran.

```diff
diff --git a/include/mad_amd.h b/include/mad_amd.h
--- a/include/mad_amd.h
+++ b/include/mad_amd.h
@@ -111,6 +111,7 @@
 int mad_set_option(mad_ctx *ctx, const char *name, double value);
 
 int mad_last_pose_kernel(mad_ctx *ctx);
+int mad_last_pose_shared(mad_ctx *ctx);
 int64_t mad_last_pose_selected(mad_ctx *ctx);
 int64_t mad_device_allocations(mad_ctx *ctx);
 int mad_match_fetch(mad_ctx *ctx, int32_t *pair_hi, int32_t *pair_lo, double *pair_score,
diff --git a/mad_amd/_lib.py b/mad_amd/_lib.py
--- a/mad_amd/_lib.py
+++ b/mad_amd/_lib.py
@@ -19,7 +19,7 @@
     "mad_set_eqsp", "mad_upload_field", "mad_upload_field_device", "mad_free_field",
     "mad_set_orient_window", "mad_orient", "mad_describe", "mad_describe_sized", "mad_correlate", "mad_pose_score", "mad_topk",
     "mad_set_create", "mad_set_destroy", "mad_set_build", "mad_set_build_many", "mad_set_load", "mad_set_mark_wide", "mad_set_is_wide", "mad_set_size", "mad_set_download",
-    "mad_match_topk", "mad_match_topk_many", "mad_match_topk_many_begin", "mad_match_topk_many_finish", "mad_match_topk_many_begin2", "mad_match_topk_many2", "mad_set_batching", "mad_set_option", "mad_last_pose_kernel", "mad_last_pose_selected", "mad_device_allocations", "mad_match_fetch", "mad_match_results", "mad_match_used",
+    "mad_match_topk", "mad_match_topk_many", "mad_match_topk_many_begin", "mad_match_topk_many_finish", "mad_match_topk_many_begin2", "mad_match_topk_many2", "mad_set_batching", "mad_set_option", "mad_last_pose_kernel", "mad_last_pose_shared", "mad_last_pose_selected", "mad_device_allocations", "mad_match_fetch", "mad_match_results", "mad_match_used",
     "mad_match_shard_pairs", "mad_match_shard_topk", "mad_match_shard_begin", "mad_match_shard_score", "mad_match_shard_record_doubles", "mad_match_shard_collect", "mad_match_shard_wait",
     "mad_set_wire_bytes", "mad_set_export", "mad_set_import", "mad_set_lane", "mad_set_stream", "mad_set_bind_lane",
     "mad_upload_density", "mad_refine", "mad_structure_to_density", "mad_ccc", "mad_density_ccc", "mad_dock_refine_score", "mad_grid_overlap", "mad_overlap_matrix",
@@ -572,6 +572,9 @@
     def last_pose_kernel(self):
         return int(self.dll.mad_last_pose_kernel(self.ctx))
 
+    def last_pose_shared(self):
+        return int(self.dll.mad_last_pose_shared(self.ctx))
+
     def last_pose_selected(self):
         return int(self.dll.mad_last_pose_selected(self.ctx))
 
diff --git a/mad_amd/csrc/mad_common.h b/mad_amd/csrc/mad_common.h
--- a/mad_amd/csrc/mad_common.h
+++ b/mad_amd/csrc/mad_common.h
@@ -148,6 +148,7 @@
     int pose_mx = 0;
     int pose_split = -1;
     int64_t n_device_allocs = 0;
+    int pose_shared = -1;
     int64_t pose_split_min = 4096;
     bool batch_gemm = false;
     bool spatial_order = true;
@@ -185,6 +186,7 @@
     hipEvent_t shard_ev[MAD_LANES][MAD_SHARD_RING] = {};
     bool shard_busy[MAD_LANES][MAD_SHARD_RING] = {};
     int shard_next[MAD_LANES] = {};
+    int last_pose_shared = -1;
     int last_pose_kernel = -1;
     int64_t lane_sel_hint[MAD_LANES] = {};
     void *many[MAD_BRACKETS] = {};
diff --git a/mad_amd/csrc/mad_ctx.hip b/mad_amd/csrc/mad_ctx.hip
--- a/mad_amd/csrc/mad_ctx.hip
+++ b/mad_amd/csrc/mad_ctx.hip
@@ -64,6 +64,7 @@
     ctx->batch_gemm = getenv("MAD_GEMM_BATCH") != nullptr;
     if (getenv("MAD_POSE_SPLIT_MIN")) ctx->pose_split_min = atoll(getenv("MAD_POSE_SPLIT_MIN"));
     if (getenv("MAD_POSE_SPLIT")) ctx->pose_split = atoi(getenv("MAD_POSE_SPLIT"));
+    if (getenv("MAD_POSE_SHARED")) { const int v = atoi(getenv("MAD_POSE_SHARED")); ctx->pose_shared = v < 0 ? -1 : (v != 0 ? 1 : 0); }
     if (getenv("MAD_POSE_MX")) ctx->pose_mx = atoi(getenv("MAD_POSE_MX")) != 0;
     if (getenv("MAD_BALL")) ctx->dsc_ball = atoi(getenv("MAD_BALL")) != 0;
     ctx->device = device;
diff --git a/mad_amd/csrc/mad_match.hip b/mad_amd/csrc/mad_match.hip
--- a/mad_amd/csrc/mad_match.hip
+++ b/mad_amd/csrc/mad_match.hip
@@ -513,7 +513,7 @@
     if (J.hi_words && threadIdx.x < 4) J.status[ST_NHI + threadIdx.x] = J.hi_words[threadIdx.x];
     if (J.lo_words && threadIdx.x >= 4 && threadIdx.x < 8) J.status[ST_NLO + threadIdx.x - 4] = J.lo_words[threadIdx.x - 4];
     __syncthreads();
-    for (int b = 0; b < J.n; b += 1024) {
+    for (int b = 0; b < J.n; b += (int)blockDim.x) {
         const int i = b + threadIdx.x;
         const bool p = i < J.n && (!J.used || J.used[i]);
         int tot;
@@ -555,24 +555,40 @@
     return min(max(c, 0), dim - 1);
 }
 
+template <int U>
 __device__ __forceinline__ void pose_grid_block(const double *__restrict__ pts, const uint8_t *__restrict__ used, int n, const PoseGrid &G,
                                                 int32_t *__restrict__ cell_start, unsigned short *__restrict__ cell_start16,
                                                 double *__restrict__ sorted, float4 *__restrict__ sorted_f, int32_t *__restrict__ n_used,
                                                 int *cnt, int *wt, int *carry_p) {
     int &carry = *carry_p;
-    for (int c = threadIdx.x; c < G.ncell; c += 1024) cnt[c] = 0;
+    const int T = (int)blockDim.x;
+    for (int c = threadIdx.x; c < G.ncell; c += T) cnt[c] = 0;
     if (threadIdx.x == 0) carry = 0;
     __syncthreads();
-    for (int i = threadIdx.x; i < n; i += 1024)
-        if (!used || used[i]) {
-            const int c = (pg_cell(pts[3 * i], G.mn[0], G.inv_cell[0], G.dim[0]) * G.dim[1] +
-                           pg_cell(pts[3 * i + 1], G.mn[1], G.inv_cell[1], G.dim[1])) * G.dim[2] +
-                          pg_cell(pts[3 * i + 2], G.mn[2], G.inv_cell[2], G.dim[2]);
-            atomicAdd(&cnt[c], 1);
-        }
+    auto cell_of = [&](double x, double y, double z) {
+        return (pg_cell(x, G.mn[0], G.inv_cell[0], G.dim[0]) * G.dim[1] + pg_cell(y, G.mn[1], G.inv_cell[1], G.dim[1])) * G.dim[2] +
+               pg_cell(z, G.mn[2], G.inv_cell[2], G.dim[2]);
+    };
+    for (int i0 = threadIdx.x; i0 < n; i0 += U * T) {
+        bool take[U];
+        double x[U], y[U], z[U];
+#pragma unroll
+        for (int u = 0; u < U; u++) {
+            const int i = i0 + u * T;
+            take[u] = i < n && (!used || used[i]);
+        }
+#pragma unroll
+        for (int u = 0; u < U; u++) {
+            const int i = min(i0 + u * T, n - 1);
+            x[u] = pts[3 * i]; y[u] = pts[3 * i + 1]; z[u] = pts[3 * i + 2];
+        }
+#pragma unroll
+        for (int u = 0; u < U; u++)
+            if (take[u]) atomicAdd(&cnt[cell_of(x[u], y[u], z[u])], 1);
+    }
     __syncthreads();
     {
-        const int per = (G.ncell + 1023) / 1024;
+        const int per = (G.ncell + T - 1) / T;
         const int c0 = min((int)threadIdx.x * per, G.ncell), c1 = min(c0 + per, G.ncell);
         int sum = 0;
         for (int c = c0; c < c1; c++) sum += cnt[c];
@@ -591,16 +607,27 @@
         cell_start16[G.ncell] = (unsigned short)carry; cell_start16[G.ncell + 1] = 0;
     }
     __syncthreads();
-    for (int i = threadIdx.x; i < n; i += 1024)
-        if (!used || used[i]) {
-            const int c = (pg_cell(pts[3 * i], G.mn[0], G.inv_cell[0], G.dim[0]) * G.dim[1] +
-                           pg_cell(pts[3 * i + 1], G.mn[1], G.inv_cell[1], G.dim[1])) * G.dim[2] +
-                          pg_cell(pts[3 * i + 2], G.mn[2], G.inv_cell[2], G.dim[2]);
-            const int o = atomicAdd(&cnt[c], 1);
-            sorted[3 * o] = pts[3 * i]; sorted[3 * o + 1] = pts[3 * i + 1]; sorted[3 * o + 2] = pts[3 * i + 2];
-            if (sorted_f)
-                sorted_f[o] = make_float4((float)(pts[3 * i] - G.mn[0]), (float)(pts[3 * i + 1] - G.mn[1]), (float)(pts[3 * i + 2] - G.mn[2]), 0.f);
-        }
+    for (int i0 = threadIdx.x; i0 < n; i0 += U * T) {
+        bool take[U];
+        double x[U], y[U], z[U];
+#pragma unroll
+        for (int u = 0; u < U; u++) {
+            const int i = i0 + u * T;
+            take[u] = i < n && (!used || used[i]);
+        }
+#pragma unroll
+        for (int u = 0; u < U; u++) {
+            const int i = min(i0 + u * T, n - 1);
+            x[u] = pts[3 * i]; y[u] = pts[3 * i + 1]; z[u] = pts[3 * i + 2];
+        }
+#pragma unroll
+        for (int u = 0; u < U; u++)
+            if (take[u]) {
+                const int o = atomicAdd(&cnt[cell_of(x[u], y[u], z[u])], 1);
+                sorted[3 * o] = x[u]; sorted[3 * o + 1] = y[u]; sorted[3 * o + 2] = z[u];
+                if (sorted_f) sorted_f[o] = make_float4((float)(x[u] - G.mn[0]), (float)(y[u] - G.mn[1]), (float)(z[u] - G.mn[2]), 0.f);
+            }
+    }
 }
 
 __global__ __launch_bounds__(1024) void k_pose_grid_build(const double *__restrict__ pts, const uint8_t *__restrict__ used, int n,
@@ -614,7 +641,7 @@
         compact_cloud_block(J, wt, &carry);
         __syncthreads();
     }
-    pose_grid_block(pts, used, n, G, cell_start, cell_start16, sorted, sorted_f, n_used, (int *)smem, wt, &carry);
+    pose_grid_block<1>(pts, used, n, G, cell_start, cell_start16, sorted, sorted_f, n_used, (int *)smem, wt, &carry);
 }
 
 __host__ __device__ __forceinline__ size_t pad16(size_t b) { return (b + 15) & ~(size_t)15; }
@@ -787,13 +814,16 @@
     int roles;
 };
 
-__global__ __launch_bounds__(1024, 8) void k_pose_setup(PoseSetup S) {
+#define POSE_SETUP_NARROW 512
+template <int THREADS>
+__global__ __launch_bounds__(THREADS, THREADS == 1024 ? 8 : 6) void k_pose_setup(PoseSetup S) {
     extern __shared__ __align__(16) unsigned char smem[];
     __shared__ int wt[17];
     __shared__ int carry;
+    constexpr int GROUPS = THREADS / 256;
     const int b = (int)blockIdx.x;
     if (b == 0) {
-        if (S.roles & 1) pose_grid_block(S.pts, S.used, S.n, S.G, S.cell_start, S.cell_start16, S.sorted, S.sorted_f, S.n_used, (int *)smem, wt, &carry);
+        if (S.roles & 1) pose_grid_block<1024 / THREADS>(S.pts, S.used, S.n, S.G, S.cell_start, S.cell_start16, S.sorted, S.sorted_f, S.n_used, (int *)smem, wt, &carry);
         return;
     }
     if (b == 1) {
@@ -802,8 +832,8 @@
     }
     if (b < 2 + S.n_bits_wgs) {
         if (!(S.roles & 4)) return;
-        const int groups = S.n_bits_wgs * 4 / S.n_bit_jobs;
-        const int g = (b - 2) * 4 + ((int)threadIdx.x >> 8);
+        const int groups = S.n_bits_wgs * GROUPS / S.n_bit_jobs;
+        const int g = (b - 2) * GROUPS + ((int)threadIdx.x >> 8);
         const int job = g / groups, first = g % groups;
         if (job >= S.n_bit_jobs) return;
         const PoseBits B = S.bits.B[job];
@@ -817,7 +847,7 @@
     if (S.status[ST_FLAG_C] || S.status[ST_FLAG_PAIRS] || !(S.roles & 8)) return;
     const int64_t n_pairs = min((int64_t)S.status[ST_NPAIRS], S.cap_pairs);
     const int64_t wg = b - 2 - S.n_bits_wgs, n_wg = (int64_t)gridDim.x - 2 - S.n_bits_wgs;
-    pose_prep_range(S.pair_hi, S.pair_lo, n_pairs, wg * 1024 + threadIdx.x, n_wg * 1024, S.hi_p, S.hi_R, S.lo_p, S.lo_Rinv, S.hi_row_anchor,
+    pose_prep_range(S.pair_hi, S.pair_lo, n_pairs, wg * THREADS + threadIdx.x, n_wg * THREADS, S.hi_p, S.hi_R, S.lo_p, S.lo_Rinv, S.hi_row_anchor,
                     S.lo_row_anchor, S.Bf, S.Bc, S.rec);
 }
 
@@ -827,6 +857,9 @@
 #define POSE_RING 256
 #define POSE_WAVE_LDS (POSE_RING * 2 + 256)
 #define POSE_OWN_CAP 2048
+#define POSE_NARROW_THREADS 256
+#define POSE_OWN_CAP_NARROW 512
+__host__ __device__ constexpr int pose_own_cap(int threads) { return threads == POSE_NARROW_THREADS ? POSE_OWN_CAP_NARROW : POSE_OWN_CAP; }
 
 struct PoseOwnSel {
     const unsigned short *upper;
@@ -838,7 +871,8 @@
     int32_t *status_w;
 };
 
-__global__ __launch_bounds__(POSE_LDS_THREADS) void k_pose_lds(const int32_t *__restrict__ status, int64_t cap_pairs,
+template <int THREADS>
+__global__ __launch_bounds__(THREADS) void k_pose_lds(const int32_t *__restrict__ status, int64_t cap_pairs,
                                                                const PosePair *__restrict__ rec,
                                                                const double *__restrict__ hi_cloud, const double *__restrict__ lo_sorted,
                                                                const int32_t *__restrict__ cell_start,
@@ -847,7 +881,7 @@
                                                                const unsigned *__restrict__ bits, int32_t *__restrict__ counts,
                                                                const int32_t *__restrict__ sel, PoseOwnSel own) {
     extern __shared__ __align__(16) unsigned char smem[];
-    __shared__ int t_wt[POSE_LDS_THREADS / MAD_WAVE + 1];
+    __shared__ int t_wt[THREADS / MAD_WAVE + 1];
     __shared__ int t_sh[3];
     __shared__ int s_nloc, s_gbase;
     if (status[ST_FLAG_C] || status[ST_FLAG_PAIRS]) return;
@@ -867,7 +901,7 @@
     stage_lds(cs, cell_start16, (size_t)((G.ncell + 2) & ~1) * 2);
     stage_lds(cl, hi_cloud, (size_t)l_hi * 24);
     const int lane = lane_id();
-    int *own_list = (int *)((unsigned char *)cs + pad16((size_t)(G.ncell + 1) * 2) + (POSE_LDS_THREADS / MAD_WAVE) * POSE_WAVE_LDS);
+    int *own_list = (int *)((unsigned char *)cs + pad16((size_t)(G.ncell + 1) * 2) + (THREADS / MAD_WAVE) * POSE_WAVE_LDS);
     if (own_sel) {
         const int64_t n_all = min((int64_t)status[ST_NPAIRS], cap_pairs);
         int need;
@@ -875,7 +909,7 @@
         if (threadIdx.x == 0) s_nloc = 0;
         __syncthreads();
         const int64_t per_wg = (n_all + gridDim.x - 1) / gridDim.x;
-        for (int64_t j0 = 0; j0 < per_wg; j0 += POSE_LDS_THREADS) {
+        for (int64_t j0 = 0; j0 < per_wg; j0 += THREADS) {
             const int64_t i = (int64_t)blockIdx.x + (int64_t)gridDim.x * (j0 + threadIdx.x);
             const bool take = i < n_all && (int)own.upper[i] >= T;
             const unsigned long long bal = __ballot(take);
@@ -885,33 +919,33 @@
             base = __shfl(base, 0, MAD_WAVE);
             const int o = base + __popcll(bal & lanemask_lt());
             if (take) {
-                if (o < POSE_OWN_CAP) own_list[o] = (int)i;
+                if (o < pose_own_cap(THREADS)) own_list[o] = (int)i;
                 counts[i] = 0;
             }
         }
         __syncthreads();
         if (threadIdx.x == 0) {
             const int n_loc = s_nloc;
-            if (n_loc > POSE_OWN_CAP) { own.status_w[ST_FLAG_SEL] = 1; s_gbase = -1; }
+            if (n_loc > pose_own_cap(THREADS)) { own.status_w[ST_FLAG_SEL] = 1; s_gbase = -1; }
             else s_gbase = n_loc ? atomicAdd(own.status_w + ST_NSEL, n_loc) : 0;
         }
     }
     __syncthreads();
     if (own_sel) {
         if (s_gbase < 0) return;
-        for (int i = threadIdx.x; i < s_nloc; i += POSE_LDS_THREADS)
+        for (int i = threadIdx.x; i < s_nloc; i += THREADS)
             if (s_gbase + i < own.sel_cap) own.sel_out[s_gbase + i] = own_list[i];
             else own.status_w[ST_FLAG_SEL] = 1;
     }
     const int *lst = own_sel ? own_list : sel;
     const int64_t n_pairs = own_sel ? (int64_t)s_nloc * parts
                                     : (sel ? (int64_t)status[ST_NSEL] * parts : min((int64_t)status[ST_NPAIRS], cap_pairs));
-    for (int i = threadIdx.x; i < l_hi; i += POSE_LDS_THREADS)
+    for (int i = threadIdx.x; i < l_hi; i += THREADS)
         clf[i] = make_float4((float)cl[3 * i], (float)cl[3 * i + 1], (float)cl[3 * i + 2], 0.f);
     __syncthreads();
     const int64_t wave = own_sel ? (int64_t)(threadIdx.x >> 6)
-                                 : (int64_t)__builtin_amdgcn_readfirstlane((int)(blockIdx.x * (POSE_LDS_THREADS / MAD_WAVE) + (threadIdx.x >> 6)));
-    const int64_t nwaves = own_sel ? (int64_t)(POSE_LDS_THREADS / MAD_WAVE) : (int64_t)gridDim.x * (POSE_LDS_THREADS / MAD_WAVE);
+                                 : (int64_t)__builtin_amdgcn_readfirstlane((int)(blockIdx.x * (THREADS / MAD_WAVE) + (threadIdx.x >> 6)));
+    const int64_t nwaves = own_sel ? (int64_t)(THREADS / MAD_WAVE) : (int64_t)gridDim.x * (THREADS / MAD_WAVE);
     PosePair cur;
     if (wave < n_pairs) cur = rec[listed ? lst[wave / parts] : wave];
     const float mnx = (float)G.mn[0], mny = (float)G.mn[1], mnz = (float)G.mn[2];
@@ -2070,6 +2104,8 @@
     return correlate_pairs(ctx, hi, lo, cc, d_status, cap_pairs, d_used_hi, d_used_lo);
 }
 
+#define POSE_NARROW_LDS_MAX ((size_t)112 * 1024)
+
 static int pose_wgs_per_cu() {
     static const int v = getenv("MAD_POSE_WGS") ? atoi(getenv("MAD_POSE_WGS")) : 1;
     return v == 2 ? 2 : 1;
@@ -2080,9 +2116,9 @@
     PoseBits B;
     PoseCoarse PC;
     double bits_rad, bits_rad_in, rad_c_out, dd_lim, reach;
-    size_t n_words, fine_bytes, coarse_bytes, lds, lds32, lds32_hi;
+    size_t n_words, fine_bytes, coarse_bytes, lds, lds_narrow, lds32, lds32_hi;
     float lim_in, lim_out;
-    bool fits64, fits32, hi_in_lds, lds_path, prune;
+    bool fits64, fits32, fits_narrow, hi_in_lds, lds_path, prune;
     int l_hi_max, n_cloud;
 };
 
@@ -2129,6 +2165,7 @@
         if (P.n_words * 4 <= bits_budget) break;
     }
     P.lds = lds_base;
+    P.lds_narrow = lds_base - stacks - (size_t)POSE_OWN_CAP * 4 + (size_t)(POSE_NARROW_THREADS / MAD_WAVE) * POSE_WAVE_LDS + (size_t)POSE_OWN_CAP_NARROW * 4;
     P.bits_rad = dist + B.h * 0.8660254037844387 + slack;
     P.bits_rad_in = dist - B.h * 0.8660254037844387 - slack;
     {
@@ -2157,6 +2194,7 @@
     P.lim_in = nextafterf((float)(dist * dist - band), 0.f);
     P.lim_out = nextafterf((float)(dist * dist + band), 1e30f);
     P.fits64 = base64 && l_hi_max < 32768;
+    P.fits_narrow = P.fits64 && P.lds_narrow <= POSE_NARROW_LDS_MAX;
     P.fits32 = P.lds32 <= 150 * 1024 && P.lim_in > 0.f && l_hi_max < 65536;
     P.lds_path = !have_fallback && (P.fits64 || P.fits32) && n_cloud < 65535 && G.ncell <= 30000;
     static const bool no_prune = getenv("MAD_NO_PRUNE") != nullptr;
@@ -2192,9 +2230,11 @@
         if (!attr_set) {
             MAD_HIP(hipFuncSetAttribute((const void *)k_pose_lds32<true>, hipFuncAttributeMaxDynamicSharedMemorySize, 160 * 1024));
             MAD_HIP(hipFuncSetAttribute((const void *)k_pose_lds32<false>, hipFuncAttributeMaxDynamicSharedMemorySize, 160 * 1024));
-            MAD_HIP(hipFuncSetAttribute((const void *)k_pose_lds, hipFuncAttributeMaxDynamicSharedMemorySize, 159 * 1024));
+            MAD_HIP(hipFuncSetAttribute((const void *)k_pose_lds<POSE_LDS_THREADS>, hipFuncAttributeMaxDynamicSharedMemorySize, 159 * 1024));
+            MAD_HIP(hipFuncSetAttribute((const void *)k_pose_lds<POSE_NARROW_THREADS>, hipFuncAttributeMaxDynamicSharedMemorySize, (int)POSE_NARROW_LDS_MAX));
             MAD_HIP(hipFuncSetAttribute((const void *)k_pose_grid_build, hipFuncAttributeMaxDynamicSharedMemorySize, 150 * 1024));
-            MAD_HIP(hipFuncSetAttribute((const void *)k_pose_setup, hipFuncAttributeMaxDynamicSharedMemorySize, 150 * 1024));
+            MAD_HIP(hipFuncSetAttribute((const void *)k_pose_setup<1024>, hipFuncAttributeMaxDynamicSharedMemorySize, 150 * 1024));
+            MAD_HIP(hipFuncSetAttribute((const void *)k_pose_setup<POSE_SETUP_NARROW>, hipFuncAttributeMaxDynamicSharedMemorySize, 150 * 1024));
             attr_set = true;
         }
         const bool prune = P.prune;
@@ -2220,24 +2260,34 @@
         for (int j = n_jobs; j < 4; j++) { J.B[j] = B; J.rad[j] = 0; J.plane[j] = 0; J.planes[j] = 2; J.bits[j] = nullptr; }
         MAD_TRY(mad_reserve(ctx, mad_sb(ctx, S_PG_PAIRS), (size_t)cap_pairs * sizeof(PosePair)));
         PosePair *d_rec = scratch<PosePair>(ctx, S_PG_PAIRS);
+        int shared_forms = 0;
         if (fused) {
             PoseSetup S;
             S.pts = d_cloud; S.used = d_cloud_used; S.n = n_cloud; S.G = G;
             S.cell_start = scratch<int32_t>(ctx, S_PG_START); S.cell_start16 = d_start16; S.sorted = scratch<double>(ctx, S_PG_PTS);
             S.sorted_f = fits64 ? (float4 *)nullptr : scratch<float4>(ctx, S_PG_PTSF); S.n_used = d_status + ST_LLO;
             S.J = job ? *job : no_job;
-            S.bits = J; S.n_bit_jobs = n_jobs; S.n_bits_wgs = n_jobs * 64;
+            S.bits = J; S.n_bit_jobs = n_jobs;
             S.pair_hi = scratch<int32_t>(ctx, S_PAIR_HI); S.pair_lo = scratch<int32_t>(ctx, S_PAIR_LO); S.status = d_status; S.cap_pairs = cap_pairs;
             S.hi_p = hi.p; S.hi_R = hi.R; S.lo_p = lo.p; S.lo_Rinv = lo.Rinv; S.hi_row_anchor = hi.row_anchor; S.lo_row_anchor = lo.row_anchor;
             S.Bf = B; S.Bc = PC.B; S.rec = d_rec;
-            const int prep_wgs = std::max(ctx->n_cu * 2 - 2 - S.n_bits_wgs, ctx->n_cu / 2);
+            const bool narrow_setup = ctx->pose_shared >= 0 ? ctx->pose_shared != 0 : ctx->overlap;
+            const int per_wg = narrow_setup ? POSE_SETUP_NARROW / 256 : 4;
+            S.n_bits_wgs = n_jobs * 256 / per_wg;
+            const int prep_wgs = std::max(ctx->n_cu * 2 - 2 - n_jobs * 64, ctx->n_cu / 2) * (4 / per_wg);
+            const dim3 grid((unsigned)(2 + S.n_bits_wgs + prep_wgs));
+            auto launch_setup = [&]() {
+                if (narrow_setup) hipLaunchKernelGGL(k_pose_setup<POSE_SETUP_NARROW>, grid, dim3(POSE_SETUP_NARROW), (size_t)G.ncell * 4, ctx->stream, S);
+                else hipLaunchKernelGGL(k_pose_setup<1024>, grid, dim3(1024), (size_t)G.ncell * 4, ctx->stream, S);
+            };
+            if (narrow_setup) shared_forms |= 2;
             S.roles = 15;
-            hipLaunchKernelGGL(k_pose_setup, dim3((unsigned)(2 + S.n_bits_wgs + prep_wgs)), dim3(1024), (size_t)G.ncell * 4, ctx->stream, S);
+            launch_setup();
             static const bool probe_setup = getenv("MAD_PROBE_SETUP") != nullptr;
             if (probe_setup)
                 for (int r = 1; r < 16; r <<= 1) {
                     S.roles = r;
-                    hipLaunchKernelGGL(k_pose_setup, dim3((unsigned)(2 + S.n_bits_wgs + prep_wgs)), dim3(1024), (size_t)G.ncell * 4, ctx->stream, S);
+                    launch_setup();
                 }
         } else {
             hipLaunchKernelGGL(k_pose_grid_build, dim3(1), dim3(1024), (size_t)G.ncell * 4, ctx->stream, d_cloud, d_cloud_used, n_cloud, G,
@@ -2340,11 +2390,18 @@
             if (pruned) *pruned = true;
         }
         unsigned wgs_sel = (unsigned)ctx->n_cu;
-        if ((d_sel || own.upper) && ctx->lane_sel_hint[ctx->lane] > 0)
-            wgs_sel = (unsigned)std::min<int64_t>(ctx->n_cu, std::max<int64_t>(16, (ctx->lane_sel_hint[ctx->lane] * (fits64 ? POSE_PARTS : 1) * 5 / 4) / (POSE_LDS_THREADS / MAD_WAVE) + 4));
         const bool listed = d_sel || own.upper;
-        if (fits64)
-            hipLaunchKernelGGL(k_pose_lds, dim3(listed ? wgs_sel : ctx->n_cu * (P.lds > 80 * 1024 ? 1 : pose_wgs_per_cu())), dim3(POSE_LDS_THREADS), P.lds, ctx->stream, d_status, cap_pairs, d_rec,
+        const bool narrow = P.fits_narrow && ctx->pose_shared == 1;
+        const int64_t waves_wg = narrow ? (POSE_NARROW_THREADS / MAD_WAVE) * 2 : POSE_LDS_THREADS / MAD_WAVE;
+        if (listed && ctx->lane_sel_hint[ctx->lane] > 0)
+            wgs_sel = (unsigned)std::min<int64_t>(ctx->n_cu, std::max<int64_t>(16, (ctx->lane_sel_hint[ctx->lane] * (fits64 ? POSE_PARTS : 1) * 5 / 4) / waves_wg + 4));
+        if (fits64 && narrow) {
+            shared_forms |= 1;
+            hipLaunchKernelGGL(k_pose_lds<POSE_NARROW_THREADS>, dim3(listed ? wgs_sel : ctx->n_cu), dim3(POSE_NARROW_THREADS), P.lds_narrow, ctx->stream, d_status, cap_pairs, d_rec,
+                               d_hi_cloud, scratch<double>(ctx, S_PG_PTS), scratch<int32_t>(ctx, S_PG_START), d_start16, G,
+                               l_hi_max, n_cloud, (float)reach, dd_lim, B, d_bits, scratch<int32_t>(ctx, S_COUNTS), d_sel, own);
+        } else if (fits64)
+            hipLaunchKernelGGL(k_pose_lds<POSE_LDS_THREADS>, dim3(listed ? wgs_sel : ctx->n_cu * (P.lds > 80 * 1024 ? 1 : pose_wgs_per_cu())), dim3(POSE_LDS_THREADS), P.lds, ctx->stream, d_status, cap_pairs, d_rec,
                                d_hi_cloud, scratch<double>(ctx, S_PG_PTS), scratch<int32_t>(ctx, S_PG_START), d_start16, G,
                                l_hi_max, n_cloud, (float)reach, dd_lim, B, d_bits, scratch<int32_t>(ctx, S_COUNTS), d_sel, own);
         else if (P.hi_in_lds)
@@ -2358,9 +2415,11 @@
                                scratch<int32_t>(ctx, S_PG_START), d_start16, G, n_cloud, l_hi_max, (float)reach, dd_lim, P.lim_in, P.lim_out, B, d_bits,
                                scratch<int32_t>(ctx, S_COUNTS), d_sel);
         mad_timer_end(ctx, MAD_T_POSE);
+        ctx->last_pose_shared = shared_forms;
         MAD_HIP(hipGetLastError());
         return MAD_OK;
     }
+    ctx->last_pose_shared = 0;
     if (!fallback) return mad_fail(ctx, MAD_EINVAL, "pose: clouds of %d + %d points need the global cell list", l_hi_max, n_cloud);
     if (job) hipLaunchKernelGGL(k_compact_cloud, dim3(1), dim3(1024), 0, ctx->stream, *job);
     const size_t lds2 = (size_t)l_hi_max * 24;
@@ -3379,6 +3438,10 @@
         ctx->pose_mx = value != 0 ? 1 : 0;
         return MAD_OK;
     }
+    if (!strcmp(name, "pose_shared")) {
+        ctx->pose_shared = value < 0 ? -1 : (value != 0 ? 1 : 0);
+        return MAD_OK;
+    }
     if (!strcmp(name, "pose_split")) {
         ctx->pose_split = value < 0 ? -1 : (value != 0 ? 1 : 0);
         return MAD_OK;
@@ -3402,6 +3465,7 @@
 }
 
 extern "C" int mad_last_pose_kernel(mad_ctx *ctx) { return ctx ? ctx->last_pose_kernel : -1; }
+extern "C" int mad_last_pose_shared(mad_ctx *ctx) { return ctx ? ctx->last_pose_shared : -1; }
 
 extern "C" int64_t mad_last_pose_selected(mad_ctx *ctx) { return ctx ? ctx->match.n_sel : -1; }
 
```

Result: faster. 108.6 billion (median of 6 runs) (+1.5%).
